# luotuoqingshan/SDPLRPlus.jl

Measured on NVIDIA B200. Metric: AL inner iterations per second, MaxCut on a synthetic 10M-vertex power-law graph (rank 10), higher is better.
Workload: dtype f64

## Files before the change

### sdplrplus.jl_b200/csrc/api.cu

```cuda
#include <math.h>
#include <stdlib.h>
#include <string.h>
#include <algorithm>
#include "common.cuh"

static const char *kNoHandle = "null handle";

#define REQUIRE_H(h) \
    if (!(h)) return SDPLRP_ERR_ARG
#define REQUIRE_PRE(h)                                                                   \
    if (!(h)->preprocessed) return fail(h, SDPLRP_ERR_STATE, "call sdplrp_preprocess first")
#define REQUIRE_RANK(h)                                                                  \
    if ((h)->r <= 0) return fail(h, SDPLRP_ERR_STATE, "call sdplrp_set_rank first")

int32_t fetch_scalars(sdplrp_handle *h, int first, int count) {
    CUDA_TRY(h, cudaMemcpyAsync(h->hscal + first, h->dscal + first, (size_t)count * sizeof(double), cudaMemcpyDeviceToHost, h->stream));
    CUDA_TRY(h, cudaStreamSynchronize(h->stream));
    return SDPLRP_OK;
}

cudaEvent_t prof_begin(sdplrp_handle *h) {
    cudaEvent_t e = nullptr;
    if (!h->ev_free.empty()) { e = h->ev_free.back(); h->ev_free.pop_back(); }
    else if (cudaEventCreate(&e) != cudaSuccess) return nullptr;
    cudaEventRecord(e, h->stream);
    return e;
}
void prof_end(sdplrp_handle *h, int sec, cudaEvent_t a) {
    cudaEvent_t e = nullptr;
    if (!h->ev_free.empty()) { e = h->ev_free.back(); h->ev_free.pop_back(); }
    else if (cudaEventCreate(&e) != cudaSuccess) { h->ev_free.push_back(a); return; }
    cudaEventRecord(e, h->stream);
    h->ev_pending.push_back({sec, a, e});
}
static void prof_collect(sdplrp_handle *h) {
    for (auto &p : h->ev_pending) {
        float ms = 0.f;
        if (cudaEventElapsedTime(&ms, p.a, p.b) == cudaSuccess) { h->sec_ms[p.sec] += ms; h->sec_cnt[p.sec] += 1; }
        h->ev_free.push_back(p.a); h->ev_free.push_back(p.b);
    }
    h->ev_pending.clear();
}

static double *mat_ptr(sdplrp_handle *h, int id) {
    switch (id) {
    case SDPLRP_MAT_R: return h->R;
    case SDPLRP_MAT_G: return h->G;
    case SDPLRP_MAT_D: return h->D;
    case SDPLRP_MAT_W0: return h->W0;
    case SDPLRP_MAT_W1: return h->W1;
    case SDPLRP_MAT_CR: return h->CR;
    case SDPLRP_MAT_CD: return h->CD;
    default: break;
    }
    if (id >= SDPLRP_MAT_S0 && id < SDPLRP_MAT_S0 + h->hist) return h->Sh[id - SDPLRP_MAT_S0];
    if (id >= SDPLRP_MAT_Y0 && id < SDPLRP_MAT_Y0 + h->hist) return h->Yh[id - SDPLRP_MAT_Y0];
    return nullptr;
}

static double *vec_ptr(sdplrp_handle *h, int id, i64 *len) {
    switch (id) {
    case SDPLRP_VEC_LAMBDA: *len = h->m; return h->lambda;
    case SDPLRP_VEC_LAMBDA_UB: *len = h->m; return h->lambda_ub;
    case SDPLRP_VEC_B: *len = h->m; return h->b;
    case SDPLRP_VEC_PVIO_RAW: *len = h->m + 1; return h->pvio_raw;
    case SDPLRP_VEC_Y: *len = h->m + 1; return h->y;
    case SDPLRP_VEC_PVIO_LB: *len = h->m; return h->pvio_lb;
    case SDPLRP_VEC_A_RD: *len = h->m + 1; return h->A_RD;
    case SDPLRP_VEC_A_DD: *len = h->m + 1; return h->A_DD;
    case SDPLRP_VEC_S_NZVAL: *len = h->nnzF; return h->S;
    default: return nullptr;
    }
}

__global__ void k_fill(i64 len, double v, double *__restrict__ x) {
    for (i64 i = blockIdx.x * (i64)blockDim.x + threadIdx.x; i < len; i += (i64)gridDim.x * blockDim.x) x[i] = v;
}
__global__ void k_bounds(i64 m, const unsigned char *__restrict__ ineq, const int *__restrict__ cperm, double *__restrict__ ub,
                         double *__restrict__ lb) {
    for (i64 g = blockIdx.x * (i64)blockDim.x + threadIdx.x; g < m; g += (i64)gridDim.x * blockDim.x) {
        const bool q = ineq && ineq[g];
        const i64 c = cperm ? cperm[g] : g;
        ub[c] = q ? 0.0 : INFINITY;
        lb[c] = q ? 0.0 : -INFINITY;
    }
}

extern "C" {

int32_t sdplrp_version(void) { return 100; }

const char *sdplrp_error_string(int32_t code) {
    switch (code) {
    case SDPLRP_OK: return "ok";
    case SDPLRP_ERR_CUDA: return "CUDA runtime error";
    case SDPLRP_ERR_ARG: return "bad argument";
    case SDPLRP_ERR_STATE: return "call order violated";
    case SDPLRP_ERR_ASYMMETRIC: return "constraint matrix not stored symmetric";
    case SDPLRP_ERR_NCCL: return "NCCL error";
    case SDPLRP_ERR_NO_DEVICE: return "no CUDA device (there is no CPU fallback)";
    case SDPLRP_ERR_LINESEARCH: return "line search slope is positive";
    default: return "unknown error";
    }
}

const char *sdplrp_last_error(sdplrp_handle *h) { return h ? h->err.c_str() : kNoHandle; }

int32_t sdplrp_create(int32_t device, int32_t rank, int32_t world, const void *nccl_id, sdplrp_handle **out) {
    if (!out) return SDPLRP_ERR_ARG;
    *out = nullptr;
    int ndev = 0;
    if (cudaGetDeviceCount(&ndev) != cudaSuccess || ndev <= 0) return SDPLRP_ERR_NO_DEVICE;
    if (device < 0 || device >= ndev || world < 1 || rank < 0 || rank >= world) return SDPLRP_ERR_ARG;
    if (cudaSetDevice(device) != cudaSuccess) return SDPLRP_ERR_CUDA;
    sdplrp_handle *h = new sdplrp_handle();
    h->device = device; h->rank = rank; h->world = world;
    if (const char *e = getenv("SDPLRP_RELABEL")) h->relabel_mode = atoi(e) < 0 ? -1 : (atoi(e) > 0 ? 1 : 0);
    if (const char *e = getenv("SDPLRP_HOT_ROWS")) h->hot_rows = atoll(e);
    if (const char *e = getenv("SDPLRP_LBFGS_KERNEL")) h->lbfgs_kernel = atoi(e);
    if (const char *e = getenv("SDPLRP_SPMM_UNROLL")) h->spmm_unroll = atoi(e);
    if (const char *e = getenv("SDPLRP_SPMM_G0")) h->spmm_g0 = atoi(e);
    if (const char *e = getenv("SDPLRP_LANCZOS_DIST")) h->lanczos_dist = atoi(e) > 0 ? 1 : 0;
    if (cudaStreamCreateWithFlags(&h->stream, cudaStreamNonBlocking) != cudaSuccess) { delete h; return SDPLRP_ERR_CUDA; }
    {
        const char *e = getenv("SDPLRP_CLASS_STREAMS");
        if (!e || atoi(e) != 0) {
            bool ok = cudaEventCreateWithFlags(&h->ev_fork, cudaEventDisableTiming) == cudaSuccess;
            for (int c = 0; c < 2 && ok; c++)
                ok = cudaStreamCreateWithFlags(&h->class_streams[c], cudaStreamNonBlocking) == cudaSuccess &&
                     cudaEventCreateWithFlags(&h->ev_join[c], cudaEventDisableTiming) == cudaSuccess;
            if (!ok) { cudaGetLastError(); h->class_streams[0] = nullptr; }
        }
    }
    if (const char *e = getenv("SDPLRP_L2_FETCH")) {
        if (cudaDeviceSetLimit(cudaLimitMaxL2FetchGranularity, (size_t)atoll(e)) != cudaSuccess) cudaGetLastError();
    }
    if (const char *e = getenv("SDPLRP_L2_PERSIST_MB")) {
        int maxp = 0;
        cudaDeviceGetAttribute(&maxp, cudaDevAttrMaxPersistingL2CacheSize, device);
        const size_t want = std::min<size_t>((size_t)maxp, (size_t)atoll(e) << 20);
        if (cudaDeviceSetLimit(cudaLimitPersistingL2CacheSize, want) == cudaSuccess) h->l2_persist_bytes = (i64)want;
        else cudaGetLastError();
    }
    bool ok = cudaMalloc((void **)&h->dscal, SC_COUNT * sizeof(double)) == cudaSuccess &&
              cudaMallocHost((void **)&h->hscal, SC_COUNT * sizeof(double)) == cudaSuccess &&
              cudaMalloc((void **)&h->partials, (size_t)kPartialsLen * sizeof(double)) == cudaSuccess &&
              cudaMalloc((void **)&h->ticket, 4 * sizeof(unsigned)) == cudaSuccess;
    if (ok) ok = cudaMemset(h->dscal, 0, SC_COUNT * sizeof(double)) == cudaSuccess && cudaMemset(h->ticket, 0, 4 * sizeof(unsigned)) == cudaSuccess;
    if (!ok) { sdplrp_destroy(h); return SDPLRP_ERR_CUDA; }
    memset(h->hscal, 0, SC_COUNT * sizeof(double));
    if (world > 1) {
        int32_t rc = comm_init(h, nccl_id);
        if (rc != SDPLRP_OK) { sdplrp_destroy(h); return rc; }
    }
    *out = h;
    return SDPLRP_OK;
}

static i64 mat_capacity(const sdplrp_handle *h, int r) {
    const i64 rows = h->equal_blocks ? std::max<i64>(h->n, (i64)h->world * h->block_rows) : h->n;
    return rows * (i64)r;
}

static void free_state(sdplrp_handle *h) {
    dev_free(&h->R); dev_free(&h->G); dev_free(&h->D); dev_free(&h->W0); dev_free(&h->W1);
    dev_free(&h->CR); dev_free(&h->CD);
    h->CR_valid = h->CD_valid = false;
    for (int j = 0; j < kMaxHist; j++) { dev_free(&h->Sh[j]); dev_free(&h->Yh[j]); }
    dev_free(&h->lb_small);
    h->gram_pairs_valid = h->gram_g_valid = false; h->gram_prestored = -1;
    dev_free(&h->lr_tmp); h->lr_tmp_len = 0;
    h->r = 0; h->hist = 0;
    h->state_cap = 0;
}

static void free_problem(sdplrp_handle *h) {
    pre_free(h);
    for (LowRank &L : h->lr) { dev_free(&L.dB); dev_free(&L.dD); }
    h->lr.clear();
    dev_free(&h->b); dev_free(&h->lambda); dev_free(&h->lambda_ub); dev_free(&h->pvio_lb);
    dev_free(&h->y); dev_free(&h->pvio_raw); dev_free(&h->pvio_raw_alt); dev_free(&h->A_RD); dev_free(&h->A_DD); dev_free(&h->A_out);
    dev_free(&h->lz_v); dev_free(&h->lz_w); dev_free(&h->lz_vp); dev_free(&h->lz_ab); dev_free(&h->lz_basis);
    h->lz_ab_len = 0; h->lz_basis_len = 0;
    dev_free(&h->stage); h->stage_len = 0;
}

int32_t sdplrp_destroy(sdplrp_handle *h) {
    if (!h) return SDPLRP_OK;
    cudaSetDevice(h->device);
    if (h->stream) cudaStreamSynchronize(h->stream);
    comm_destroy(h);
    prof_collect(h);
    for (cudaEvent_t e : h->ev_free) cudaEventDestroy(e);
    h->ev_free.clear();
    free_state(h);
    free_problem(h);
    dev_free(&h->dscal); dev_free(&h->partials); dev_free(&h->ticket);
    if (h->hscal) cudaFreeHost(h->hscal);
    for (int c = 0; c < 2; c++) {
        if (h->class_streams[c]) cudaStreamDestroy(h->class_streams[c]);
        if (h->ev_join[c]) cudaEventDestroy(h->ev_join[c]);
    }
    if (h->ev_fork) cudaEventDestroy(h->ev_fork);
    if (h->stream) cudaStreamDestroy(h->stream);
    delete h;
    return SDPLRP_OK;
}

int32_t sdplrp_synchronize(sdplrp_handle *h) {
    REQUIRE_H(h);
    CUDA_TRY(h, cudaStreamSynchronize(h->stream));
    return SDPLRP_OK;
}

void *sdplrp_stream(sdplrp_handle *h) { return h ? (void *)h->stream : nullptr; }

static int32_t preprocess_common(sdplrp_handle *h, int64_t n, int64_t m, int64_t nA, const int64_t *mat_off, const int64_t *I,
                                 const int64_t *J, const double *V, const int64_t *gids, bool triplets_on_device);

int32_t sdplrp_preprocess(sdplrp_handle *h, int64_t n, int64_t m, int64_t nA, const int64_t *mat_off, const int64_t *I,
                          const int64_t *J, const double *V, const int64_t *gids) {
    return preprocess_common(h, n, m, nA, mat_off, I, J, V, gids, false);
}

int32_t sdplrp_preprocess_device(sdplrp_handle *h, int64_t n, int64_t m, int64_t nA, const int64_t *mat_off, const int64_t *d_I,
                                 const int64_t *d_J, const double *d_V, const int64_t *gids) {
    REQUIRE_H(h);
    if (nA > 0 && mat_off && mat_off[nA] > 0) {
        if (!d_I || !d_J || !d_V) return fail(h, SDPLRP_ERR_ARG, "preprocess_device: null triplet arrays");
        cudaPointerAttributes at;
        const void *ptrs[3] = {d_I, d_J, d_V};
        for (const void *p : ptrs) {
            if (cudaPointerGetAttributes(&at, p) != cudaSuccess || at.type != cudaMemoryTypeDevice || at.device != h->device) {
                cudaGetLastError();
                return fail(h, SDPLRP_ERR_ARG, "preprocess_device: I, J, V must be device memory of the handle's GPU");
            }
        }
    }
    return preprocess_common(h, n, m, nA, mat_off, d_I, d_J, d_V, gids, true);
}

static int32_t preprocess_common(sdplrp_handle *h, int64_t n, int64_t m, int64_t nA, const int64_t *mat_off, const int64_t *I,
                                 const int64_t *J, const double *V, const int64_t *gids, bool triplets_on_device) {
    REQUIRE_H(h);
    CUDA_TRY(h, cudaSetDevice(h->device));
    free_state(h);
    free_problem(h);
    if (nA > 0 && (!mat_off || !gids)) return fail(h, SDPLRP_ERR_ARG, "preprocess: null arrays");
    int32_t rc = pre_build(h, n, m, nA, mat_off, I, J, V, gids, triplets_on_device);
    if (rc != SDPLRP_OK && rc != SDPLRP_ERR_ASYMMETRIC) return rc;
    SDP_CHECK(dev_alloc(h, &h->b, m)); SDP_CHECK(dev_alloc(h, &h->lambda, m)); SDP_CHECK(dev_alloc(h, &h->lambda_ub, m));
    SDP_CHECK(dev_alloc(h, &h->pvio_lb, m)); SDP_CHECK(dev_alloc(h, &h->y, m + 1)); SDP_CHECK(dev_alloc(h, &h->pvio_raw, m + 1)); SDP_CHECK(dev_alloc(h, &h->pvio_raw_alt, m + 1));
    SDP_CHECK(dev_alloc(h, &h->A_RD, m + 1)); SDP_CHECK(dev_alloc(h, &h->A_DD, m + 1)); SDP_CHECK(dev_alloc(h, &h->A_out, m + 1));
    cudaStream_t st = h->stream;
    CUDA_TRY(h, cudaMemsetAsync(h->b, 0, (size_t)std::max<i64>(m, 1) * 8, st));
    CUDA_TRY(h, cudaMemsetAsync(h->lambda, 0, (size_t)std::max<i64>(m, 1) * 8, st));
    CUDA_TRY(h, cudaMemsetAsync(h->y, 0, (size_t)(m + 1) * 8, st));
    CUDA_TRY(h, cudaMemsetAsync(h->pvio_raw, 0, (size_t)(m + 1) * 8, st));
    CUDA_TRY(h, cudaMemsetAsync(h->pvio_raw_alt, 0, (size_t)(m + 1) * 8, st));
    CUDA_TRY(h, cudaMemsetAsync(h->A_RD, 0, (size_t)(m + 1) * 8, st));
    CUDA_TRY(h, cudaMemsetAsync(h->A_DD, 0, (size_t)(m + 1) * 8, st));
    CUDA_TRY(h, cudaMemsetAsync(h->A_out, 0, (size_t)(m + 1) * 8, st));
    k_bounds<<<grid_for(m, 256, kRedBlocks), 256, 0, st>>>(m, nullptr, h->cperm, h->lambda_ub, h->pvio_lb);
    KLAUNCH(h);
    CUDA_TRY(h, cudaStreamSynchronize(st));
    h->y_obj = 0.0;
    SDP_CHECK(comm_partition(h));
    SDP_CHECK(halo_build(h));
    return rc;
}

int32_t sdplrp_halo_stats(sdplrp_handle *h, int64_t out[7]) {
    REQUIRE_H(h);
    REQUIRE_PRE(h);
    const HaloPlan &p = h->halo;
    out[0] = halo_active(h) ? 1 : 0; out[1] = p.nloc; out[2] = p.lnnz; out[3] = p.n_ghost[0]; out[4] = p.n_ghost[1];
    out[5] = p.n_send[0]; out[6] = p.n_send[1];
    return SDPLRP_OK;
}

int32_t sdplrp_pattern_sizes(sdplrp_handle *h, int64_t *nnzT, int64_t *nnzF, int64_t *Ec) {
    REQUIRE_H(h);
    REQUIRE_PRE(h);
    if (nnzT) *nnzT = h->nnzT;
    if (nnzF) *nnzF = h->nnzF;
    if (Ec) *Ec = h->Ec;
    return SDPLRP_OK;
}

int32_t sdplrp_pattern_export(sdplrp_handle *h, int64_t *triu_colptr, int64_t *triu_rowval, int64_t *matptr, int64_t *nzind,
                              double *nzval_one, double *nzval_two, int64_t *full_colptr, int64_t *full_rowval,
                              int64_t *mappedto_triu) {
    REQUIRE_H(h);
    REQUIRE_PRE(h);
    CUDA_TRY(h, cudaSetDevice(h->device));
    return pre_export(h, triu_colptr, triu_rowval, matptr, nzind, nzval_one, nzval_two, full_colptr, full_rowval, mappedto_triu);
}

int32_t sdplrp_add_symlowrank(sdplrp_handle *h, int64_t global_id, int64_t s, const double *B, const double *D) {
    REQUIRE_H(h);
    REQUIRE_PRE(h);
    if (global_id < 1 || global_id > h->m + 1 || s < 1 || !B || !D) return fail(h, SDPLRP_ERR_ARG, "add_symlowrank: bad argument");
    CUDA_TRY(h, cudaSetDevice(h->device));
    LowRank L;
    int gid_internal = (int)(global_id - 1);
    CUDA_TRY(h, cudaMemcpy(&gid_internal, h->cperm + (global_id - 1), sizeof(int), cudaMemcpyDeviceToHost));
    L.gid = gid_internal; L.s = s; L.dB = nullptr; L.dD = nullptr;
    SDP_CHECK(dev_alloc(h, &L.dB, h->n * s));
    SDP_CHECK(dev_alloc(h, &L.dD, s));
    h->lr.push_back(L);
    SDP_CHECK(perm_upload(h, L.dB, B, s, false));
    CUDA_TRY(h, cudaMemcpy(L.dD, D, (size_t)s * 8, cudaMemcpyHostToDevice));
    return SDPLRP_OK;
}

int32_t sdplrp_set_problem(sdplrp_handle *h, const double *b, const uint8_t *is_ineq) {
    REQUIRE_H(h);
    REQUIRE_PRE(h);
    CUDA_TRY(h, cudaSetDevice(h->device));
    const i64 m = h->m;
    if (m > 0 && !b) return fail(h, SDPLRP_ERR_ARG, "set_problem: null b");
    if (m > 0) SDP_CHECK(perm_cvec_upload(h, h->b, b, m));
    unsigned char *dq = nullptr;
    h->has_ineq = false;
    if (is_ineq) for (i64 i = 0; i < m; i++) h->has_ineq |= is_ineq[i] != 0;
    if (is_ineq && m > 0) {
        CUDA_TRY(h, cudaMalloc((void **)&dq, (size_t)m));
        CUDA_TRY(h, cudaMemcpy(dq, is_ineq, (size_t)m, cudaMemcpyHostToDevice));
    }
    k_bounds<<<grid_for(m, 256, kRedBlocks), 256, 0, h->stream>>>(m, dq, h->cperm, h->lambda_ub, h->pvio_lb);
    KLAUNCH(h);
    cudaError_t e = cudaStreamSynchronize(h->stream);
    if (dq) cudaFree(dq);
    CUDA_TRY(h, e);
    return SDPLRP_OK;
}

int32_t sdplrp_set_rank(sdplrp_handle *h, int32_t r, int32_t numlbfgsvecs) {
    REQUIRE_H(h);
    REQUIRE_PRE(h);
    if (r < 1 || numlbfgsvecs < 0 || numlbfgsvecs > kMaxHist) return fail(h, SDPLRP_ERR_ARG, "set_rank: bad rank / history length");
    CUDA_TRY(h, cudaSetDevice(h->device));
    const i64 N = mat_capacity(h, r);
    const bool reuse = h->R && h->G && h->D && h->lb_small && h->r == r && h->hist == numlbfgsvecs && h->state_cap == N &&
                       ((h->obj_mat >= 0) == (h->CR != nullptr)) && ((h->obj_mat >= 0) == (h->CD != nullptr));
    if (reuse) {
        h->CR_valid = h->CD_valid = false;
        if (h->W0) CUDA_TRY(h, cudaMemsetAsync(h->W0, 0, (size_t)N * 8, h->stream));
        if (h->W1) CUDA_TRY(h, cudaMemsetAsync(h->W1, 0, (size_t)N * 8, h->stream));
    } else {
        free_state(h);
        SDP_CHECK(dev_alloc(h, &h->R, N)); SDP_CHECK(dev_alloc(h, &h->G, N)); SDP_CHECK(dev_alloc(h, &h->D, N));
        if (h->obj_mat >= 0) { SDP_CHECK(dev_alloc(h, &h->CR, N)); SDP_CHECK(dev_alloc(h, &h->CD, N)); }
        for (int j = 0; j < numlbfgsvecs; j++) { SDP_CHECK(dev_alloc(h, &h->Sh[j], N)); SDP_CHECK(dev_alloc(h, &h->Yh[j], N)); }
        SDP_CHECK(dev_alloc(h, &h->lb_small, kLbSmallLen));
        h->state_cap = N;
    }
    h->r = r; h->hist = numlbfgsvecs; h->latest = numlbfgsvecs;
    CUDA_TRY(h, cudaMemsetAsync(h->R, 0, (size_t)N * 8, h->stream));
    CUDA_TRY(h, cudaMemsetAsync(h->G, 0, (size_t)N * 8, h->stream));
    CUDA_TRY(h, cudaMemsetAsync(h->D, 0, (size_t)N * 8, h->stream));
    SDP_CHECK(lb_clear(h));
    CUDA_TRY(h, cudaStreamSynchronize(h->stream));
    return SDPLRP_OK;
}

int32_t sdplrp_set_option(sdplrp_handle *h, const char *key, double value) {
    REQUIRE_H(h);
    if (!key) return fail(h, SDPLRP_ERR_ARG, "set_option: null key");
    const std::string k(key);
    if (k == "relabel") { h->relabel_mode = value < 0 ? -1 : (value > 0 ? 1 : 0); return SDPLRP_OK; }
    if (k == "hot_rows") { h->hot_rows = (i64)value; return SDPLRP_OK; }
    if (k == "spmm_phases") { h->spmm_phases = value < 0 ? 0 : (int)value; return SDPLRP_OK; }
    if (k == "lanczos_dist") { h->lanczos_dist = value > 0 ? 1 : 0; return SDPLRP_OK; }
    if (k == "row_group_max") { h->row_group_max = std::max(1, std::min((int)value, kRowWarpMax)); return SDPLRP_OK; }
    if (k == "spmm_unroll") { h->spmm_unroll = (int)value; return SDPLRP_OK; }
    if (k == "spmm_g0") { h->spmm_g0 = (int)value; return SDPLRP_OK; }
    if (k == "rowc_kernel") { h->rowc_kernel = value > 0 ? 1 : 0; return SDPLRP_OK; }
    if (k == "tail_ctas") { h->tail_ctas = std::max(0, std::min((int)value, 8)); return SDPLRP_OK; }
    if (k == "halo") { h->halo_mode = value < 0.5 ? 0 : (value < 1.5 ? 1 : (value < 2.5 ? 2 : 3)); return SDPLRP_OK; }
    if (k == "gather_mode") { h->gather_mode = value < 0 ? 0 : (int)value; return SDPLRP_OK; }
    if (k == "gather_tile") { h->gather_tile = (int)value; return SDPLRP_OK; }
    if (k == "gather_stages") { h->gather_stages = (int)value; return SDPLRP_OK; }
    if (k == "gather_warps") { h->gather_warps = (int)value; return SDPLRP_OK; }
    if (k == "gather_hints") { h->gather_hints = value > 0 ? 1 : 0; return SDPLRP_OK; }
    if (k == "fused_tail") { h->fused_tail = value != 0; return SDPLRP_OK; }
    if (k == "lbfgs_kernel") { h->lbfgs_kernel = (int)value; h->gram_pairs_valid = h->gram_g_valid = false; return SDPLRP_OK; }
    return fail(h, SDPLRP_ERR_ARG, "set_option: unknown key " + k);
}

int32_t sdplrp_set_sigma(sdplrp_handle *h, double sigma) { REQUIRE_H(h); h->sigma = sigma; return SDPLRP_OK; }
int32_t sdplrp_get_sigma(sdplrp_handle *h, double *sigma) { REQUIRE_H(h); *sigma = h->sigma; return SDPLRP_OK; }
int32_t sdplrp_get_obj(sdplrp_handle *h, double *obj) {
    REQUIRE_H(h);
    SDP_CHECK(fetch_scalars(h, SC_OBJ, 1));
    *obj = h->hscal[SC_OBJ];
    return SDPLRP_OK;
}

static int32_t lazy_scratch(sdplrp_handle *h, int id) {
    const i64 N = mat_capacity(h, h->r);
    if (id == SDPLRP_MAT_W0 && !h->W0) { SDP_CHECK(dev_alloc(h, &h->W0, N)); CUDA_TRY(h, cudaMemset(h->W0, 0, (size_t)N * 8)); }
    if (id == SDPLRP_MAT_W1 && !h->W1) { SDP_CHECK(dev_alloc(h, &h->W1, N)); CUDA_TRY(h, cudaMemset(h->W1, 0, (size_t)N * 8)); }
    return SDPLRP_OK;
}

int32_t sdplrp_upload_mat(sdplrp_handle *h, int32_t id, const double *src) {
    REQUIRE_H(h);
    REQUIRE_RANK(h);
    CUDA_TRY(h, cudaSetDevice(h->device));
    SDP_CHECK(lazy_scratch(h, id));
    if (id == SDPLRP_MAT_CR || id == SDPLRP_MAT_CD) return fail(h, SDPLRP_ERR_ARG, "upload_mat: CR / CD are download-only");
    double *p = mat_ptr(h, id);
    if (!p || !src) return fail(h, SDPLRP_ERR_ARG, "upload_mat: bad id");
    SDP_CHECK(perm_upload(h, p, src, h->r, true));
    comm_mark_full(h, id);
    if (id == SDPLRP_MAT_R) h->CR_valid = false;
    if (id == SDPLRP_MAT_D) { h->CD_valid = false; h->ls_valid = false; }
    if (id == SDPLRP_MAT_R) h->ls_valid = false;
    if (id == SDPLRP_MAT_G) h->gram_g_valid = false;
    if (id >= SDPLRP_MAT_S0) { h->gram_pairs_valid = false; h->gram_prestored = -1; }
    return SDPLRP_OK;
}

int32_t sdplrp_upload_mat_slice(sdplrp_handle *h, int32_t id, const double *src) {
    REQUIRE_H(h);
    REQUIRE_RANK(h);
    if (h->world <= 1) return sdplrp_upload_mat(h, id, src);
    CUDA_TRY(h, cudaSetDevice(h->device));
    SDP_CHECK(lazy_scratch(h, id));
    if (id == SDPLRP_MAT_CR || id == SDPLRP_MAT_CD) return fail(h, SDPLRP_ERR_ARG, "upload_mat: CR / CD are download-only");
    double *p = mat_ptr(h, id);
    if (!p || !src) return fail(h, SDPLRP_ERR_ARG, "upload_mat_slice: bad id");
    SDP_CHECK(perm_upload_slice(h, p, src, h->r));
    comm_mark_full(h, id);
    if (id == SDPLRP_MAT_R) { h->CR_valid = false; h->ls_valid = false; }
    if (id == SDPLRP_MAT_D) { h->CD_valid = false; h->ls_valid = false; }
    if (id == SDPLRP_MAT_G) h->gram_g_valid = false;
    if (id >= SDPLRP_MAT_S0) { h->gram_pairs_valid = false; h->gram_prestored = -1; }
    return SDPLRP_OK;
}

int32_t sdplrp_download_mat_slice(sdplrp_handle *h, int32_t id, double *dst) {
    REQUIRE_H(h);
    REQUIRE_RANK(h);
    if (h->world <= 1) return sdplrp_download_mat(h, id, dst);
    CUDA_TRY(h, cudaSetDevice(h->device));
    SDP_CHECK(lazy_scratch(h, id));
    double *p = mat_ptr(h, id);
    if (!p || !dst) return fail(h, SDPLRP_ERR_ARG, "download_mat_slice: bad id");
    SDP_CHECK(comm_gather_rows(h, p, id));
    return perm_download_slice(h, p, dst, h->r);
}

int32_t sdplrp_download_mat(sdplrp_handle *h, int32_t id, double *dst) {
    REQUIRE_H(h);
    REQUIRE_RANK(h);
    CUDA_TRY(h, cudaSetDevice(h->device));
    SDP_CHECK(lazy_scratch(h, id));
    double *p = mat_ptr(h, id);
    if (!p || !dst) return fail(h, SDPLRP_ERR_ARG, "download_mat: bad id");
    SDP_CHECK(comm_gather_rows(h, p, id));
    return perm_download(h, p, dst, h->r, true);
}

int32_t sdplrp_upload_vec(sdplrp_handle *h, int32_t id, const double *src, int64_t len) {
    REQUIRE_H(h);
    REQUIRE_PRE(h);
    CUDA_TRY(h, cudaSetDevice(h->device));
    i64 want = 0;
    double *p = vec_ptr(h, id, &want);
    if (!p || !src || len != want) return fail(h, SDPLRP_ERR_ARG, "upload_vec: bad id or length");
    if (id == SDPLRP_VEC_S_NZVAL) {
        SDP_CHECK(perm_slots_upload(h, p, src, len));
    } else {
        SDP_CHECK(perm_cvec_upload(h, p, src, len));
    }
    if (id == SDPLRP_VEC_Y) { h->y_obj = src[h->m]; h->S_current = false; }
    if (id == SDPLRP_VEC_S_NZVAL) { h->S_static_valid = false; h->S_current = true; }
    return SDPLRP_OK;
}

int32_t sdplrp_download_vec(sdplrp_handle *h, int32_t id, double *dst, int64_t len) {
    REQUIRE_H(h);
    REQUIRE_PRE(h);
    CUDA_TRY(h, cudaSetDevice(h->device));
    if (id == SDPLRP_VEC_TRIUS_NZVAL) {
        if (len != h->nnzT || !dst) return fail(h, SDPLRP_ERR_ARG, "download_vec: bad length");
        double *tmp = nullptr;
        SDP_CHECK(dev_alloc(h, &tmp, h->nnzT));
        int32_t rc = grad_triuS(h, tmp);
        if (rc == SDPLRP_OK && len > 0) {
            cudaError_t e = cudaMemcpyAsync(dst, tmp, (size_t)len * 8, cudaMemcpyDeviceToHost, h->stream);
            if (e == cudaSuccess) e = cudaStreamSynchronize(h->stream);
            if (e != cudaSuccess) { h->err = cudaGetErrorString(e); rc = SDPLRP_ERR_CUDA; }
        }
        cudaFree(tmp);
        return rc;
    }
    i64 want = 0;
    double *p = vec_ptr(h, id, &want);
    if (!p || !dst || len != want) return fail(h, SDPLRP_ERR_ARG, "download_vec: bad id or length");
    if (id == SDPLRP_VEC_S_NZVAL) return perm_slots_download(h, p, dst, len);
    SDP_CHECK(comm_gather_cvec(h, p));
    return perm_cvec_download(h, p, dst, len);
}

static int32_t copy_out(sdplrp_handle *h, double *dev, double *host, i64 len) {
    if (!host) return SDPLRP_OK;
    SDP_CHECK(comm_gather_cvec(h, dev));
    return perm_cvec_download(h, dev, host, len);
}

int32_t sdplrp_A_uu(sdplrp_handle *h, int32_t U_id, double *out) {
    REQUIRE_H(h); REQUIRE_PRE(h); REQUIRE_RANK(h);
    CUDA_TRY(h, cudaSetDevice(h->device));
    SDP_CHECK(lazy_scratch(h, U_id));
    const double *U = mat_ptr(h, U_id);
    if (!U) return fail(h, SDPLRP_ERR_ARG, "A_uu: bad matrix id");
    SDP_CHECK(comm_require_full(h, U_id));
    SDP_CHECK(aop_uu(h, U, h->A_out));
    SDP_CHECK(comm_reduce_mvec(h, h->A_out, nullptr));
    return copy_out(h, h->A_out, out, h->m + 1);
}

int32_t sdplrp_A_uv(sdplrp_handle *h, int32_t U_id, int32_t V_id, double *out) {
    REQUIRE_H(h); REQUIRE_PRE(h); REQUIRE_RANK(h);
    CUDA_TRY(h, cudaSetDevice(h->device));
    SDP_CHECK(lazy_scratch(h, U_id)); SDP_CHECK(lazy_scratch(h, V_id));
    const double *U = mat_ptr(h, U_id), *V = mat_ptr(h, V_id);
    if (!U || !V) return fail(h, SDPLRP_ERR_ARG, "A_uv: bad matrix id");
    SDP_CHECK(comm_require_full(h, U_id)); SDP_CHECK(comm_require_full(h, V_id));
    SDP_CHECK(aop_uv(h, U, V, h->A_out));
    SDP_CHECK(comm_reduce_mvec(h, h->A_out, nullptr));
    return copy_out(h, h->A_out, out, h->m + 1);
}

int32_t sdplrp_At_preprocess(sdplrp_handle *h, const double *y) {
    REQUIRE_H(h); REQUIRE_PRE(h);
    CUDA_TRY(h, cudaSetDevice(h->device));
    if (y) {
        SDP_CHECK(perm_cvec_upload(h, h->y, y, h->m + 1));
        h->y_obj = y[h->m];
    }
    return grad_assemble_S(h);
}

int32_t sdplrp_At_left(sdplrp_handle *h, int32_t X_id, int32_t Y_id) {
    REQUIRE_H(h); REQUIRE_PRE(h); REQUIRE_RANK(h);
    CUDA_TRY(h, cudaSetDevice(h->device));
    SDP_CHECK(lazy_scratch(h, X_id)); SDP_CHECK(lazy_scratch(h, Y_id));
    const double *X = mat_ptr(h, X_id);
    double *Y = mat_ptr(h, Y_id);
    if (!X || !Y || X == Y) return fail(h, SDPLRP_ERR_ARG, "At_left: bad matrix ids");
    SDP_CHECK(comm_require_full(h, X_id));
    if (!h->S_current) SDP_CHECK(grad_assemble_S(h));
    SDP_CHECK(grad_spmm(h, X, Y, 1.0, false));
    comm_mark_partial(h, Y_id);
    return SDPLRP_OK;
}

int32_t sdplrp_At_right(sdplrp_handle *h, const double *x, double *y, int64_t ncols) {
    REQUIRE_H(h); REQUIRE_PRE(h);
    if (!x || !y || ncols < 1) return fail(h, SDPLRP_ERR_ARG, "At_right: bad argument");
    CUDA_TRY(h, cudaSetDevice(h->device));
    double *dx = nullptr, *dy = nullptr;
    const i64 len = h->n * ncols;
    SDP_CHECK(dev_alloc(h, &dx, len));
    int32_t rc = dev_alloc(h, &dy, len);
    if (rc == SDPLRP_OK && !h->S_current) rc = grad_assemble_S(h);
    if (rc == SDPLRP_OK) rc = perm_upload(h, dx, x, ncols, false);
    if (rc == SDPLRP_OK) rc = grad_spmv(h, dx, dy, ncols);
    if (rc == SDPLRP_OK) rc = perm_download(h, dy, y, ncols, false);
    cudaFree(dx);
    if (dy) cudaFree(dy);
    return rc;
}

static bool needs_remote_R_rows(const sdplrp_handle *h) {
    const i64 general = h->nA - h->n_sd - (h->obj_mat >= 0 ? 1 : 0);
    return general > 0 || h->n_dynF > 0;
}

static int32_t rebuild_CR(sdplrp_handle *h) {
    if (halo_active(h)) SDP_CHECK(halo_begin(h, h->R));
    else SDP_CHECK(comm_require_full(h, SDPLRP_MAT_R));
    SectionScope sc(h, SDPLRP_SEC_SPMM);
    SDP_CHECK(grad_obj_spmm(h, h->R, h->CR, nullptr, h->dscal + SC_SUMS));
    h->CR_valid = true;
    return SDPLRP_OK;
}

__global__ void k_store_sum3(const double *__restrict__ sums6, double *out) { *out = sums6[0] + sums6[2] + sums6[4]; }

static int32_t do_f(sdplrp_handle *h) {
    if (!halo_active(h)) SDP_CHECK(comm_require_full(h, SDPLRP_MAT_R));
    const bool split = h->obj_mat >= 0;
    {
        SectionScope sc(h, SDPLRP_SEC_A_UU);
        SDP_CHECK(aop_uu_skip(h, h->R, h->pvio_raw, split));
    }
    if (split) {
        SDP_CHECK(rebuild_CR(h));
        k_store_sum3<<<1, 1, 0, h->stream>>>(h->dscal + SC_SUMS, h->pvio_raw + h->m);
        KLAUNCH(h);
    }
    SDP_CHECK(comm_reduce_mvec(h, h->pvio_raw, nullptr));
    SectionScope sc(h, SDPLRP_SEC_F_FINISH);
    return vec_f_finish(h);
}

static int32_t do_g(sdplrp_handle *h) {
    if (h->obj_mat >= 0 && !h->CR_valid) SDP_CHECK(rebuild_CR(h));
    if (needs_remote_R_rows(h)) SDP_CHECK(comm_require_full(h, SDPLRP_MAT_R));
    {
        SectionScope sc(h, SDPLRP_SEC_S_ASSEMBLE);
        SDP_CHECK(grad_form_y(h));
    }
    {
        SectionScope sc(h, SDPLRP_SEC_GRAD);
        SDP_CHECK(grad_hot(h));
    }
    h->gram_g_valid = false;
    comm_mark_partial(h, SDPLRP_MAT_G);
    SectionScope sc(h, SDPLRP_SEC_NORMS);
    SDP_CHECK(comm_reduce_scalars(h, SC_GNORM2, 1));
    return vec_pnorm2(h);
}

int32_t sdplrp_f(sdplrp_handle *h, double *L, double *obj) {
    REQUIRE_H(h); REQUIRE_PRE(h); REQUIRE_RANK(h);
    CUDA_TRY(h, cudaSetDevice(h->device));
    SDP_CHECK(do_f(h));
    SDP_CHECK(fetch_scalars(h, SC_OBJ, 2));
    if (obj) *obj = h->hscal[SC_OBJ];
    if (L) *L = h->hscal[SC_LVAL];
    return SDPLRP_OK;
}

int32_t sdplrp_g(sdplrp_handle *h, double *gnorm2, double *pnorm2) {
    REQUIRE_H(h); REQUIRE_PRE(h); REQUIRE_RANK(h);
    CUDA_TRY(h, cudaSetDevice(h->device));
    SDP_CHECK(do_g(h));
    SDP_CHECK(fetch_scalars(h, SC_GNORM2, 2));
    if (gnorm2) *gnorm2 = h->hscal[SC_GNORM2];
    if (pnorm2) *pnorm2 = h->hscal[SC_PNORM2];
    return SDPLRP_OK;
}

int32_t sdplrp_fg(sdplrp_handle *h, double out[4]) {
    REQUIRE_H(h); REQUIRE_PRE(h); REQUIRE_RANK(h);
    CUDA_TRY(h, cudaSetDevice(h->device));
    SDP_CHECK(do_f(h));
    SDP_CHECK(do_g(h));
    SDP_CHECK(fetch_scalars(h, SC_GNORM2, 4));
    out[0] = h->hscal[SC_LVAL]; out[1] = h->hscal[SC_OBJ]; out[2] = h->hscal[SC_GNORM2]; out[3] = h->hscal[SC_PNORM2];
    return SDPLRP_OK;
}

int32_t api_lbfgs_dir_async(sdplrp_handle *h) {
    REQUIRE_H(h); REQUIRE_PRE(h); REQUIRE_RANK(h);
    CUDA_TRY(h, cudaSetDevice(h->device));
    {
        SectionScope sc(h, SDPLRP_SEC_LBFGS_DIR);
        SDP_CHECK(lb_dir(h));
    }
    h->CD_valid = false; h->ls_valid = false;
    comm_mark_partial(h, SDPLRP_MAT_D);
    return SDPLRP_OK;
}

int32_t sdplrp_lbfgs_dir(sdplrp_handle *h, double *descent) {
    SDP_CHECK(api_lbfgs_dir_async(h));
    SDP_CHECK(fetch_scalars(h, SC_DESCENT, 1));
    if (descent) *descent = h->hscal[SC_DESCENT];
    return SDPLRP_OK;
}

int32_t sdplrp_use_gradient_direction(sdplrp_handle *h) {
    REQUIRE_H(h); REQUIRE_PRE(h); REQUIRE_RANK(h);
    CUDA_TRY(h, cudaSetDevice(h->device));
    SDP_CHECK(lb_neg_copy(h));
    h->gram_g_valid = false;
    h->CD_valid = false; h->ls_valid = false;
    comm_mark_partial(h, SDPLRP_MAT_D);
    return SDPLRP_OK;
}

int32_t api_linesearch_coeffs_descent(sdplrp_handle *h, double bq[5], double *descent) {
    REQUIRE_H(h); REQUIRE_PRE(h); REQUIRE_RANK(h);
    CUDA_TRY(h, cudaSetDevice(h->device));
    const bool split = h->obj_mat >= 0;
    if (split && !h->CR_valid) SDP_CHECK(rebuild_CR(h));
    if (halo_active(h)) SDP_CHECK(halo_begin(h, h->D));
    else SDP_CHECK(comm_require_full(h, SDPLRP_MAT_D));
    if (needs_remote_R_rows(h)) SDP_CHECK(comm_require_full(h, SDPLRP_MAT_R));
    {
        SectionScope sc(h, SDPLRP_SEC_LS_PASS);
        SDP_CHECK(aop_linesearch(h, split));
    }
    if (split) {
        SectionScope sc(h, SDPLRP_SEC_SPMM);
        SDP_CHECK(grad_obj_spmm(h, h->D, h->CD, h->CR, h->dscal + SC_SUMS));
        SDP_CHECK(grad_obj_slots(h, h->dscal + SC_SUMS, h->A_RD + h->m, h->A_DD + h->m));
        h->CD_valid = true;
    }
    SDP_CHECK(comm_reduce_mvec(h, h->A_RD, h->A_DD));
    {
        SectionScope sc(h, SDPLRP_SEC_LS_COEFF);
        SDP_CHECK(vec_biquadratic(h));
    }
    h->ls_valid = true;
    static_assert(SC_DESCENT < SC_BQ, "one contiguous fetch covers descent and the coefficients");
    SDP_CHECK(fetch_scalars(h, SC_DESCENT, SC_BQ + 5 - SC_DESCENT));
    for (int k = 0; k < 5; k++) bq[k] = h->hscal[SC_BQ + k];
    if (descent) *descent = h->hscal[SC_DESCENT];
    return SDPLRP_OK;
}

int32_t sdplrp_linesearch_coeffs(sdplrp_handle *h, double bq[5]) { return api_linesearch_coeffs_descent(h, bq, nullptr); }


int32_t sdplrp_step(sdplrp_handle *h, double alpha, double *obj) {
    REQUIRE_H(h); REQUIRE_PRE(h); REQUIRE_RANK(h);
    CUDA_TRY(h, cudaSetDevice(h->device));
    {
        SectionScope sc(h, SDPLRP_SEC_STEP);
        SDP_CHECK(vec_commit(h, alpha));
        const bool recur = h->obj_mat >= 0 && h->CR_valid && h->CD_valid;
        if (recur && h->world == 1) {
            SDP_CHECK(lb_axpy2(h, alpha, h->D, h->R, h->CD, h->CR));
        } else {
            SDP_CHECK(comm_step_R(h, alpha));
            if (recur) SDP_CHECK(lb_axpy(h, alpha, h->CD, h->CR));
            else h->CR_valid = false;
        }
    }
    h->ls_valid = false;
    if (obj) {
        SDP_CHECK(fetch_scalars(h, SC_OBJ, 1));
        *obj = h->hscal[SC_OBJ];
    }
    return SDPLRP_OK;
}

int32_t sdplrp_step_g(sdplrp_handle *h, double alpha, double out[3]) {
    REQUIRE_H(h); REQUIRE_PRE(h); REQUIRE_RANK(h);
    if (!out) return fail(h, SDPLRP_ERR_ARG, "step_g: null output");
    CUDA_TRY(h, cudaSetDevice(h->device));
    const bool split = h->obj_mat >= 0;
    const bool fused = h->fused_tail && h->ls_valid && (!split || (h->CR_valid && h->CD_valid));
    if (fused) {
        SectionScope sc(h, SDPLRP_SEC_TAIL);
        SDP_CHECK(grad_step_fused(h, alpha));
        h->ls_valid = false; h->CD_valid = false;
        h->gram_g_valid = false;
    } else {
        SDP_CHECK(sdplrp_step(h, alpha, nullptr));
        SDP_CHECK(do_g(h));
    }
    SDP_CHECK(fetch_scalars(h, SC_GNORM2, 3));
    out[0] = h->hscal[SC_OBJ]; out[1] = h->hscal[SC_GNORM2]; out[2] = h->hscal[SC_PNORM2];
    return SDPLRP_OK;
}

int32_t sdplrp_lbfgs_update(sdplrp_handle *h, double alpha) {
    REQUIRE_H(h); REQUIRE_PRE(h); REQUIRE_RANK(h);
    CUDA_TRY(h, cudaSetDevice(h->device));
    SectionScope sc(h, SDPLRP_SEC_LBFGS_UPDATE);
    return lb_update(h, alpha);
}

int32_t sdplrp_lbfgs_clear(sdplrp_handle *h) {
    REQUIRE_H(h); REQUIRE_PRE(h); REQUIRE_RANK(h);
    CUDA_TRY(h, cudaSetDevice(h->device));
    return lb_clear(h);
}

int32_t sdplrp_dual_update(sdplrp_handle *h) {
    REQUIRE_H(h); REQUIRE_PRE(h);
    CUDA_TRY(h, cudaSetDevice(h->device));
    return vec_dual_update(h);
}

int32_t sdplrp_armijo_eval(sdplrp_handle *h, const double *alphas, int32_t k, double *L, double *slope) {
    REQUIRE_H(h); REQUIRE_PRE(h);
    if (k < 0 || (k > 0 && (!alphas || !L))) return fail(h, SDPLRP_ERR_ARG, "armijo_eval: bad argument");
    CUDA_TRY(h, cudaSetDevice(h->device));
    return vec_armijo(h, alphas, k, L, slope);
}

int32_t sdplrp_lanczos(sdplrp_handle *h, int64_t q, const double *v0, uint64_t seed, int32_t reorth, double *alpha, double *beta,
                       int64_t *iters) {
    REQUIRE_H(h); REQUIRE_PRE(h);
    if (q < 1 || !alpha || !beta || !iters) return fail(h, SDPLRP_ERR_ARG, "lanczos: bad argument");
    CUDA_TRY(h, cudaSetDevice(h->device));
    i64 it = 0;
    if (!h->S_current) SDP_CHECK(grad_assemble_S(h));
    {
        SectionScope sc(h, SDPLRP_SEC_LANCZOS);
        SDP_CHECK(lz_run(h, q, v0, seed, reorth, alpha, beta, &it));
    }
    *iters = it;
    return SDPLRP_OK;
}

int32_t sdplrp_tridiag_mineig(const double *d, const double *e, int64_t k, double *out) {
    if (!d || !out || k < 1 || (k > 1 && !e)) return SDPLRP_ERR_ARG;
    *out = tridiag_mineig_host(d, e, k);
    return SDPLRP_OK;
}

int32_t sdplrp_dual_obj(sdplrp_handle *h, double trace_bound, int64_t iter, const double *v0, uint64_t seed, double *dual_value,
                        double *mineig, int64_t *lanczos_steps) {
    REQUIRE_H(h); REQUIRE_PRE(h);
    CUDA_TRY(h, cudaSetDevice(h->device));
    SDP_CHECK(grad_form_y(h));
    SDP_CHECK(grad_assemble_S(h));
    const double it = (double)std::max<i64>(iter, 100);
    i64 q = (i64)(2.0 * ceil(sqrt(it) * log((double)h->n)));
    q = std::max<i64>(1, std::min<i64>(q, h->n - 1));
    std::vector<double> a((size_t)q), b((size_t)q);
    i64 steps = 0;
    {
        SectionScope sc(h, SDPLRP_SEC_LANCZOS);
        SDP_CHECK(lz_run(h, q, v0, seed, 0, a.data(), b.data(), &steps));
    }
    for (i64 i = 0; i < steps; i++) a[(size_t)i] += 1.0;
    const double lam = (steps == 1 ? a[0] : tridiag_mineig_host(a.data(), b.data(), steps)) - 1.0;
    double yb = 0.0;
    SDP_CHECK(vec_dual_dot(h, &yb));
    if (dual_value) *dual_value = yb + trace_bound * std::min(lam, 0.0);
    if (mineig) *mineig = lam;
    if (lanczos_steps) *lanczos_steps = steps;
    return SDPLRP_OK;
}

int32_t sdplrp_dense_symeig(const double *A, int64_t k, double *ev, double *Q) {
    if (!A || !ev || k < 1 || k > 4096) return SDPLRP_ERR_ARG;
    dense_symeig_host(A, k, ev, Q);
    return SDPLRP_OK;
}

int32_t sdplrp_S_eigval(sdplrp_handle *h, int64_t nevs, int64_t ncv, double tol, int64_t maxiter, const double *v0, uint64_t seed,
                        double *eigvals, double *bounds, int64_t *matvecs, int64_t *restarts) {
    REQUIRE_H(h); REQUIRE_PRE(h);
    if (!eigvals) return fail(h, SDPLRP_ERR_ARG, "S_eigval: eigvals is null");
    CUDA_TRY(h, cudaSetDevice(h->device));
    if (!h->S_current) SDP_CHECK(grad_assemble_S(h));
    i64 mv = 0, rs = 0;
    {
        SectionScope sc(h, SDPLRP_SEC_LANCZOS);
        SDP_CHECK(lz_eigs(h, nevs, ncv, tol, maxiter, v0, seed, eigvals, bounds, &mv, &rs));
    }
    if (matvecs) *matvecs = mv;
    if (restarts) *restarts = rs;
    return SDPLRP_OK;
}

int32_t sdplrp_dual_obj_highprecision(sdplrp_handle *h, double trace_bound, const double *v0, uint64_t seed, double *dual_value,
                                      double *mineig, int64_t *matvecs) {
    REQUIRE_H(h); REQUIRE_PRE(h);
    CUDA_TRY(h, cudaSetDevice(h->device));
    SDP_CHECK(grad_form_y(h));
    SDP_CHECK(grad_assemble_S(h));
    double lam = 0.0;
    i64 mv = 0;
    {
        SectionScope sc(h, SDPLRP_SEC_LANCZOS);
        SDP_CHECK(lz_eigs(h, 1, std::min<i64>(100, h->n), 1e-6, 1000000, v0, seed, &lam, nullptr, &mv, nullptr));
    }
    double yb = 0.0;
    SDP_CHECK(vec_dual_dot(h, &yb));
    if (dual_value) *dual_value = yb + trace_bound * std::min(lam, 0.0);
    if (mineig) *mineig = lam;
    if (matvecs) *matvecs = mv;
    return SDPLRP_OK;
}

int32_t sdplrp_dimacs_errors(sdplrp_handle *h, double normb, double normC, const double *v0, uint64_t seed, double errs[6]) {
    REQUIRE_H(h); REQUIRE_PRE(h); REQUIRE_RANK(h);
    if (!errs) return fail(h, SDPLRP_ERR_ARG, "dimacs_errors: errs is null");
    CUDA_TRY(h, cudaSetDevice(h->device));
    double raw2 = 0.0, lamb = 0.0, obj = 0.0;
    SDP_CHECK(vec_dimacs_sums(h, &raw2, &lamb));
    SDP_CHECK(fetch_scalars(h, SC_OBJ, 1));
    obj = h->hscal[SC_OBJ];
    SDP_CHECK(vec_copy2y_lambda(h));
    SDP_CHECK(grad_assemble_S(h));
    double lam = 0.0;
    {
        SectionScope sc(h, SDPLRP_SEC_LANCZOS);
        SDP_CHECK(lz_eigs(h, 1, std::min<i64>(100, h->n), 0.0, 1000000, v0, seed, &lam, nullptr, nullptr, nullptr));
    }
    SDP_CHECK(lazy_scratch(h, SDPLRP_MAT_W0));
    SDP_CHECK(comm_require_full(h, SDPLRP_MAT_R));
    SDP_CHECK(grad_spmm_sparse(h, h->R, h->W0, 1.0));
    comm_mark_partial(h, SDPLRP_MAT_W0);
    SDP_CHECK(lb_dot(h, h->R, h->W0, SC_LANCZOS + 9));
    SDP_CHECK(comm_reduce_scalars(h, SC_LANCZOS + 9, 1));
    SDP_CHECK(fetch_scalars(h, SC_LANCZOS + 9, 1));
    const double xz = h->hscal[SC_LANCZOS + 9];
    const double den = 1.0 + fabs(obj) + fabs(lamb);
    errs[0] = sqrt(raw2) / (1.0 + normb);
    errs[1] = 0.0;
    errs[2] = 0.0;
    errs[3] = std::max(0.0, -lam) / (1.0 + normC);
    errs[4] = (obj - lamb) / den;
    errs[5] = xz / den;
    return SDPLRP_OK;
}

int32_t sdplrp_set_profiling(sdplrp_handle *h, int32_t on) {
    REQUIRE_H(h);
    h->prof = on != 0;
    return SDPLRP_OK;
}

int32_t sdplrp_section_times(sdplrp_handle *h, double *ms, int64_t *counts) {
    REQUIRE_H(h);
    CUDA_TRY(h, cudaSetDevice(h->device));
    CUDA_TRY(h, cudaStreamSynchronize(h->stream));
    prof_collect(h);
    for (int k = 0; k < SDPLRP_SEC_COUNT; k++) {
        if (ms) ms[k] = h->sec_ms[k];
        if (counts) counts[k] = h->sec_cnt[k];
        h->sec_ms[k] = 0.0; h->sec_cnt[k] = 0;
    }
    return SDPLRP_OK;
}

int32_t sdplrp_launch_count(sdplrp_handle *h, int64_t *count) {
    REQUIRE_H(h);
    if (count) *count = h->launches;
    return SDPLRP_OK;
}

int32_t sdplrp_row_range(sdplrp_handle *h, int64_t *lo, int64_t *hi) {
    REQUIRE_H(h);
    if (lo) *lo = h->row_lo;
    if (hi) *hi = h->row_hi;
    return SDPLRP_OK;
}

}
```

### sdplrplus.jl_b200/csrc/common.cuh

```cuda
#pragma once
#include <cuda_runtime.h>
#include <stdint.h>
#include <string>
#include <vector>
#include "../../include/sdplrp_b200.h"

typedef long long i64;

constexpr int kNumSM = 148;
constexpr int kMaxHist = 32;
constexpr int kRedBlocks = 4 * kNumSM;
constexpr int kRedThreads = 256;
constexpr int kMaxRedK = 64;
constexpr int kLbSmallLen = 17 * 17 + 3 * 17 + 17 + 7;
constexpr long long kPartialsLen = (long long)kRedBlocks * kMaxRedK * 8;
constexpr int kLongMatThreshold = 64;
constexpr int kChunkEntries = 2048;
constexpr int kRowGroupMax = 64;
constexpr int kRowWarpMax = 512;

struct RowClasses {
    int *list[3] = {nullptr, nullptr, nullptr};
    long long cnt[3] = {0, 0, 0};
    int *storage = nullptr;
};

struct TileLayout {
    long long n_long = 0, n_chunks = 0;
    int *long_rows = nullptr;
    int *long_cptr = nullptr;
    int *chunk_start = nullptr, *chunk_end = nullptr, *chunk_row = nullptr;
};

struct GatherPlan {
    int4 *tiles = nullptr;
    long long ntiles = 0, n_long = 0, n_chunks = 0;
    int *long_rows = nullptr;
    int *long_cptr = nullptr;
    const int *ptr_key = nullptr;
    long long row_lo = 0, row_hi = 0;
    int T = 0;
};

struct HaloPlan {
    bool active = false;
    long long nloc = 0, lnnz = 0;
    long long n_ghost[2] = {0, 0};
    long long n_send[2] = {0, 0};
    int *lptr = nullptr, *lmid = nullptr, *lidx = nullptr;
    double *lval = nullptr;
    RowClasses cls;
    TileLayout longs;
    int *send_rows[2] = {nullptr, nullptr};
    std::vector<long long> send_off[2], recv_off[2];
    double *sendbuf = nullptr;
    double *xc = nullptr;
    long long sendbuf_len = 0, xc_len = 0;
};

struct LowRank {
    i64 gid;
    i64 s;
    double *dB;
    double *dD;
};

enum {
    SC_DOT = 0,
    SC_DESCENT = 1,
    SC_GNORM2 = 2,
    SC_PNORM2 = 3,
    SC_OBJ = 4,
    SC_LVAL = 5,
    SC_BQ = 8,
    SC_RHO = 32,
    SC_A = 64,
    SC_SUMS = 16,
    SC_LANCZOS = 96,
    SC_COUNT = 128
};

struct sdplrp_handle {
    int device = 0, rank = 0, world = 1;
    cudaStream_t stream = nullptr;
    std::string err;
    i64 launches = 0;
    void *nccl = nullptr;

    i64 n = 0, m = 0, nA = 0, nnzT = 0, nnzF = 0, Ec = 0;
    i64 row_lo = 0, row_hi = 0;
    std::vector<i64> row_starts;
    i64 c_lo = 0, c_hi = 0;
    std::vector<i64> c_starts;
    bool mat_full[8] = {true, true, true, true, true, true, true, true};
    bool preprocessed = false;
    bool has_ineq = false;

    int *triu_colptr = nullptr, *triu_rowval = nullptr;
    int *ref_full_ptr = nullptr, *ref_full_idx = nullptr;
    int *mapped = nullptr;
    bool relabeled = false;
    bool equal_blocks = false;
    i64 block_rows = 0;
    bool dealt = false;
    int relabel_mode = -1;
    int *perm = nullptr, *iperm = nullptr;
    int *i2r = nullptr, *r2i = nullptr;
    int *full_ptr = nullptr, *full_idx = nullptr;
    double *S = nullptr;
    double *stage = nullptr;
    i64 stage_len = 0;
    i64 l2_persist_bytes = 0;
    i64 hot_rows = -1;
    int row_group_max = kRowGroupMax;
    int spmm_unroll = 8;
    int tail_ctas = 0;
    int rowc_kernel = 1;
    int spmm_g0 = 1;
    int spmm_phases = 0;
    int lanczos_dist = 1;
    cudaStream_t class_streams[2] = {nullptr, nullptr};
    cudaEvent_t ev_fork = nullptr, ev_join[2] = {nullptr, nullptr};
    bool fork_open = false;
    int halo_mode = 3;
    HaloPlan halo;
    void *nccl_halo = nullptr;
    cudaStream_t comm_stream = nullptr;
    cudaEvent_t ev_pack = nullptr, ev_class[2] = {nullptr, nullptr};
    int gather_mode = 0;
    int gather_tile = 0, gather_stages = 0, gather_warps = 0;
    int gather_hints = 0;
    i64 gather_attr_smem[2][5] = {{0}};
    GatherPlan full_plan;
    int *row_mid = nullptr;
    i64 row_mid_cols = -1;
    int *matptr = nullptr;
    int *mat_gid = nullptr;
    int *ent_slot = nullptr;
    int *ent_row = nullptr, *ent_col = nullptr;
    double *ent_one = nullptr, *ent_two = nullptr;
    i64 n_long = 0, n_chunks = 0;
    int *long_mat = nullptr;
    int *long_chunk_ptr = nullptr;
    int *chunk_mat = nullptr;
    double *chunk_part = nullptr;
    int obj_mat = -1;
    double *triuS_static = nullptr;
    double S_static_scale = 0.0;
    bool S_static_valid = false;
    bool S_current = false;
    i64 n_dyn = 0;
    int *dyn_slot = nullptr;
    int *dyn_ptr = nullptr;
    int *dyn_gid = nullptr;
    double *dyn_val = nullptr;
    int *dyn_pos_a = nullptr, *dyn_pos_b = nullptr;
    double *Cfull = nullptr;
    double *dynS = nullptr;
    i64 n_dynF = 0;
    int *dynrow_ptr = nullptr;
    int *dynrow_col = nullptr;
    int *dynrow_src = nullptr;
    int *dyn_diag = nullptr;
    i64 n_sd = 0;
    int *rowc_ptr = nullptr;
    double *rowc_val = nullptr;
    int *cperm = nullptr;
    int *dyn_nsd_end = nullptr;
    i64 n_dyn_nsd = 0;
    unsigned char *sd_flag = nullptr;
    RowClasses full_cls, dyn_cls;
    TileLayout full_long, dyn_long;
    double *tile_scratch = nullptr;
    i64 tile_scratch_len = 0;
    double *CR = nullptr, *CD = nullptr;
    bool CR_valid = false, CD_valid = false;
    i64 state_cap = 0;
    bool ls_valid = false;
    bool fused_tail = true;

    std::vector<LowRank> lr;
    double *lr_tmp = nullptr;
    i64 lr_tmp_len = 0;

    double *b = nullptr, *lambda = nullptr, *lambda_ub = nullptr, *pvio_lb = nullptr;
    double *y = nullptr, *pvio_raw = nullptr, *A_RD = nullptr, *A_DD = nullptr, *A_out = nullptr;
    double *pvio_raw_alt = nullptr;
    double sigma = 2.0;
    double y_obj = 0.0;

    int r = 0, hist = 0, latest = 0;
    double *R = nullptr, *G = nullptr, *D = nullptr, *W0 = nullptr, *W1 = nullptr;
    double *Sh[kMaxHist] = {nullptr}, *Yh[kMaxHist] = {nullptr};
    int lbfgs_kernel = 1;
    double *lb_small = nullptr;
    bool gram_pairs_valid = false, gram_g_valid = false;
    int gram_prestored = -1;

    double *dscal = nullptr;
    double *hscal = nullptr;
    double *partials = nullptr;
    unsigned *ticket = nullptr;
    bool prof = false;
    std::vector<cudaEvent_t> ev_free;
    struct Pending { int sec; cudaEvent_t a, b; };
    std::vector<Pending> ev_pending;
    double sec_ms[SDPLRP_SEC_COUNT] = {0};
    i64 sec_cnt[SDPLRP_SEC_COUNT] = {0};
    double *lz_v = nullptr, *lz_w = nullptr, *lz_vp = nullptr, *lz_ab = nullptr;
    i64 lz_ab_len = 0;
    double *lz_basis = nullptr;
    i64 lz_basis_len = 0;
};

#define CUDA_TRY(h, call)                                                                      \
    do {                                                                                       \
        cudaError_t e__ = (call);                                                              \
        if (e__ != cudaSuccess) {                                                              \
            (h)->err = std::string(#call) + ": " + cudaGetErrorString(e__);                    \
            return SDPLRP_ERR_CUDA;                                                            \
        }                                                                                      \
    } while (0)

#define SDP_CHECK(expr)                        \
    do {                                       \
        int32_t rc__ = (expr);                 \
        if (rc__ != SDPLRP_OK) return rc__;    \
    } while (0)

#define KLAUNCH(h) ((h)->launches++)

static inline int32_t fail(sdplrp_handle *h, int32_t code, const std::string &msg) {
    h->err = msg;
    return code;
}

template <typename T>
static inline int32_t dev_alloc(sdplrp_handle *h, T **p, i64 count) {
    if (*p) { cudaFree(*p); *p = nullptr; }
    if (count <= 0) count = 1;
    CUDA_TRY(h, cudaMalloc((void **)p, (size_t)count * sizeof(T)));
    return SDPLRP_OK;
}
template <typename T>
static inline void dev_free(T **p) {
    if (*p) { cudaFree(*p); *p = nullptr; }
}

static inline int grid_for(i64 work_items, int per_block, int max_blocks = 1 << 30) {
    i64 g = (work_items + per_block - 1) / per_block;
    if (g < 1) g = 1;
    if (g > max_blocks) g = max_blocks;
    return (int)g;
}

__device__ __forceinline__ double warp_sum(double v) {
#pragma unroll
    for (int o = 16; o > 0; o >>= 1) v += __shfl_xor_sync(0xffffffffu, v, o);
    return v;
}

template <int K>
__device__ __forceinline__ void block_sum(double (&v)[K]) {
    __shared__ double sm[K][32];
    const int lane = threadIdx.x & 31, wid = threadIdx.x >> 5, nw = blockDim.x >> 5;
#pragma unroll
    for (int k = 0; k < K; k++) v[k] = warp_sum(v[k]);
    __syncthreads();
    if (lane == 0) {
#pragma unroll
        for (int k = 0; k < K; k++) sm[k][wid] = v[k];
    }
    __syncthreads();
    if (wid == 0) {
#pragma unroll
        for (int k = 0; k < K; k++) {
            double t = lane < nw ? sm[k][lane] : 0.0;
            v[k] = warp_sum(t);
        }
    }
}

template <int K, typename Fin>
__device__ __forceinline__ void grid_sum_finalize(double (&v)[K], double *partials, unsigned *ticket, Fin fin) {
    block_sum<K>(v);
    __shared__ bool is_last;
    if (threadIdx.x == 0) {
#pragma unroll
        for (int k = 0; k < K; k++) partials[(size_t)blockIdx.x * K + k] = v[k];
        __threadfence();
        unsigned t = atomicAdd(ticket, 1u);
        is_last = (t == gridDim.x - 1);
    }
    __syncthreads();
    if (is_last) {
        __threadfence();
        double s[K];
#pragma unroll
        for (int k = 0; k < K; k++) s[k] = 0.0;
        for (unsigned bI = threadIdx.x; bI < gridDim.x; bI += blockDim.x) {
#pragma unroll
            for (int k = 0; k < K; k++) s[k] += __ldcg(&partials[(size_t)bI * K + k]);
        }
        block_sum<K>(s);
        if (threadIdx.x == 0) {
            fin(s);
            *ticket = 0u;
        }
    }
}

__device__ __forceinline__ double2 ldg2(const double *p) { return __ldg(reinterpret_cast<const double2 *>(p)); }

int32_t pre_build(sdplrp_handle *h, i64 n, i64 m, i64 nA, const int64_t *mat_off, const int64_t *I,
                  const int64_t *J, const double *V, const int64_t *gids, bool triplets_on_device = false);
int32_t pre_export(sdplrp_handle *h, int64_t *triu_colptr, int64_t *triu_rowval, int64_t *matptr,
                   int64_t *nzind, double *one, double *two, int64_t *full_colptr, int64_t *full_rowval,
                   int64_t *mapped);
void pre_free(sdplrp_handle *h);

int32_t aop_uu(sdplrp_handle *h, const double *U, double *out_dev);
int32_t aop_uv(sdplrp_handle *h, const double *U, const double *V, double *out_dev);
int32_t aop_linesearch(sdplrp_handle *h, bool skip_objective);
int32_t aop_uu_skip(sdplrp_handle *h, const double *U, double *out_dev, bool skip_objective);

int32_t lr_project(sdplrp_handle *h, const LowRank &L, const double *X, double *dst);
int32_t lr_scratch(sdplrp_handle *h);

int32_t grad_form_y(sdplrp_handle *h);
int32_t grad_assemble_S(sdplrp_handle *h);
int32_t grad_spmm(sdplrp_handle *h, const double *X, double *Y, double scale, bool want_norm);
int32_t grad_spmm_sparse(sdplrp_handle *h, const double *X, double *Y, double scale);
int32_t grad_obj_spmm(sdplrp_handle *h, const double *X, double *Y, const double *Z, double *sums6);
int32_t grad_obj_slots(sdplrp_handle *h, const double *sums6, double *a_rd_m, double *a_dd_m);
int32_t grad_hot(sdplrp_handle *h);
int32_t grad_step_fused(sdplrp_handle *h, double alpha);
int32_t vec_tail_rest(sdplrp_handle *h, double alpha, const double *raw_in, double *raw_out, double *pn2_out);
int32_t grad_spmv(sdplrp_handle *h, const double *x, double *y, i64 ncols);
int32_t grad_triuS(sdplrp_handle *h, double *out_dev);

bool gather_supported(const sdplrp_handle *h);
int gather_tile_size(const sdplrp_handle *h);
void gather_plan_free(GatherPlan &p);
int32_t gather_plan_build(sdplrp_handle *h, GatherPlan &p, const int *ptr_dev, i64 row_lo, i64 row_hi, int T);
int32_t gather_spmm(sdplrp_handle *h, const GatherPlan &plan, const int *ptr, const int *idx, const double *val, const double *Xg,
                    const double *X, const double *Z, double *Y, int epi, double scale, double *sums4);

i64 tile_hot_rows(const sdplrp_handle *h);

int32_t vec_f_finish(sdplrp_handle *h);
int32_t vec_biquadratic(sdplrp_handle *h);
int32_t vec_commit(sdplrp_handle *h, double alpha);
int32_t vec_pnorm2(sdplrp_handle *h);
int32_t vec_dual_update(sdplrp_handle *h);
int32_t vec_armijo(sdplrp_handle *h, const double *alphas, int k, double *L, double *slope);
int32_t vec_dual_dot(sdplrp_handle *h, double *out);
int32_t vec_copy2y_lambda(sdplrp_handle *h);
int32_t vec_dimacs_sums(sdplrp_handle *h, double *raw_norm2, double *lambda_b);

int32_t lb_dir(sdplrp_handle *h);
int32_t lb_update(sdplrp_handle *h, double alpha);
int32_t lb_clear(sdplrp_handle *h);
int32_t lb_axpy(sdplrp_handle *h, double alpha, const double *x, double *y);
int32_t lb_axpy2(sdplrp_handle *h, double alpha, const double *x1, double *y1, const double *x2, double *y2);
int32_t lb_neg_copy(sdplrp_handle *h);
int32_t lb_norm2(sdplrp_handle *h, const double *x, int slot);
int32_t lb_dot(sdplrp_handle *h, const double *x, const double *y, int slot);

int32_t lz_run(sdplrp_handle *h, i64 q, const double *v0_host, uint64_t seed, int reorth, double *alpha,
               double *beta, i64 *iters);
double tridiag_mineig_host(const double *d, const double *e, i64 k);
void dense_symeig_host(const double *A, i64 m, double *ev, double *Q);
int32_t lz_eigs(sdplrp_handle *h, i64 nev, i64 ncv, double tol, i64 maxiter, const double *v0_host, uint64_t seed, double *eigs,
                double *bounds, i64 *matvecs, i64 *restarts);

int32_t comm_init(sdplrp_handle *h, const void *nccl_id);
void comm_destroy(sdplrp_handle *h);
int32_t comm_partition(sdplrp_handle *h);
void comm_mark_partial(sdplrp_handle *h, int mat_id);
void comm_mark_full(sdplrp_handle *h, int mat_id);
int32_t comm_require_full(sdplrp_handle *h, int mat_id);
int32_t comm_gather_rows(sdplrp_handle *h, double *p, int mat_id);
int32_t comm_reduce_mvec(sdplrp_handle *h, double *v1, double *v2);
int32_t comm_gather_rowvec(sdplrp_handle *h, double *v);
int32_t comm_gather_cvec(sdplrp_handle *h, double *v);
int32_t comm_reduce_scalars(sdplrp_handle *h, int slot, int count);
int32_t comm_check_same(sdplrp_handle *h, unsigned long long value, const char *what);
int32_t comm_reduce_ptr(sdplrp_handle *h, double *p, int count);
int32_t comm_step_R(sdplrp_handle *h, double alpha);
int32_t comm_allgather_bytes(sdplrp_handle *h, const void *send, void *recv, size_t bytes);
int32_t halo_build(sdplrp_handle *h);
void halo_free(sdplrp_handle *h);
bool halo_active(const sdplrp_handle *h);
int32_t halo_begin(sdplrp_handle *h, const double *X);
int32_t halo_wait(sdplrp_handle *h, int klass);

int32_t perm_stage(sdplrp_handle *h, i64 len);
int32_t perm_upload(sdplrp_handle *h, double *dst_dev, const double *src_host, i64 ncols, bool row_major);
int32_t perm_download(sdplrp_handle *h, const double *src_dev, double *dst_host, i64 ncols, bool row_major);
int32_t perm_upload_slice(sdplrp_handle *h, double *dst_dev, const double *src_host, i64 ncols);
int32_t perm_download_slice(sdplrp_handle *h, const double *src_dev, double *dst_host, i64 ncols);
int32_t comm_allgather_inplace(sdplrp_handle *h, double *buf, size_t cnt);
int32_t perm_device(sdplrp_handle *h, double *dst, const double *src, i64 ncols, bool row_major, bool to_internal);
int32_t perm_slots_upload(sdplrp_handle *h, double *dst_dev, const double *src_host, i64 len);
int32_t perm_slots_download(sdplrp_handle *h, const double *src_dev, double *dst_host, i64 len);
int32_t perm_cvec_upload(sdplrp_handle *h, double *dst_dev, const double *src_host, i64 len);
int32_t perm_cvec_download(sdplrp_handle *h, const double *src_dev, double *dst_host, i64 len);

cudaEvent_t prof_begin(sdplrp_handle *h);
void prof_end(sdplrp_handle *h, int sec, cudaEvent_t a);
struct SectionScope {
    sdplrp_handle *h; int sec; cudaEvent_t a;
    SectionScope(sdplrp_handle *h_, int sec_) : h(h_), sec(sec_), a(h_->prof ? prof_begin(h_) : nullptr) {}
    ~SectionScope() { if (a) prof_end(h, sec, a); }
};

int32_t fetch_scalars(sdplrp_handle *h, int first, int count);
```

### sdplrplus.jl_b200/csrc/driver.cu

```cuda
#include <math.h>
#include <stdio.h>
#include <algorithm>
#include <chrono>
#include <vector>
#include "common.cuh"

extern "C" {
int32_t api_lbfgs_dir_async(sdplrp_handle *h);
int32_t api_linesearch_coeffs_descent(sdplrp_handle *h, double bq[5], double *descent);
}

namespace {

constexpr double kEps = 2.220446049250313e-16;

double now_s() {
    return std::chrono::duration<double>(std::chrono::steady_clock::now().time_since_epoch()).count();
}

unsigned long long mix64(unsigned long long x) {
    x += 0x9E3779B97F4A7C15ull;
    x = (x ^ (x >> 30)) * 0xBF58476D1CE4E5B9ull;
    x = (x ^ (x >> 27)) * 0x94D049BB133111EBull;
    return x ^ (x >> 31);
}

double horner(const double *c, int deg, double x) {
    double v = c[deg];
    for (int k = deg - 1; k >= 0; k--) v = v * x + c[k];
    return v;
}

long double cubic_eval(const double *c, long double x) { return ((c[3] * x + c[2]) * x + c[1]) * x + c[0]; }

int cubic_roots_in(const double *c, double A, double *out) {
    double cuts[4];
    int nc = 0;
    cuts[nc++] = 0.0;
    const double qa = 3.0 * c[3], qb = 2.0 * c[2], qc = c[1];
    double cp[2];
    int ncp = 0;
    if (qa != 0.0) {
        const double disc = qb * qb - 4.0 * qa * qc;
        if (disc > 0.0) {
            const double t = -0.5 * (qb + (qb >= 0.0 ? 1.0 : -1.0) * sqrt(disc));
            cp[ncp++] = t / qa;
            if (t != 0.0) cp[ncp++] = qc / t;
        }
    } else if (qb != 0.0) {
        cp[ncp++] = -qc / qb;
    }
    if (ncp == 2 && cp[0] > cp[1]) std::swap(cp[0], cp[1]);
    for (int k = 0; k < ncp; k++)
        if (cp[k] > 0.0 && cp[k] < A && std::isfinite(cp[k])) cuts[nc++] = cp[k];
    cuts[nc++] = A;
    int nr = 0;
    for (int k = 0; k + 1 < nc; k++) {
        long double lo = cuts[k], hi = cuts[k + 1];
        long double flo = cubic_eval(c, lo), fhi = cubic_eval(c, hi);
        if (flo == 0.0L) { if (nr == 0 || out[nr - 1] != (double)lo) out[nr++] = (double)lo; continue; }
        if (fhi == 0.0L) { out[nr++] = (double)hi; continue; }
        if ((flo < 0.0L) == (fhi < 0.0L)) continue;
        for (int it = 0; it < 200; it++) {
            const long double mid = 0.5L * (lo + hi);
            if (mid <= lo || mid >= hi) break;
            const long double fm = cubic_eval(c, mid);
            if (fm == 0.0L) { lo = hi = mid; break; }
            if ((fm < 0.0L) == (flo < 0.0L)) { lo = mid; flo = fm; } else { hi = mid; }
        }
        out[nr++] = (double)(0.5L * (lo + hi));
    }
    return nr;
}

int32_t pick_alpha(const double bq[5], double alpha_max, double *alpha_star, double *f_star) {
    double cubic[4] = {bq[1], 2.0 * bq[2], 3.0 * bq[3], 4.0 * bq[4]};
    if (cubic[0] > kEps) return SDPLRP_ERR_LINESEARCH;
    if (fabs(cubic[3]) < kEps) cubic[3] = 0.0;
    double roots[5];
    int nr = cubic_roots_in(cubic, alpha_max, roots);
    roots[nr++] = alpha_max;
    double a_best = 0.0, f_best = bq[0];
    for (int i = 0; i < nr; i++) {
        const double x = roots[i];
        if (!(x >= 0.0) || x > alpha_max || !std::isfinite(x)) continue;
        const double fx = horner(bq, 4, x);
        if (fx < f_best) { f_best = fx; a_best = x; }
    }
    *alpha_star = a_best;
    *f_star = f_best;
    return SDPLRP_OK;
}

__global__ void k_fill_uniform(i64 n, int r, unsigned long long seed, const int *__restrict__ iperm, double *__restrict__ X) {
    const i64 total = n * r;
    for (i64 e = blockIdx.x * (i64)blockDim.x + threadIdx.x; e < total; e += (i64)gridDim.x * blockDim.x) {
        const i64 i = e / r, c = e - i * r;
        const unsigned long long v = (unsigned long long)(iperm ? iperm[i] : i);
        unsigned long long x = seed ^ (v * (unsigned long long)r + (unsigned long long)c) * 0xD6E8FEB86659FD93ull;
        x += 0x9E3779B97F4A7C15ull;
        x = (x ^ (x >> 30)) * 0xBF58476D1CE4E5B9ull;
        x = (x ^ (x >> 27)) * 0x94D049BB133111EBull;
        x ^= x >> 31;
        X[e] = 2.0 * ((double)(x >> 11) * (1.0 / 9007199254740992.0)) - 1.0;
    }
}

struct Driver {
    sdplrp_handle *h;
    const sdplrp_config &cfg;
    unsigned long long seed_ctr = 0;
    unsigned long long next_seed() { return mix64((unsigned long long)cfg.seed + 0x632BE59BD9B4E019ull * (++seed_ctr)); }
};

int32_t agree(sdplrp_handle *h, bool mine, bool *all) {
    if (h->world <= 1) { *all = mine; return SDPLRP_OK; }
    h->hscal[SC_LANCZOS + 11] = mine ? 1.0 : 0.0;
    CUDA_TRY(h, cudaMemcpyAsync(h->dscal + SC_LANCZOS + 11, h->hscal + SC_LANCZOS + 11, sizeof(double), cudaMemcpyHostToDevice, h->stream));
    SDP_CHECK(comm_reduce_scalars(h, SC_LANCZOS + 11, 1));
    SDP_CHECK(fetch_scalars(h, SC_LANCZOS + 11, 1));
    *all = h->hscal[SC_LANCZOS + 11] != 0.0;
    return SDPLRP_OK;
}

void print_row(const sdplrp_config &cfg, i64 T, i64 localiter, i64 it, double L, double obj, double sigma, double gtol, double ptol,
               double gn, double pn, double gap, double dual) {
    printf("T=%lld iter_T=%lld tot=%lld L=%.6e pobj=%.6e sigma=%g eta=%.2e omega=%.2e |grad|=%.3e |pinf|=%.3e gap=%.3e dobj=%.6e\n",
           (long long)T, (long long)localiter, (long long)it, L, obj, sigma, ptol, gtol, gn, pn, gap, dual);
    fflush(stdout);
}

int32_t inner_iteration(sdplrp_handle *h, bool use_armijo, double alpha_max, double *L_val, double *alpha_out, double sg[3]) {
    double descent = 0.0, alpha = 0.0, bq[5];
    SDP_CHECK(api_lbfgs_dir_async(h));
    SDP_CHECK(api_linesearch_coeffs_descent(h, bq, &descent));
    if (std::isnan(descent) || descent >= 0.0) {
        SDP_CHECK(sdplrp_use_gradient_direction(h));
        SDP_CHECK(sdplrp_linesearch_coeffs(h, bq));
    }
    if (!use_armijo) {
        if (pick_alpha(bq, alpha_max, &alpha, L_val) != SDPLRP_OK)
            return fail(h, SDPLRP_ERR_LINESEARCH, "Error: cubic[1] = " + std::to_string(bq[1]) + " should be less than 0.");
    } else {
        double L0 = 0.0, slope = 0.0, zero = 0.0;
        SDP_CHECK(sdplrp_armijo_eval(h, &zero, 1, &L0, &slope));
        double alphas[51], Ls[51];
        for (int k = 0; k < 51; k++) alphas[k] = alpha_max / pow(2.0, (double)k);
        int pick = 50;
        bool found = false;
        for (int s = 0; s < 51 && !found; s += 15) {
            const int cnt = std::min(15, 51 - s);
            SDP_CHECK(sdplrp_armijo_eval(h, alphas + s, cnt, Ls + s, nullptr));
            for (int k = s; k < s + cnt; k++)
                if (Ls[k] <= L0 + 1e-4 * alphas[k] * slope) { pick = k; found = true; break; }
        }
        alpha = alphas[pick]; *L_val = Ls[pick];
    }
    SDP_CHECK(sdplrp_step_g(h, alpha, sg));
    *alpha_out = alpha;
    return SDPLRP_OK;
}

}

extern "C" {

int32_t sdplrp_config_default(sdplrp_config *c) {
    if (!c) return SDPLRP_ERR_ARG;
    c->ptol = 1e-2; c->gtol = 0.0; c->objtol = 1e-2; c->sigma_0 = 2.0; c->sigmafac = 2.0; c->maxtime = 3600.0;
    c->printfreq = 60.0; c->fprec = 1e8; c->prior_trace_bound = 1e18; c->alpha_max = 1.0;
    c->maxmajoriter = 100000; c->maxiter = 10000000; c->numlbfgsvecs = 4; c->rankupd_tol = 4; c->printlevel = 1;
    c->gtol_relative = 1; c->ptol_relative = 1; c->objtol_relative = 1; c->eval_DIMACS_errs = 0; c->eigval_highprecision = 0;
    c->seed = 0;
    return SDPLRP_OK;
}

int32_t sdplrp_pick_alpha(const double biquadratic[5], double alpha_max, double *alpha, double *value) {
    if (!biquadratic || !alpha || !value) return SDPLRP_ERR_ARG;
    return pick_alpha(biquadratic, alpha_max, alpha, value);
}

int32_t sdplrp_fill_uniform(sdplrp_handle *h, int32_t mat_id, uint64_t seed) {
    if (!h) return SDPLRP_ERR_ARG;
    if (!h->preprocessed || h->r <= 0) return fail(h, SDPLRP_ERR_STATE, "fill_uniform: call sdplrp_set_rank first");
    double *X = mat_id == SDPLRP_MAT_R ? h->R : mat_id == SDPLRP_MAT_G ? h->G : mat_id == SDPLRP_MAT_D ? h->D : nullptr;
    if (!X) return fail(h, SDPLRP_ERR_ARG, "fill_uniform: R, G or D only");
    CUDA_TRY(h, cudaSetDevice(h->device));
    k_fill_uniform<<<grid_for(h->n * h->r, 256, 8 * kNumSM), 256, 0, h->stream>>>(h->n, h->r, seed, h->relabeled ? h->iperm : nullptr, X);
    KLAUNCH(h);
    CUDA_TRY(h, cudaGetLastError());
    comm_mark_full(h, mat_id);
    if (mat_id == SDPLRP_MAT_R) { h->CR_valid = false; h->ls_valid = false; }
    if (mat_id == SDPLRP_MAT_D) { h->CD_valid = false; h->ls_valid = false; }
    if (mat_id == SDPLRP_MAT_G) h->gram_g_valid = false;
    return SDPLRP_OK;
}

int32_t sdplrp_iterate(sdplrp_handle *h, int64_t k, double alpha_max, int32_t use_armijo, int32_t update_history, double out[5]) {
    if (!h) return SDPLRP_ERR_ARG;
    if (!h->preprocessed || h->r <= 0) return fail(h, SDPLRP_ERR_STATE, "iterate: no problem / rank set");
    if (k < 0 || !out) return fail(h, SDPLRP_ERR_ARG, "iterate: bad argument");
    double L_val = 0.0, alpha = 0.0, sg[3] = {0.0, 0.0, 0.0};
    for (int64_t i = 0; i < k; i++) {
        SDP_CHECK(inner_iteration(h, use_armijo != 0, alpha_max, &L_val, &alpha, sg));
        if (update_history && h->hist > 0) SDP_CHECK(sdplrp_lbfgs_update(h, alpha));
    }
    out[0] = L_val; out[1] = sg[0]; out[2] = sg[1]; out[3] = sg[2]; out[4] = alpha;
    return SDPLRP_OK;
}

int32_t sdplrp_solve(sdplrp_handle *h, const sdplrp_config *cfgp, int64_t r0, const double *Rt0, const double *lambda0, double normb,
                     double normC, sdplrp_result *res, double *best_lambda) {
    if (!h) return SDPLRP_ERR_ARG;
    if (!h->preprocessed) return fail(h, SDPLRP_ERR_STATE, "solve: sdplrp_preprocess / sdplrp_set_problem first");
    if (!cfgp || !res || r0 < 1) return fail(h, SDPLRP_ERR_ARG, "solve: bad argument");
    const sdplrp_config &cfg = *cfgp;
    Driver drv{h, cfg};
    const i64 n = h->n, m = h->m;
    const double t_start = now_s();
    double lastprint = t_start, dual_time = 0.0;
    const int hist = (int)cfg.numlbfgsvecs;

    auto init_point = [&](i64 r, const double *R_in, const double *lam_in) -> int32_t {
        SDP_CHECK(sdplrp_set_rank(h, (int32_t)r, hist));
        if (R_in) SDP_CHECK(sdplrp_upload_mat(h, SDPLRP_MAT_R, R_in));
        else SDP_CHECK(sdplrp_fill_uniform(h, SDPLRP_MAT_R, drv.next_seed()));
        std::vector<double> lam((size_t)std::max<i64>(m, 1), 0.0);
        if (lam_in) for (i64 i = 0; i < m; i++) lam[(size_t)i] = lam_in[i];
        if (h->has_ineq) {
            std::vector<double> ub((size_t)std::max<i64>(m, 1));
            SDP_CHECK(sdplrp_download_vec(h, SDPLRP_VEC_LAMBDA_UB, ub.data(), m));
            for (i64 i = 0; i < m; i++) lam[(size_t)i] = std::min(lam[(size_t)i], ub[(size_t)i]);
        }
        SDP_CHECK(sdplrp_upload_vec(h, SDPLRP_VEC_LAMBDA, lam.data(), m));
        return sdplrp_set_sigma(h, cfg.sigma_0);
    };
    i64 r = r0;
    SDP_CHECK(init_point(r, Rt0, lambda0));

    const double gscale = cfg.gtol_relative ? normC : 1.0, pscale = cfg.ptol_relative ? normb : 1.0;
    double sigma = h->sigma;
    double cur_gtol = std::max(1.0 / sigma, cfg.gtol), cur_ptol = std::max(1.0 / pow(sigma, 0.1), cfg.ptol);
    double fg[4];
    SDP_CHECK(sdplrp_fg(h, fg));
    double L_val = fg[0], obj = fg[1], grad_norm = sqrt(fg[2]) / gscale, pvio_norm = sqrt(fg[3]) / pscale;

    i64 it = 0, majoriter = 0, lanczos_steps = 0;
    const bool use_armijo = h->has_ineq;
    i64 rankupd_cnt = cfg.rankupd_tol;
    double duality_gap = 1e20, min_gap = 1e20, max_dual = -1e20;
    if (best_lambda) {
        SDP_CHECK(sdplrp_download_vec(h, SDPLRP_VEC_LAMBDA, best_lambda, m));
        best_lambda[m] = 0.0;
    }
    std::vector<double> ybuf;
    bool stop = false, out_of_budget = false;

    for (i64 major = 0; major < cfg.maxmajoriter; major++) {
        majoriter++;
        i64 localiter = 0;
        while (grad_norm > cur_gtol) {
            localiter++; it++;
            const double lastval = L_val;
            double alpha = 0.0, sg[3];
            SDP_CHECK(inner_iteration(h, use_armijo, cfg.alpha_max, &L_val, &alpha, sg));
            obj = sg[0]; grad_norm = sqrt(sg[1]) / gscale; pvio_norm = sqrt(sg[2]) / pscale;
            const double rel_delta = (lastval - L_val) / std::max(1.0, std::max(fabs(L_val), fabs(lastval)));
            if (rel_delta < cfg.fprec * kEps) break;
            if (hist > 0) SDP_CHECK(sdplrp_lbfgs_update(h, alpha));
            if (it > cfg.maxiter) { out_of_budget = true; break; }
            if ((it & 15) == 0 || h->world <= 1) {
                const double now = now_s();
                if (now - lastprint >= cfg.printfreq) {
                    lastprint = now;
                    if (cfg.printlevel > 0 && h->rank == 0)
                        print_row(cfg, majoriter, localiter, it, L_val, obj, h->sigma, cur_gtol, cur_ptol, grad_norm, pvio_norm, min_gap, max_dual);
                }
                bool over = false;
                SDP_CHECK(agree(h, now - t_start > cfg.maxtime, &over));
                if (over) { out_of_budget = true; break; }
            }
        }
        if (cfg.printlevel > 0 && h->rank == 0)
            print_row(cfg, majoriter, localiter, it, L_val, obj, h->sigma, cur_gtol, cur_ptol, grad_norm, pvio_norm, min_gap, max_dual);
        lastprint = now_s();
        {
            bool over = false;
            SDP_CHECK(agree(h, out_of_budget || lastprint - t_start > cfg.maxtime || it > cfg.maxiter, &over));
            if (over) break;
        }

        bool rank_double = false;
        sigma = h->sigma;
        if (pvio_norm <= cur_ptol) {
            const double t0 = now_s();
            double dual_value = 0.0, mineig = 0.0;
            int64_t steps = 0;
            if (cfg.eigval_highprecision) SDP_CHECK(sdplrp_dual_obj_highprecision(h, cfg.prior_trace_bound, nullptr, drv.next_seed(), &dual_value, &mineig, &steps));
            else SDP_CHECK(sdplrp_dual_obj(h, cfg.prior_trace_bound, it, nullptr, drv.next_seed(), &dual_value, &mineig, &steps));
            lanczos_steps += steps;
            if (dual_value > max_dual) {
                if (best_lambda) {
                    SDP_CHECK(sdplrp_download_vec(h, SDPLRP_VEC_Y, best_lambda, m + 1));
                    for (i64 i = 0; i <= m; i++) best_lambda[i] = -best_lambda[i];
                }
                max_dual = dual_value;
            }
            duality_gap = cfg.objtol_relative ? (obj - max_dual) / std::min(fabs(obj), fabs(max_dual)) : obj - max_dual;
            dual_time += now_s() - t0;
            if (pvio_norm <= cfg.ptol) {
                if (std::isinf(cfg.objtol) && cfg.objtol > 0) stop = true;
                else if (duality_gap <= cfg.objtol) { min_gap = std::min(min_gap, duality_gap); stop = true; }
                else {
                    if (min_gap - duality_gap < cfg.objtol) rankupd_cnt--;
                    else rankupd_cnt = cfg.rankupd_tol;
                    min_gap = std::min(min_gap, duality_gap);
                    if (rankupd_cnt == 0) rank_double = true;
                }
            }
            if (stop) break;
            SDP_CHECK(sdplrp_dual_update(h));
            cur_ptol = cur_ptol / pow(sigma, 0.9);
            cur_gtol = cur_gtol / sigma;
        } else {
            sigma *= cfg.sigmafac;
            SDP_CHECK(sdplrp_set_sigma(h, sigma));
            cur_ptol = 1.0 / pow(sigma, 0.1);
            cur_gtol = 1.0 / sigma;
        }

        if (rank_double) {
            const i64 bp = std::min<i64>(n, (i64)floor(sqrt(2.0 * (double)m) + 1.0));
            r = std::min<i64>(bp, 2 * r);
            SDP_CHECK(init_point(r, nullptr, nullptr));
            sigma = cfg.sigma_0;
            cur_ptol = 1.0 / pow(sigma, 0.1);
            cur_gtol = 1.0 / sigma;
            min_gap = 1e20; max_dual = -1e20; rankupd_cnt = cfg.rankupd_tol;
        } else {
            SDP_CHECK(sdplrp_lbfgs_clear(h));
        }
        cur_ptol = std::max(cur_ptol, cfg.ptol);
        cur_gtol = std::max(cur_gtol, cfg.gtol);
        SDP_CHECK(sdplrp_fg(h, fg));
        L_val = fg[0]; obj = fg[1]; grad_norm = sqrt(fg[2]) / gscale; pvio_norm = sqrt(fg[3]) / pscale;
    }

    SDP_CHECK(sdplrp_fg(h, fg));
    L_val = fg[0]; obj = fg[1]; grad_norm = sqrt(fg[2]) / gscale; pvio_norm = sqrt(fg[3]) / pscale;
    const double t_end = now_s();
    res->sigma = h->sigma; res->grad_norm = grad_norm; res->primal_vio = pvio_norm; res->obj = obj; res->L = L_val;
    res->max_dual_value = max_dual; res->min_duality_gap = min_gap;
    res->totaltime = t_end - t_start; res->dual_time = dual_time; res->primaltime = res->totaltime - dual_time;
    res->iter = it; res->majoriter = majoriter; res->lanczos_steps = lanczos_steps; res->r = r;
    res->status = stop ? 0 : 1;
    for (int k = 0; k < 6; k++) res->DIMACS_errs[k] = 0.0;
    res->DIMACS_time = 0.0;
    if (cfg.eval_DIMACS_errs) {
        const double t0 = now_s();
        SDP_CHECK(sdplrp_dimacs_errors(h, normb, normC, nullptr, drv.next_seed(), res->DIMACS_errs));
        res->DIMACS_time = now_s() - t0;
    }
    return SDPLRP_OK;
}

}
```

### sdplrplus.jl_b200/csrc/gradient.cu

```cuda
#include <algorithm>
#include "common.cuh"

namespace {

constexpr int TPB = 256;

__device__ __forceinline__ unsigned long long pol_evict_last() {
    unsigned long long p;
    asm volatile("createpolicy.fractional.L2::evict_last.b64 %0, 1.0;" : "=l"(p));
    return p;
}
__device__ __forceinline__ unsigned long long pol_evict_first() {
    unsigned long long p;
    asm volatile("createpolicy.fractional.L2::evict_first.b64 %0, 1.0;" : "=l"(p));
    return p;
}
__device__ __forceinline__ int ldg_i32_hint(const int *p, unsigned long long pol) {
    int v;
    asm volatile("ld.global.nc.L2::cache_hint.b32 %0, [%1], %2;" : "=r"(v) : "l"(p), "l"(pol));
    return v;
}
__device__ __forceinline__ double ldg_f64_hint(const double *p, unsigned long long pol) {
    double v;
    asm volatile("ld.global.nc.L2::cache_hint.f64 %0, [%1], %2;" : "=d"(v) : "l"(p), "l"(pol));
    return v;
}
__device__ __forceinline__ double2 ldg_f64x2_hint(const double *p, unsigned long long pol) {
    double2 v;
    asm volatile("ld.global.nc.L2::cache_hint.v2.f64 {%0, %1}, [%2], %3;" : "=d"(v.x), "=d"(v.y) : "l"(p), "l"(pol));
    return v;
}

__global__ void k_form_y(i64 m, double sigma, const double *__restrict__ lambda, const double *__restrict__ ub,
                         const double *__restrict__ raw, double *__restrict__ y) {
    for (i64 i = blockIdx.x * (i64)blockDim.x + threadIdx.x; i <= m; i += (i64)gridDim.x * blockDim.x) {
        if (i == m) { y[i] = 1.0; continue; }
        y[i] = -fmin(ub[i], lambda[i] - sigma * raw[i]);
    }
}

__global__ void k_S_static(i64 nnzF, double yobj, const double *__restrict__ cfull, double *__restrict__ S) {
    for (i64 k = blockIdx.x * (i64)blockDim.x + threadIdx.x; k < nnzF; k += (i64)gridDim.x * blockDim.x) S[k] = yobj * cfull[k];
}

template <int MODE>
__global__ void k_S_dynamic(i64 nd, double yobj, const int *__restrict__ dyn_slot, const int *__restrict__ dyn_ptr,
                            const int *__restrict__ dyn_nsd_end, const int *__restrict__ dyn_gid, const double *__restrict__ dyn_val,
                            const int *__restrict__ pos_a, const int *__restrict__ pos_b, const double *__restrict__ st,
                            const double *__restrict__ y, double *__restrict__ out) {
    for (i64 d = blockIdx.x * (i64)blockDim.x + threadIdx.x; d < nd; d += (i64)gridDim.x * blockDim.x) {
        double s = 0.0;
        const int jend = (MODE == 2) ? dyn_nsd_end[d] : dyn_ptr[d + 1];
        for (int j = dyn_ptr[d]; j < jend; j++) s += dyn_val[j] * y[dyn_gid[j]];
        if (MODE == 2) { out[d] = s; continue; }
        const int t = dyn_slot[d];
        s += yobj * st[t];
        if (MODE == 1) {
            out[t] = s;
        } else {
            out[pos_a[d]] = s;
            const int pb = pos_b[d];
            if (pb >= 0) out[pb] = s;
        }
    }
}

__global__ void k_scale_copy(i64 len, double a, const double *__restrict__ x, double *__restrict__ y) {
    for (i64 k = blockIdx.x * (i64)blockDim.x + threadIdx.x; k < len; k += (i64)gridDim.x * blockDim.x) y[k] = a * x[k];
}

template <int VEC>
struct Acc;
template <>
struct Acc<1> {
    double v;
    __device__ __forceinline__ void zero() { v = 0.0; }
    __device__ __forceinline__ void fma(double s, const double *p) { v += s * __ldg(p); }
    __device__ __forceinline__ void fma_hint(double s, const double *p, unsigned long long pol) { v += s * ldg_f64_hint(p, pol); }
    __device__ __forceinline__ void shfl_add(int o) { v += __shfl_xor_sync(0xffffffffu, v, o); }
    __device__ __forceinline__ void add_from_lane(const Acc &o, int src) { v += __shfl_sync(0xffffffffu, o.v, src & 31); }
    __device__ __forceinline__ void scale_add(double sc, double a, const double *p) { v = sc * (v + a * __ldg(p)); }
    __device__ __forceinline__ void accumulate_onto(double sc, const double *p) { v = p[0] + sc * v; }
    __device__ __forceinline__ void fma_reg(double s, const Acc &o) { v += s * o.v; }
    __device__ __forceinline__ void add_mem(const double *p) { v += p[0]; }
    __device__ __forceinline__ void scale(double sc) { v *= sc; }
    __device__ __forceinline__ double dot_ld(const double *p) const { return v * __ldg(p); }
    __device__ __forceinline__ double norm2() const { return v * v; }
    __device__ __forceinline__ void store(double *p) const { *p = v; }
    __device__ __forceinline__ void ld(const double *p) { v = __ldg(p); }
    __device__ __forceinline__ void ld_hint(const double *p, unsigned long long pol) { v = ldg_f64_hint(p, pol); }
    __device__ __forceinline__ double dot_reg(const Acc &o) const { return v * o.v; }
    __device__ __forceinline__ void add_reg_first(const Acc &o) { v = o.v + 1.0 * v; }
};
template <>
struct Acc<2> {
    double2 v;
    __device__ __forceinline__ void zero() { v.x = v.y = 0.0; }
    __device__ __forceinline__ void fma(double s, const double *p) {
        const double2 x = ldg2(p);
        v.x += s * x.x; v.y += s * x.y;
    }
    __device__ __forceinline__ void fma_hint(double s, const double *p, unsigned long long pol) {
        const double2 x = ldg_f64x2_hint(p, pol);
        v.x += s * x.x; v.y += s * x.y;
    }
    __device__ __forceinline__ void shfl_add(int o) {
        v.x += __shfl_xor_sync(0xffffffffu, v.x, o);
        v.y += __shfl_xor_sync(0xffffffffu, v.y, o);
    }
    __device__ __forceinline__ void add_from_lane(const Acc &o, int src) {
        v.x += __shfl_sync(0xffffffffu, o.v.x, src & 31);
        v.y += __shfl_sync(0xffffffffu, o.v.y, src & 31);
    }
    __device__ __forceinline__ void scale_add(double sc, double a, const double *p) {
        const double2 x = ldg2(p);
        v.x = sc * (v.x + a * x.x); v.y = sc * (v.y + a * x.y);
    }
    __device__ __forceinline__ void scale(double sc) { v.x *= sc; v.y *= sc; }
    __device__ __forceinline__ void accumulate_onto(double sc, const double *p) {
        const double2 x = *reinterpret_cast<const double2 *>(p);
        v.x = x.x + sc * v.x; v.y = x.y + sc * v.y;
    }
    __device__ __forceinline__ void fma_reg(double s, const Acc &o) { v.x += s * o.v.x; v.y += s * o.v.y; }
    __device__ __forceinline__ void add_mem(const double *p) {
        const double2 x = *reinterpret_cast<const double2 *>(p);
        v.x += x.x; v.y += x.y;
    }
    __device__ __forceinline__ double dot_ld(const double *p) const {
        const double2 x = ldg2(p);
        return v.x * x.x + v.y * x.y;
    }
    __device__ __forceinline__ double norm2() const { return v.x * v.x + v.y * v.y; }
    __device__ __forceinline__ void store(double *p) const { *reinterpret_cast<double2 *>(p) = v; }
    __device__ __forceinline__ void ld(const double *p) { v = ldg2(p); }
    __device__ __forceinline__ void ld_hint(const double *p, unsigned long long pol) { v = ldg_f64x2_hint(p, pol); }
    __device__ __forceinline__ double dot_reg(const Acc &o) const { return v.x * o.v.x + v.y * o.v.y; }
    __device__ __forceinline__ void add_reg_first(const Acc &o) { v.x = o.v.x + 1.0 * v.x; v.y = o.v.y + 1.0 * v.y; }
};

struct RowArgs {
    const int *rows;
    i64 n_rows;
    const int *ptr, *idx;
    const int *beg_arr, *end_arr;
    const double *val;
    const int *src;
    const double *X;
    double *Y;
    int r, G;
    int Gw;
    int G0;
    int hot_rows;
    double scale, yobj;
    const double *ADD, *Z;
    double *partials;
    unsigned *ticket;
    double *out;
    i64 own_lo, own_hi;
    const int *chunk_start, *chunk_end, *chunk_row;
    const int *long_rows, *long_cptr;
    double *scratch;
};

template <int VEC, int MAXU, int EPI>
__device__ __forceinline__ void row_epilogue(const RowArgs &a, i64 i, Acc<VEC> (&acc)[MAXU], int lg, int nv, double &s0, double &s1,
                                             int G) {
#pragma unroll
    for (int u = 0; u < MAXU; u++) {
        const int c = lg + u * G;
        if (c < nv) {
            const size_t off = (size_t)i * a.r + c * VEC;
            if (EPI == 0) {
                acc[u].scale(a.scale);
            } else if (EPI == 3) {
                acc[u].accumulate_onto(a.scale, a.Y + off);
            } else if (EPI == 4) {
                acc[u].accumulate_onto(1.0, a.Y + off);
                s0 += acc[u].dot_ld(a.X + off);
                if (a.Z) {
                    Acc<VEC> t;
                    t.zero(); t.fma(1.0, a.X + off);
                    s1 += t.dot_ld(a.Z + off);
                }
            } else if (EPI == 1) {
                if (a.ADD) acc[u].scale_add(a.scale, a.yobj, a.ADD + off); else acc[u].scale(a.scale);
                s0 += acc[u].norm2();
            } else {
                s0 += acc[u].dot_ld(a.X + off);
                if (a.Z) {
                    Acc<VEC> t;
                    t.zero(); t.fma(1.0, a.X + off);
                    s1 += t.dot_ld(a.Z + off);
                }
            }
            acc[u].store(a.Y + off);
        }
    }
}

template <int EPI>
__device__ __forceinline__ void finish_sums(const RowArgs &a, double s0, double s1) {
    if (EPI == 0 || EPI == 3) return;
    double v[2] = {s0, s1};
    double *out = a.out;
    grid_sum_finalize<2>(v, a.partials, a.ticket, [&](double (&s)[2]) { out[0] = s[0]; out[1] = s[1]; });
}

#define VAL_AT(k) (IND ? __ldg(a.val + __ldg(a.src + (k))) : __ldg(a.val + (k)))

#ifndef SDPLRP_LB_GROUP
#define SDPLRP_LB_GROUP 0
#endif
#ifndef SDPLRP_LB_WARP
#define SDPLRP_LB_WARP 0
#endif
#if SDPLRP_LB_GROUP > 0
#define LB_GROUP __launch_bounds__(TPB, SDPLRP_LB_GROUP)
#else
#define LB_GROUP __launch_bounds__(TPB)
#endif
#if SDPLRP_LB_WARP > 0
#define LB_WARP __launch_bounds__(TPB, SDPLRP_LB_WARP)
#else
#define LB_WARP __launch_bounds__(TPB)
#endif

template <int VEC, int MAXU, bool IND, int EPI, int NB>
__global__ void LB_GROUP k_rows_group(RowArgs a) {
    const int nv = a.r / VEC;
    const int G = a.G0;
    const int gpb = TPB / G;
    const int gib = threadIdx.x / G;
    const int lg = threadIdx.x - gib * G;
    const bool lane_ok = gib < gpb;
    const i64 group = (i64)blockIdx.x * gpb + gib;
    const i64 n_groups = (i64)gridDim.x * gpb;
    const unsigned long long p_hot = pol_evict_last(), p_str = pol_evict_first();
    double s0 = 0.0, s1 = 0.0;
    if (lane_ok)
    for (i64 q = group; q < a.n_rows; q += n_groups) {
        const i64 i = a.rows ? a.rows[q] : q;
        if (i < a.own_lo || i >= a.own_hi) continue;
        const int beg = a.beg_arr ? a.beg_arr[i] : a.ptr[i], end = a.end_arr ? a.end_arr[i] : a.ptr[i + 1];
        Acc<VEC> acc[MAXU];
#pragma unroll
        for (int u = 0; u < MAXU; u++) acc[u].zero();
        for (int k0 = beg; k0 < end; k0 += NB) {
            int cc[NB];
            double vv[NB];
#pragma unroll
            for (int j = 0; j < NB; j++) {
                const bool ok = k0 + j < end;
                cc[j] = ok ? ldg_i32_hint(a.idx + k0 + j, p_str) : 0;
                vv[j] = ok ? (IND ? __ldg(a.val + ldg_i32_hint(a.src + k0 + j, p_str)) : ldg_f64_hint(a.val + k0 + j, p_str)) : 0.0;
            }
#pragma unroll
            for (int u = 0; u < MAXU; u++) {
                const int c = lg + u * G;
                if (c < nv) {
#pragma unroll
                    for (int j = 0; j < NB; j++)
                        if (k0 + j < end) acc[u].fma_hint(vv[j], a.X + (size_t)cc[j] * a.r + c * VEC, cc[j] < a.hot_rows ? p_hot : p_str);
                }
            }
        }
        row_epilogue<VEC, MAXU, EPI>(a, i, acc, lg, nv, s0, s1, G);
    }
    finish_sums<EPI>(a, s0, s1);
}

template <int VEC, int MAXU, bool IND, int EPI, bool CHUNK>
__global__ void LB_WARP k_rows_warp(RowArgs a) {
    const int nv = a.r / VEC;
    const int lane = threadIdx.x & 31;
    const int Gw = a.Gw, ng = 32 / Gw;
    const int grp = lane / Gw, lg = lane - grp * Gw;
    const bool lane_ok = grp < ng;
    const i64 warp = (i64)blockIdx.x * (TPB / 32) + (threadIdx.x >> 5);
    const i64 n_warps = (i64)gridDim.x * (TPB / 32);
    const unsigned long long p_hot = pol_evict_last(), p_str = pol_evict_first();
    double s0 = 0.0, s1 = 0.0;
    for (i64 q = warp; q < a.n_rows; q += n_warps) {
        const i64 i = CHUNK ? a.chunk_row[q] : (a.rows ? a.rows[q] : q);
        if (i < a.own_lo || i >= a.own_hi) continue;
        const int beg = CHUNK ? a.chunk_start[q] : (a.beg_arr ? a.beg_arr[i] : a.ptr[i]);
        const int end = CHUNK ? a.chunk_end[q] : (a.end_arr ? a.end_arr[i] : a.ptr[i + 1]);
        Acc<VEC> acc[MAXU];
#pragma unroll
        for (int u = 0; u < MAXU; u++) acc[u].zero();
        for (int k0 = beg + grp * 4; lane_ok && k0 < end; k0 += ng * 4) {
            int cc[4];
            double vv[4];
#pragma unroll
            for (int j = 0; j < 4; j++) {
                const bool ok = k0 + j < end;
                cc[j] = ok ? ldg_i32_hint(a.idx + k0 + j, p_str) : 0;
                vv[j] = ok ? (IND ? __ldg(a.val + ldg_i32_hint(a.src + k0 + j, p_str)) : ldg_f64_hint(a.val + k0 + j, p_str)) : 0.0;
            }
#pragma unroll
            for (int u = 0; u < MAXU; u++) {
                const int c = lg + u * Gw;
                if (c < nv) {
#pragma unroll
                    for (int j = 0; j < 4; j++)
                        if (k0 + j < end) acc[u].fma_hint(vv[j], a.X + (size_t)cc[j] * a.r + c * VEC, cc[j] < a.hot_rows ? p_hot : p_str);
                }
            }
        }
        if ((Gw & (Gw - 1)) == 0) {
#pragma unroll
            for (int u = 0; u < MAXU; u++)
                for (int o = Gw; o < 32; o <<= 1) acc[u].shfl_add(o);
        } else {
#pragma unroll
            for (int u = 0; u < MAXU; u++) {
                const Acc<VEC> own = acc[u];
                for (int o = 1; o < ng; o++) acc[u].add_from_lane(own, (((lane_ok ? grp : 0) + o) % ng) * Gw + lg);
            }
        }
        if (grp == 0) {
            if (CHUNK) {
#pragma unroll
                for (int u = 0; u < MAXU; u++) {
                    const int c = lg + u * Gw;
                    if (c < nv) acc[u].store(a.scratch + (size_t)q * a.r + c * VEC);
                }
            } else {
                row_epilogue<VEC, MAXU, EPI>(a, i, acc, lg, nv, s0, s1, Gw);
            }
        }
    }
    if (!CHUNK) finish_sums<EPI>(a, s0, s1);
}

template <int VEC, int MAXU, int EPI>
__global__ void __launch_bounds__(TPB) k_rows_combine(RowArgs a) {
    const int nv = a.r / VEC;
    const int lg = threadIdx.x & (a.G - 1);
    const i64 group = ((i64)blockIdx.x * TPB + threadIdx.x) / a.G;
    const i64 n_groups = (i64)gridDim.x * TPB / a.G;
    double s0 = 0.0, s1 = 0.0;
    for (i64 q = group; q < a.n_rows; q += n_groups) {
        const i64 i = a.long_rows[q];
        if (i < a.own_lo || i >= a.own_hi) continue;
        Acc<VEC> acc[MAXU];
#pragma unroll
        for (int u = 0; u < MAXU; u++) acc[u].zero();
        for (int c = a.long_cptr[q]; c < a.long_cptr[q + 1]; c++) {
#pragma unroll
            for (int u = 0; u < MAXU; u++) {
                const int p = lg + u * a.G;
                if (p < nv) acc[u].add_mem(a.scratch + (size_t)c * a.r + p * VEC);
            }
        }
        row_epilogue<VEC, MAXU, EPI>(a, i, acc, lg, nv, s0, s1, a.G);
    }
    finish_sums<EPI>(a, s0, s1);
}

__global__ void k_lr_apply(i64 lo, i64 hi, int r, int s, i64 n, const double *__restrict__ XB, const double *__restrict__ Dg,
                           const double *__restrict__ B, const double *__restrict__ y, int gid, double scale,
                           double *__restrict__ Y) {
    const double coeff = scale * y[gid];
    for (i64 e = lo * r + blockIdx.x * (i64)blockDim.x + threadIdx.x; e < hi * r; e += (i64)gridDim.x * blockDim.x) {
        const i64 j = e / r;
        const int i = (int)(e - j * r);
        double t = 0.0;
        for (int k = 0; k < s; k++) t += XB[k * r + i] * Dg[k] * __ldg(&B[j + k * n]);
        Y[e] += coeff * t;
    }
}

constexpr int SPMV_L = 8;
__global__ void __launch_bounds__(TPB) k_spmv(i64 n, const int *__restrict__ ptr, const int *__restrict__ idx,
                                              const double *__restrict__ S, const double *__restrict__ x,
                                              double *__restrict__ y) {
    const int lg = threadIdx.x & (SPMV_L - 1);
    const i64 warp_global = (i64)blockIdx.x * (TPB / 32) + (threadIdx.x >> 5);
    const i64 n_warps = (i64)gridDim.x * (TPB / 32);
    const int g_in_warp = (threadIdx.x & 31) / SPMV_L;
    constexpr int gpw = 32 / SPMV_L;
    for (i64 base = warp_global * gpw; base < n; base += n_warps * gpw) {
        const i64 i = base + g_in_warp;
        double t = 0.0;
        if (i < n)
            for (int k = ptr[i] + lg; k < ptr[i + 1]; k += SPMV_L) t += __ldg(S + k) * __ldg(x + __ldg(idx + k));
#pragma unroll
        for (int o = SPMV_L >> 1; o > 0; o >>= 1) t += __shfl_xor_sync(0xffffffffu, t, o);
        if (i < n && lg == 0) y[i] = t;
    }
}

__global__ void __launch_bounds__(TPB) k_lr_dot(i64 n, const double *__restrict__ B, const double *__restrict__ x,
                                                double *__restrict__ partials, unsigned *__restrict__ ticket,
                                                double *__restrict__ out) {
    double acc[1] = {0.0};
    for (i64 j = blockIdx.x * (i64)blockDim.x + threadIdx.x; j < n; j += (i64)gridDim.x * blockDim.x) acc[0] += B[j] * x[j];
    grid_sum_finalize<1>(acc, partials, ticket, [&](double (&sv)[1]) { out[0] = sv[0]; });
}
__global__ void k_lr_axpy_vec(i64 n, const double *__restrict__ B, const double *__restrict__ dot, const double *__restrict__ Dg,
                              int k, const double *__restrict__ yv, int gid, double *__restrict__ out) {
    const double t = dot[0] * Dg[k] * yv[gid];
    for (i64 j = blockIdx.x * (i64)blockDim.x + threadIdx.x; j < n; j += (i64)gridDim.x * blockDim.x) out[j] += B[j] * t;
}

__global__ void k_obj_slots(int ncls, const double *__restrict__ sums , double *a_rd_m, double *a_dd_m) {
    double s0 = 0.0, s1 = 0.0;
    for (int c = 0; c < ncls; c++) { s0 += sums[2 * c]; s1 += sums[2 * c + 1]; }
    if (a_dd_m) *a_dd_m = s0;
    if (a_rd_m) *a_rd_m = 2.0 * s1;
}
__global__ void k_sum_slots(int ncls, const double *__restrict__ sums, int stride, double *out) {
    double s = 0.0;
    for (int c = 0; c < ncls; c++) s += sums[stride * c];
    *out = s;
}

template <int VEC>
__global__ void __launch_bounds__(TPB) k_grad_diag(i64 lo, i64 hi, int r, double yobj, const double *__restrict__ CR,
                                                   const double *__restrict__ R, const int *__restrict__ rowc_ptr,
                                                   const double *__restrict__ rowc_val, const double *__restrict__ y,
                                                   const int *__restrict__ dyn_diag,
                                                   const double *__restrict__ dynS, double *__restrict__ G, double *partials,
                                                   unsigned *ticket, double *out) {
    const int nv = r / VEC;
    const i64 total = (hi - lo) * nv;
    double acc[1] = {0.0};
    for (i64 e = blockIdx.x * (i64)blockDim.x + threadIdx.x; e < total; e += (i64)gridDim.x * blockDim.x) {
        const i64 i = lo + e / nv;
        const int c = (int)(e - (i - lo) * nv);
        double d = 0.0;
        for (int p = rowc_ptr[i]; p < rowc_ptr[i + 1]; p++) d += rowc_val[p] * y[p];
        if (dynS) {
            const int dd = dyn_diag[i];
            if (dd >= 0) d += dynS[dd];
        }
        const size_t off = (size_t)i * r + c * VEC;
        Acc<VEC> g;
        g.zero();
        g.fma(d, R + off);
        if (CR) g.scale_add(2.0, yobj, CR + off); else g.scale(2.0);
        acc[0] += g.norm2();
        g.store(G + off);
    }
    grid_sum_finalize<1>(acc, partials, ticket, [&](double (&s)[1]) { out[0] = s[0]; });
}

#ifndef SDPLRP_LB_TAIL
#define SDPLRP_LB_TAIL 0
#endif
#if SDPLRP_LB_TAIL > 0
#define LB_TAIL __launch_bounds__(TPB, SDPLRP_LB_TAIL)
#else
#define LB_TAIL __launch_bounds__(TPB)
#endif
template <int VEC>
__global__ void LB_TAIL k_step_grad(i64 lo, i64 hi, int r, double a, double sigma, double yobj,
                                                   const double *__restrict__ D, double *__restrict__ R,
                                                   const double *__restrict__ CD, double *__restrict__ CR,
                                                   const int *__restrict__ rowc_ptr, const double *__restrict__ rowc_val,
                                                   const double *__restrict__ lambda, const double *__restrict__ ub,
                                                   const double *__restrict__ lb, const double *__restrict__ raw_in,
                                                   double *__restrict__ raw_out, const double *__restrict__ q1v,
                                                   const double *__restrict__ q2v, double *__restrict__ y,
                                                   const int *__restrict__ dyn_diag, const double *__restrict__ dynS,
                                                   double *__restrict__ G, const double *__restrict__ pn2_rest,
                                                   double *partials, unsigned *ticket, double *gn2_out, double *pn2_out) {
    const int nv = r / VEC;
    const i64 total = (hi - lo) * nv;
    double acc[2] = {0.0, 0.0};
    for (i64 e = blockIdx.x * (i64)blockDim.x + threadIdx.x; e < total; e += (i64)gridDim.x * blockDim.x) {
        const i64 i = lo + e / nv;
        const int c = (int)(e - (i - lo) * nv);
        const size_t off = (size_t)i * r + c * VEC;
        Acc<VEC> rr, cr;
        rr.zero(); cr.zero();
        rr.fma(1.0, R + off); rr.fma(a, D + off);
        if (CR) { cr.fma(1.0, CR + off); cr.fma(a, CD + off); }
        double d = 0.0;
        for (int p = rowc_ptr[i]; p < rowc_ptr[i + 1]; p++) {
            const double v = raw_in[p] + a * (a * q2v[p] + q1v[p]);
            const double yp = -fmin(ub[p], lambda[p] - sigma * v);
            d += rowc_val[p] * yp;
            if (c == 0) {
                raw_out[p] = v;
                y[p] = yp;
                const double w = fmax(v, lb[p]);
                acc[1] += w * w;
            }
        }
        if (dynS) {
            const int dd = dyn_diag[i];
            if (dd >= 0) d += dynS[dd];
        }
        rr.store(R + off);
        if (CR) cr.store(CR + off);
        Acc<VEC> g;
        g.zero();
        g.fma_reg(d, rr);
        if (CR) g.fma_reg(yobj, cr);
        g.scale(2.0);
        acc[0] += g.norm2();
        g.store(G + off);
    }
    grid_sum_finalize<2>(acc, partials, ticket, [&](double (&s)[2]) { gn2_out[0] = s[0]; pn2_out[0] = s[1] + pn2_rest[0]; });
}

}

i64 tile_hot_rows(const sdplrp_handle *h) {
    if (h->hot_rows >= 0) return std::min<i64>(h->hot_rows, h->n);
    if (!h->relabeled) return 0;
    if (h->dealt) return h->n;
    return std::min<i64>(h->n, (i64)(48.0 * 1024 * 1024) / (8 * (i64)std::max(1, h->r)));
}

namespace {

int pick_group(int nv) {
    int G = 1;
    while (G < nv && G < 32) G <<= 1;
    return G;
}

struct Csr {
    const int *ptr, *idx;
    const double *val;
    const int *src;
    const RowClasses *cls;
};

static int32_t classes_fork(sdplrp_handle *h) {
    if (!h->class_streams[0]) return SDPLRP_OK;
    CUDA_TRY(h, cudaEventRecord(h->ev_fork, h->stream));
    for (int c = 0; c < 2; c++) CUDA_TRY(h, cudaStreamWaitEvent(h->class_streams[c], h->ev_fork, 0));
    h->fork_open = true;
    return SDPLRP_OK;
}
static int32_t classes_join(sdplrp_handle *h) {
    if (!h->class_streams[0]) return SDPLRP_OK;
    for (int c = 0; c < 2; c++) {
        CUDA_TRY(h, cudaEventRecord(h->ev_join[c], h->class_streams[c]));
        CUDA_TRY(h, cudaStreamWaitEvent(h->stream, h->ev_join[c], 0));
    }
    h->fork_open = false;
    return SDPLRP_OK;
}

template <int VEC, int MAXU, bool IND, int EPI>
int32_t launch_classes(sdplrp_handle *h, RowArgs a, const RowClasses &cls, const TileLayout &longs, double *sums ,
                       bool long_empty = false, int class_mask = 7) {
    const int gpb = TPB / a.G;
    const int gpb0 = TPB / a.G0;
    const int spmm_cap = 16 * kNumSM;
    const bool fork = h->class_streams[0] != nullptr;
    const bool own_fork = fork && !h->fork_open;
    if (own_fork) SDP_CHECK(classes_fork(h));
    for (int c = 0; c < 3; c++) {
        if (!(class_mask & (1 << c))) continue;
        cudaStream_t st = (fork && c > 0) ? h->class_streams[c - 1] : h->stream;
        if (sums) a.out = sums + 2 * c;
        a.partials = h->partials + (size_t)c * 16384;
        a.ticket = h->ticket + c;
        a.rows = cls.list[c];
        a.n_rows = cls.cnt[c];
        if (a.n_rows <= 0) {
            if (sums) CUDA_TRY(h, cudaMemsetAsync(sums + 2 * c, 0, 2 * sizeof(double), st));
            continue;
        }
        if (c == 0) {
            if (h->spmm_unroll >= 8) k_rows_group<VEC, MAXU, IND, EPI, 8><<<grid_for(a.n_rows, gpb0, spmm_cap), TPB, 0, st>>>(a);
            else k_rows_group<VEC, MAXU, IND, EPI, 4><<<grid_for(a.n_rows, gpb0, spmm_cap), TPB, 0, st>>>(a);
        } else if (c == 1) {
            k_rows_warp<VEC, MAXU, IND, EPI, false><<<grid_for(a.n_rows, TPB / 32, spmm_cap), TPB, 0, st>>>(a);
        } else if (long_empty) {
            RowArgs b = a;
            b.beg_arr = a.ptr + 1; b.end_arr = a.ptr + 1;
            k_rows_warp<VEC, MAXU, IND, EPI, false><<<grid_for(b.n_rows, TPB / 32, spmm_cap), TPB, 0, st>>>(b);
        } else {
            const i64 need = longs.n_chunks * (i64)a.r;
            if (h->tile_scratch_len < need) {
                if (fork) CUDA_TRY(h, cudaDeviceSynchronize());
                SDP_CHECK(dev_alloc(h, &h->tile_scratch, need));
                h->tile_scratch_len = need;
            }
            RowArgs b = a;
            b.chunk_start = longs.chunk_start; b.chunk_end = longs.chunk_end; b.chunk_row = longs.chunk_row;
            b.long_rows = longs.long_rows; b.long_cptr = longs.long_cptr; b.scratch = h->tile_scratch;
            b.n_rows = longs.n_chunks;
            k_rows_warp<VEC, MAXU, IND, EPI, true><<<grid_for(b.n_rows, TPB / 32, spmm_cap), TPB, 0, st>>>(b);
            KLAUNCH(h);
            b.n_rows = longs.n_long;
            k_rows_combine<VEC, MAXU, EPI><<<grid_for(b.n_rows, gpb, 4 * kNumSM), TPB, 0, st>>>(b);
        }
        KLAUNCH(h);
    }
    if (own_fork) SDP_CHECK(classes_join(h));
    CUDA_TRY(h, cudaGetLastError());
    return SDPLRP_OK;
}

template <bool IND, int EPI>
int32_t launch_csr(sdplrp_handle *h, RowArgs a, const RowClasses &cls, const TileLayout &longs, double *sums, bool long_empty = false,
                   i64 hot_override = -1, int class_mask = 7) {
    const int r = h->r;
    const bool vec2 = (r % 2 == 0);
    const int nv = vec2 ? r / 2 : r;
    a.r = r;
    a.G = pick_group(nv);
    if (a.own_hi <= 0) {
        a.own_lo = h->row_lo;
        a.own_hi = h->row_hi;
    }
    a.G0 = (nv <= 32 && h->spmm_g0) ? nv : a.G;
    a.hot_rows = (int)(hot_override >= 0 ? hot_override : tile_hot_rows(h));
    const int units = (nv + a.G - 1) / a.G;
    a.Gw = (h->spmm_g0 && nv <= 16 && units == 1) ? nv : a.G;
    if (units > 4) return fail(h, SDPLRP_ERR_ARG, "rank too large for the sparse kernels (r <= 256 even / 128 odd)");
    if (vec2) {
        if (units == 1) return launch_classes<2, 1, IND, EPI>(h, a, cls, longs, sums, long_empty, class_mask);
        return launch_classes<2, 4, IND, EPI>(h, a, cls, longs, sums, long_empty, class_mask);
    }
    if (units == 1) return launch_classes<1, 1, IND, EPI>(h, a, cls, longs, sums, long_empty, class_mask);
    return launch_classes<1, 4, IND, EPI>(h, a, cls, longs, sums, long_empty, class_mask);
}

__global__ void k_row_split(i64 n, const int *__restrict__ ptr, const int *__restrict__ idx, int hub_cols, int *__restrict__ mid) {
    for (i64 i = blockIdx.x * (i64)blockDim.x + threadIdx.x; i < n; i += (i64)gridDim.x * blockDim.x) {
        int lo = ptr[i], hi = ptr[i + 1];
        while (lo < hi) {
            const int m = lo + ((hi - lo) >> 1);
            if (idx[m] < hub_cols) lo = m + 1; else hi = m;
        }
        mid[i] = lo;
    }
}

static i64 phase_hub_cols(const sdplrp_handle *h) {
    if (h->spmm_phases <= 0 || !h->relabeled || h->dealt || h->world > 1 || h->nnzF <= 0) return 0;
    const i64 want = h->spmm_phases == 1 ? (i64)(64.0 * 1024 * 1024) / (8 * (i64)std::max(1, h->r)) : (i64)h->spmm_phases;
    return std::min<i64>(want, h->n);
}
static int32_t ensure_row_mid(sdplrp_handle *h, i64 hub_cols) {
    if (h->row_mid && h->row_mid_cols == hub_cols) return SDPLRP_OK;
    SDP_CHECK(dev_alloc(h, &h->row_mid, h->n));
    k_row_split<<<grid_for(h->n, TPB, 8 * kNumSM), TPB, 0, h->stream>>>(h->n, h->full_ptr, h->full_idx, (int)hub_cols, h->row_mid);
    KLAUNCH(h);
    CUDA_TRY(h, cudaGetLastError());
    h->row_mid_cols = hub_cols;
    return SDPLRP_OK;
}

int32_t add_lowrank(sdplrp_handle *h, const double *X, double *Y, double scale) {
    if (h->lr.empty()) return SDPLRP_OK;
    const int r = h->r;
    SDP_CHECK(lr_scratch(h));
    for (const LowRank &L : h->lr) {
        SDP_CHECK(lr_project(h, L, X, h->lr_tmp));
        k_lr_apply<<<grid_for((h->row_hi - h->row_lo) * r, TPB, kRedBlocks), TPB, 0, h->stream>>>(
            h->row_lo, h->row_hi, r, (int)L.s, h->n, h->lr_tmp, L.dD, L.dB, h->y, (int)L.gid, scale, Y);
        KLAUNCH(h);
    }
    CUDA_TRY(h, cudaGetLastError());
    return SDPLRP_OK;
}

}

int32_t grad_form_y(sdplrp_handle *h) {
    k_form_y<<<grid_for(h->m + 1, TPB, kRedBlocks), TPB, 0, h->stream>>>(h->m, h->sigma, h->lambda, h->lambda_ub, h->pvio_raw, h->y);
    KLAUNCH(h);
    h->y_obj = 1.0;
    h->S_current = false;
    CUDA_TRY(h, cudaGetLastError());
    return SDPLRP_OK;
}

int32_t grad_assemble_S(sdplrp_handle *h) {
    h->S_current = true;
    SDP_CHECK(comm_gather_cvec(h, h->y));
    if (h->nA <= 0) return SDPLRP_OK;
    cudaStream_t st = h->stream;
    const double yobj = (h->obj_mat >= 0) ? h->y_obj : 0.0;
    if (!h->S_static_valid || h->S_static_scale != yobj) {
        if (h->nnzF > 0) {
            k_S_static<<<grid_for(h->nnzF, TPB, 8 * kNumSM), TPB, 0, st>>>(h->nnzF, yobj, h->Cfull, h->S);
            KLAUNCH(h);
        }
        h->S_static_valid = true;
        h->S_static_scale = yobj;
    }
    if (h->n_dyn > 0) {
        k_S_dynamic<0><<<grid_for(h->n_dyn, TPB, 8 * kNumSM), TPB, 0, st>>>(h->n_dyn, yobj, h->dyn_slot, h->dyn_ptr, h->dyn_nsd_end, h->dyn_gid, h->dyn_val,
                                                                           h->dyn_pos_a, h->dyn_pos_b, h->triuS_static, h->y, h->S);
        KLAUNCH(h);
    }
    CUDA_TRY(h, cudaGetLastError());
    return SDPLRP_OK;
}

int32_t grad_triuS(sdplrp_handle *h, double *out) {
    if (h->nnzT <= 0) return SDPLRP_OK;
    cudaStream_t st = h->stream;
    const double yobj = (h->obj_mat >= 0) ? h->y_obj : 0.0;
    k_scale_copy<<<grid_for(h->nnzT, TPB, 8 * kNumSM), TPB, 0, st>>>(h->nnzT, yobj, h->triuS_static, out);
    KLAUNCH(h);
    if (h->n_dyn > 0) {
        k_S_dynamic<1><<<grid_for(h->n_dyn, TPB, 8 * kNumSM), TPB, 0, st>>>(h->n_dyn, yobj, h->dyn_slot, h->dyn_ptr, h->dyn_nsd_end, h->dyn_gid, h->dyn_val,
                                                                           h->dyn_pos_a, h->dyn_pos_b, h->triuS_static, h->y, out);
        KLAUNCH(h);
    }
    CUDA_TRY(h, cudaGetLastError());
    return SDPLRP_OK;
}

int32_t grad_spmm(sdplrp_handle *h, const double *X, double *Y, double scale, bool ) {
    SDP_CHECK(grad_spmm_sparse(h, X, Y, scale));
    return add_lowrank(h, X, Y, scale);
}

int32_t grad_spmm_sparse(sdplrp_handle *h, const double *X, double *Y, double scale) {
    const int r = h->r;
    if (h->nA > 0 && gather_supported(h) && h->nnzF > 0) {
        SDP_CHECK(gather_plan_build(h, h->full_plan, h->full_ptr, h->row_lo, h->row_hi, gather_tile_size(h)));
        SDP_CHECK(gather_spmm(h, h->full_plan, h->full_ptr, h->full_idx, h->S, X, nullptr, nullptr, Y, 0, scale, nullptr));
    } else if (h->nA > 0) {
        RowArgs a = {};
        a.ptr = h->full_ptr; a.idx = h->full_idx; a.val = h->S; a.src = nullptr;
        a.X = X; a.Y = Y; a.scale = scale;
        SDP_CHECK((launch_csr<false, 0>(h, a, h->full_cls, h->full_long, nullptr)));
    } else {
        CUDA_TRY(h, cudaMemsetAsync(Y + h->row_lo * r, 0, (size_t)(h->row_hi - h->row_lo) * r * sizeof(double), h->stream));
    }
    return SDPLRP_OK;
}

static int32_t grad_obj_spmm_halo(sdplrp_handle *h, const double *X, double *Y, const double *Z, double *sums6) {
    const HaloPlan &p = h->halo;
    const size_t off = (size_t)h->row_lo * h->r;
    RowArgs a = {};
    a.ptr = p.lptr; a.idx = p.lidx; a.val = p.lval; a.src = nullptr;
    (void)X;
    a.X = p.xc; a.Y = Y + off; a.Z = Z ? Z + off : nullptr; a.scale = 1.0;
    a.own_lo = 0; a.own_hi = p.nloc;
    CUDA_TRY(h, cudaMemsetAsync(sums6, 0, 6 * sizeof(double), h->stream));
    bool single_sweep = h->halo_mode == 2;
    if (h->halo_mode == 3) {
        const double exch = (double)(p.n_ghost[0] + p.n_ghost[1]) * h->r * 8.0 / 450e9 * 1e3;
        const double sweep = (double)p.lnnz / 39e9 * 1e3;
        const double ls = 0.1 + 2.0 * (double)p.nloc * h->r * 8.0 / 3e12 * 1e3;
        const double hidden = std::min(std::max(0.0, exch - ls - 0.1), 0.58 * 1.27 * sweep);
        const double extra = 0.33 * sweep + 0.1;
        single_sweep = hidden < extra + 0.15;
    }
    if (single_sweep) {
        SDP_CHECK(halo_wait(h, 0));
        SDP_CHECK(halo_wait(h, 1));
        return launch_csr<false, 2>(h, a, p.cls, p.longs, sums6);
    }
    SDP_CHECK(halo_wait(h, 0));
    RowArgs a1 = a;
    a1.end_arr = p.lmid;
    SDP_CHECK((launch_csr<false, 0>(h, a1, p.cls, p.longs, nullptr, false, -1, 3)));
    SDP_CHECK(halo_wait(h, 1));
    RowArgs a2 = a;
    a2.beg_arr = p.lmid;
    SDP_CHECK(classes_fork(h));
    int32_t rc = launch_csr<false, 4>(h, a2, p.cls, p.longs, sums6, false, -1, 3);
    if (rc == SDPLRP_OK) rc = launch_csr<false, 2>(h, a, p.cls, p.longs, sums6, false, -1, 4);
    const int32_t rj = classes_join(h);
    return rc != SDPLRP_OK ? rc : rj;
}

int32_t grad_obj_spmm(sdplrp_handle *h, const double *X, double *Y, const double *Z, double *sums6) {
    if (halo_active(h)) return grad_obj_spmm_halo(h, X, Y, Z, sums6);
    if (gather_supported(h) && h->nnzF > 0) {
        SDP_CHECK(gather_plan_build(h, h->full_plan, h->full_ptr, h->row_lo, h->row_hi, gather_tile_size(h)));
        CUDA_TRY(h, cudaMemsetAsync(sums6 + 4, 0, 2 * sizeof(double), h->stream));
        return gather_spmm(h, h->full_plan, h->full_ptr, h->full_idx, h->Cfull, X, X, Z, Y, 2, 1.0, sums6);
    }
    RowArgs a = {};
    a.ptr = h->full_ptr; a.idx = h->full_idx; a.val = h->Cfull; a.src = nullptr;
    a.X = X; a.Y = Y; a.Z = Z; a.scale = 1.0;
    const i64 hub_cols = phase_hub_cols(h);
    if (hub_cols > 0 && hub_cols < h->n) {
        SDP_CHECK(ensure_row_mid(h, hub_cols));
        a.end_arr = h->row_mid;
        SDP_CHECK((launch_csr<false, 0>(h, a, h->full_cls, h->full_long, nullptr, false, hub_cols)));
        a.beg_arr = h->row_mid; a.end_arr = nullptr;
        return launch_csr<false, 4>(h, a, h->full_cls, h->full_long, sums6, true, hub_cols);
    }
    return launch_csr<false, 2>(h, a, h->full_cls, h->full_long, sums6);
}

int32_t grad_hot(sdplrp_handle *h) {
    cudaStream_t st = h->stream;
    const int r = h->r;
    const bool need_dynS = h->n_dyn > 0 && h->n_dyn_nsd > 0;
    if (need_dynS) {
        k_S_dynamic<2><<<grid_for(h->n_dyn, TPB, 8 * kNumSM), TPB, 0, st>>>(h->n_dyn, 0.0, h->dyn_slot, h->dyn_ptr, h->dyn_nsd_end, h->dyn_gid, h->dyn_val,
                                                                           h->dyn_pos_a, h->dyn_pos_b, h->triuS_static, h->y, h->dynS);
        KLAUNCH(h);
    }
    const bool vec2 = (r % 2 == 0);
    const int nv = vec2 ? r / 2 : r;
    const i64 total = (h->row_hi - h->row_lo) * nv;
    const double *CR = (h->obj_mat >= 0) ? h->CR : nullptr;
    const int grid = grid_for(total, TPB * 2, kRedBlocks);
    if (vec2) k_grad_diag<2><<<grid, TPB, 0, st>>>(h->row_lo, h->row_hi, r, h->y_obj, CR, h->R, h->rowc_ptr, h->rowc_val, h->y, h->dyn_diag, need_dynS ? h->dynS : nullptr, h->G, h->partials, h->ticket, h->dscal + SC_GNORM2);
    else k_grad_diag<1><<<grid, TPB, 0, st>>>(h->row_lo, h->row_hi, r, h->y_obj, CR, h->R, h->rowc_ptr, h->rowc_val, h->y, h->dyn_diag, need_dynS ? h->dynS : nullptr, h->G, h->partials, h->ticket, h->dscal + SC_GNORM2);
    KLAUNCH(h);
    bool renorm = false;
    if (h->n_dynF > 0) {
        RowArgs a = {};
        a.ptr = h->dynrow_ptr; a.idx = h->dynrow_col; a.val = h->dynS; a.src = h->dynrow_src;
        a.X = h->R; a.Y = h->G; a.scale = 2.0;
        SDP_CHECK((launch_csr<true, 3>(h, a, h->dyn_cls, h->dyn_long, nullptr)));
        renorm = true;
    }
    if (!h->lr.empty()) {
        SDP_CHECK(add_lowrank(h, h->R, h->G, 2.0));
        renorm = true;
    }
    if (renorm) SDP_CHECK(lb_norm2(h, h->G, SC_GNORM2));
    CUDA_TRY(h, cudaGetLastError());
    return SDPLRP_OK;
}

int32_t grad_step_fused(sdplrp_handle *h, double alpha) {
    cudaStream_t st = h->stream;
    const int r = h->r;
    const bool split = h->obj_mat >= 0;
    double *raw_in = h->pvio_raw, *raw_out = h->pvio_raw_alt;
    double *pn2_rest = h->dscal + SC_SUMS + 2;
    SDP_CHECK(vec_tail_rest(h, alpha, raw_in, raw_out, pn2_rest));
    h->y_obj = 1.0;
    h->S_current = false;
    const bool need_dynS = h->n_dyn > 0 && h->n_dyn_nsd > 0;
    if (need_dynS) {
        k_S_dynamic<2><<<grid_for(h->n_dyn, TPB, 8 * kNumSM), TPB, 0, st>>>(h->n_dyn, 0.0, h->dyn_slot, h->dyn_ptr, h->dyn_nsd_end, h->dyn_gid, h->dyn_val,
                                                                           h->dyn_pos_a, h->dyn_pos_b, h->triuS_static, h->y, h->dynS);
        KLAUNCH(h);
    }
    const bool vec2 = (r % 2 == 0);
    const int nv = vec2 ? r / 2 : r;
    const i64 total = (h->row_hi - h->row_lo) * nv;
    const int ctas = h->tail_ctas > 0 ? h->tail_ctas : (h->world == 1 ? 6 : 4);
    const int grid = grid_for(total, TPB * 2, ctas * kNumSM);
    const double *CD = split ? h->CD : nullptr;
    double *CR = split ? h->CR : nullptr;
#define SG_ARGS h->row_lo, h->row_hi, r, alpha, h->sigma, h->y_obj, h->D, h->R, CD, CR, h->rowc_ptr, h->rowc_val, h->lambda, h->lambda_ub, \
                h->pvio_lb, raw_in, raw_out, h->A_RD, h->A_DD, h->y, h->dyn_diag, need_dynS ? h->dynS : nullptr, h->G, pn2_rest, h->partials, \
                h->ticket, h->dscal + SC_GNORM2, h->dscal + SC_PNORM2
    if (vec2) k_step_grad<2><<<grid, TPB, 0, st>>>(SG_ARGS);
    else k_step_grad<1><<<grid, TPB, 0, st>>>(SG_ARGS);
#undef SG_ARGS
    KLAUNCH(h);
    std::swap(h->pvio_raw, h->pvio_raw_alt);
    comm_mark_partial(h, SDPLRP_MAT_R);
    comm_mark_partial(h, SDPLRP_MAT_G);
    if (h->n_dynF > 0) SDP_CHECK(comm_require_full(h, SDPLRP_MAT_R));
    bool renorm = false;
    if (h->n_dynF > 0) {
        RowArgs a = {};
        a.ptr = h->dynrow_ptr; a.idx = h->dynrow_col; a.val = h->dynS; a.src = h->dynrow_src;
        a.X = h->R; a.Y = h->G; a.scale = 2.0;
        SDP_CHECK((launch_csr<true, 3>(h, a, h->dyn_cls, h->dyn_long, nullptr)));
        renorm = true;
    }
    if (!h->lr.empty()) {
        SDP_CHECK(add_lowrank(h, h->R, h->G, 2.0));
        renorm = true;
    }
    if (renorm) SDP_CHECK(lb_norm2(h, h->G, SC_GNORM2));
    SDP_CHECK(comm_reduce_scalars(h, SC_GNORM2, 2));
    CUDA_TRY(h, cudaGetLastError());
    return SDPLRP_OK;
}

int32_t grad_obj_slots(sdplrp_handle *h, const double *sums6, double *a_rd_m, double *a_dd_m) {
    k_obj_slots<<<1, 1, 0, h->stream>>>(3, sums6, a_rd_m, a_dd_m);
    KLAUNCH(h);
    CUDA_TRY(h, cudaGetLastError());
    return SDPLRP_OK;
}

int32_t grad_spmv(sdplrp_handle *h, const double *x, double *y, i64 ncols) {
    cudaStream_t st = h->stream;
    const i64 n = h->n;
    for (i64 q = 0; q < ncols; q++) {
        const double *xq = x + q * n;
        double *yq = y + q * n;
        if (h->nA > 0) {
            k_spmv<<<grid_for(n, TPB / SPMV_L, 16 * kNumSM), TPB, 0, st>>>(n, h->full_ptr, h->full_idx, h->S, xq, yq);
            KLAUNCH(h);
        } else {
            CUDA_TRY(h, cudaMemsetAsync(yq, 0, (size_t)n * sizeof(double), st));
        }
        for (const LowRank &L : h->lr) {
            for (i64 k = 0; k < L.s; k++) {
                k_lr_dot<<<kRedBlocks, TPB, 0, st>>>(n, L.dB + k * n, xq, h->partials, h->ticket, h->dscal + SC_LANCZOS + 8);
                KLAUNCH(h);
                k_lr_axpy_vec<<<grid_for(n, TPB, kRedBlocks), TPB, 0, st>>>(n, L.dB + k * n, h->dscal + SC_LANCZOS + 8, L.dD, (int)k, h->y, (int)L.gid, yq);
                KLAUNCH(h);
            }
        }
    }
    CUDA_TRY(h, cudaGetLastError());
    return SDPLRP_OK;
}
```

### sdplrplus.jl_b200/csrc/lbfgs.cu

```cuda
#include <algorithm>
#include "common.cuh"

namespace {

constexpr int TPB = kRedThreads;

template <int VEC>
struct V;
template <>
struct V<1> {
    typedef double T;
    static __device__ __forceinline__ T ld(const double *p, i64 i) { return p[i]; }
    static __device__ __forceinline__ void st(double *p, i64 i, T v) { p[i] = v; }
    static __device__ __forceinline__ T axpy(double a, T x, T y) { return y + a * x; }
    static __device__ __forceinline__ T neg(T x) { return -x; }
    static __device__ __forceinline__ T scale(double a, T x) { return a * x; }
    static __device__ __forceinline__ double dot(T a, T b) { return a * b; }
};
template <>
struct V<2> {
    typedef double2 T;
    static __device__ __forceinline__ T ld(const double *p, i64 i) { return reinterpret_cast<const double2 *>(p)[i]; }
    static __device__ __forceinline__ void st(double *p, i64 i, T v) { reinterpret_cast<double2 *>(p)[i] = v; }
    static __device__ __forceinline__ T axpy(double a, T x, T y) { return make_double2(y.x + a * x.x, y.y + a * x.y); }
    static __device__ __forceinline__ T neg(T x) { return make_double2(-x.x, -x.y); }
    static __device__ __forceinline__ T scale(double a, T x) { return make_double2(a * x.x, a * x.y); }
    static __device__ __forceinline__ double dot(T a, T b) { return a.x * b.x + a.y * b.y; }
};

#define GRID_STRIDE(i, nu) for (i64 i = blockIdx.x * (i64)blockDim.x + threadIdx.x; i < (nu); i += (i64)gridDim.x * blockDim.x)

template <int VEC>
__global__ void __launch_bounds__(TPB) k_dot(i64 nu, const double *__restrict__ x, const double *__restrict__ y, double *partials,
                                             unsigned *ticket, double *out) {
    double acc[1] = {0.0};
    GRID_STRIDE(i, nu) acc[0] += V<VEC>::dot(V<VEC>::ld(x, i), V<VEC>::ld(y, i));
    grid_sum_finalize<1>(acc, partials, ticket, [&](double (&s)[1]) { out[0] = s[0]; });
}

template <int VEC, int PHASE>
__global__ void __launch_bounds__(TPB) k_two_loop(i64 nu, const double *in, const double *__restrict__ w,
                                                  const double *z, double *out, const double *__restrict__ rho_j,
                                                  double *a_j, const double *__restrict__ dot_in, double *dot_out,
                                                  const double *grad, double *ypre, double *partials, unsigned *ticket) {
    double coef;
    if (PHASE == 1) {
        const double a = rho_j[0] * dot_in[0];
        coef = -a;
        if (blockIdx.x == 0 && threadIdx.x == 0) a_j[0] = a;
    } else {
        coef = a_j[0] - rho_j[0] * dot_in[0];
    }
    double acc[1] = {0.0};
    GRID_STRIDE(i, nu) {
        typename V<VEC>::T d = V<VEC>::axpy(coef, V<VEC>::ld(w, i), V<VEC>::ld(in, i));
        if (PHASE == 3) {
            d = V<VEC>::neg(d);
            typename V<VEC>::T g = V<VEC>::ld(grad, i);
            V<VEC>::st(ypre, i, V<VEC>::neg(g));
            acc[0] += V<VEC>::dot(d, g);
        } else {
            acc[0] += V<VEC>::dot(V<VEC>::ld(z, i), d);
        }
        V<VEC>::st(out, i, d);
    }
    grid_sum_finalize<1>(acc, partials, ticket, [&](double (&s)[1]) { dot_out[0] = s[0]; });
}

template <int VEC>
__global__ void __launch_bounds__(TPB) k_copy_dir(i64 nu, const double *__restrict__ grad, double *__restrict__ dir,
                                                 double *partials, unsigned *ticket, double *dot_out) {
    double acc[1] = {0.0};
    GRID_STRIDE(i, nu) {
        typename V<VEC>::T g = V<VEC>::ld(grad, i);
        V<VEC>::st(dir, i, g);
        acc[0] += V<VEC>::dot(g, g);
    }
    grid_sum_finalize<1>(acc, partials, ticket, [&](double (&s)[1]) { dot_out[0] = s[0]; });
}

template <int VEC>
__global__ void __launch_bounds__(TPB) k_update(i64 nu, double alpha, const double *__restrict__ dir,
                                                const double *__restrict__ grad, double *__restrict__ sj,
                                                double *__restrict__ yj, double *partials, unsigned *ticket, double *rho_j) {
    double acc[1] = {0.0};
    GRID_STRIDE(i, nu) {
        typename V<VEC>::T s = V<VEC>::scale(alpha, V<VEC>::ld(dir, i));
        typename V<VEC>::T y = V<VEC>::axpy(1.0, V<VEC>::ld(grad, i), V<VEC>::ld(yj, i));
        V<VEC>::st(sj, i, s);
        V<VEC>::st(yj, i, y);
        acc[0] += V<VEC>::dot(y, s);
    }
    grid_sum_finalize<1>(acc, partials, ticket, [&](double (&s)[1]) { rho_j[0] = s[0]; });
}
__global__ void k_invert(double *x) { x[0] = 1.0 / x[0]; }

template <int VEC>
__global__ void __launch_bounds__(TPB) k_axpy(i64 nu, double a, const double *__restrict__ x, double *__restrict__ y) {
    GRID_STRIDE(i, nu) V<VEC>::st(y, i, V<VEC>::axpy(a, V<VEC>::ld(x, i), V<VEC>::ld(y, i)));
}

template <int VEC>
__global__ void __launch_bounds__(TPB) k_axpy2(i64 nu, double a, const double *__restrict__ x1, double *__restrict__ y1,
                                               const double *__restrict__ x2, double *__restrict__ y2) {
    GRID_STRIDE(i, nu) {
        V<VEC>::st(y1, i, V<VEC>::axpy(a, V<VEC>::ld(x1, i), V<VEC>::ld(y1, i)));
        V<VEC>::st(y2, i, V<VEC>::axpy(a, V<VEC>::ld(x2, i), V<VEC>::ld(y2, i)));
    }
}

template <int VEC>
__global__ void __launch_bounds__(TPB) k_neg_copy(i64 nu, double *__restrict__ g, double *__restrict__ d) {
    GRID_STRIDE(i, nu) {
        typename V<VEC>::T v = V<VEC>::neg(V<VEC>::ld(g, i));
        V<VEC>::st(g, i, v);
        V<VEC>::st(d, i, v);
    }
}

template <int VEC>
__global__ void __launch_bounds__(TPB) k_norm2(i64 nu, const double *__restrict__ x, double *partials, unsigned *ticket, double *out) {
    double acc[1] = {0.0};
    GRID_STRIDE(i, nu) {
        typename V<VEC>::T v = V<VEC>::ld(x, i);
        acc[0] += V<VEC>::dot(v, v);
    }
    grid_sum_finalize<1>(acc, partials, ticket, [&](double (&s)[1]) { out[0] = s[0]; });
}

template <int VEC>
__global__ void __launch_bounds__(TPB) k_dot2(i64 nu, const double *__restrict__ x, const double *__restrict__ y, double *partials,
                                              unsigned *ticket, double *out) {
    double acc[1] = {0.0};
    GRID_STRIDE(i, nu) acc[0] += V<VEC>::dot(V<VEC>::ld(x, i), V<VEC>::ld(y, i));
    grid_sum_finalize<1>(acc, partials, ticket, [&](double (&s)[1]) { out[0] = s[0]; });
}

constexpr int kGramMaxHist = 8;
constexpr int kGramNB = 2 * kGramMaxHist + 1;
struct LbPtrs {
    const double *S[kGramMaxHist];
    const double *Y[kGramMaxHist];
};

template <int VEC, int M, bool UPDATE>
__global__ void __launch_bounds__(TPB) k_gram_pass(i64 nu, double alpha, LbPtrs P, const double *__restrict__ G,
                                                   const double *__restrict__ D, double *Sj_out, double *Yj_out,
                                                   int p0, int p1, int p2, double *partials, unsigned *ticket, double *out) {
    constexpr int NB = 2 * M + 1;
    double acc[3 * NB];
#pragma unroll
    for (int k = 0; k < 3 * NB; k++) acc[k] = 0.0;
    GRID_STRIDE(i, nu) {
        typename V<VEC>::T b[NB];
#pragma unroll
        for (int k = 0; k < M; k++) {
            b[k] = (UPDATE && k == M - 1) ? V<VEC>::ld(D, i) : V<VEC>::ld(P.S[k], i);
            b[M + k] = V<VEC>::ld(P.Y[k], i);
        }
        b[2 * M] = V<VEC>::ld(G, i);
        typename V<VEC>::T pv[3];
        if (UPDATE) {
            b[M - 1] = V<VEC>::scale(alpha, b[M - 1]);
            b[2 * M - 1] = V<VEC>::axpy(1.0, b[2 * M], b[2 * M - 1]);
            V<VEC>::st(Sj_out, i, b[M - 1]);
            V<VEC>::st(Yj_out, i, b[2 * M - 1]);
            pv[0] = b[M - 1]; pv[1] = b[2 * M - 1]; pv[2] = b[2 * M];
        } else {
            const int probe[3] = {p0, p1, p2};
#pragma unroll
            for (int p = 0; p < 3; p++) {
                pv[p] = b[0];
#pragma unroll
                for (int k = 1; k < NB; k++)
                    if (k == probe[p]) pv[p] = b[k];
            }
        }
#pragma unroll
        for (int p = 0; p < 3; p++) {
#pragma unroll
            for (int k = 0; k < NB; k++) acc[p * NB + k] += V<VEC>::dot(pv[p], b[k]);
        }
    }
    grid_sum_finalize<3 * NB>(acc, partials, ticket, [&](double (&sv)[3 * NB]) {
#pragma unroll
        for (int k = 0; k < 3 * NB; k++) out[k] = sv[k];
    });
}

__global__ void k_gram_commit(int M, int rot, int p0, int p1, int p2, const double *__restrict__ tmp, double *__restrict__ gram,
                              int upd_j, double *__restrict__ rho) {
    const int NB = 2 * M + 1;
    const int probe[3] = {p0, p1, p2};
    auto true_index = [&](int b) { return b < M ? (rot + b) % M : (b < 2 * M ? M + (rot + b - M) % M : 2 * M); };
    for (int p = 0; p < 3; p++) {
        if (probe[p] < 0) continue;
        const int tp = true_index(probe[p]);
        for (int k = threadIdx.x; k < NB; k += blockDim.x) {
            const double v = tmp[p * NB + k];
            const int tk = true_index(k);
            gram[tp * NB + tk] = v;
            gram[tk * NB + tp] = v;
        }
    }
    __syncthreads();
    if (threadIdx.x == 0 && upd_j >= 0) rho[upd_j] = 1.0 / gram[(M + upd_j) * NB + upd_j];
}

__global__ void k_gram_coef(int M, int latest, const double *__restrict__ gram, const double *__restrict__ rho,
                            double *__restrict__ coef) {
    if (threadIdx.x != 0) return;
    const int NB = 2 * M + 1;
    double c[kGramNB], a[kGramMaxHist];
    for (int k = 0; k < NB; k++) c[k] = 0.0;
    c[2 * M] = 1.0;
    int order[kGramMaxHist];
    {
        int j = latest;
        for (int q = 0; q < M; q++) { order[q] = j - 1; j -= 1; if (j == 0) j = M; }
    }
    for (int q = 0; q < M; q++) {
        const int j = order[q];
        double sd = 0.0;
        for (int k = 0; k < NB; k++) sd += c[k] * gram[j * NB + k];
        a[j] = rho[j] * sd;
        c[M + j] -= a[j];
    }
    for (int q = M - 1; q >= 0; q--) {
        const int j = order[q];
        double yd = 0.0;
        for (int k = 0; k < NB; k++) yd += c[k] * gram[(M + j) * NB + k];
        c[j] += a[j] - rho[j] * yd;
    }
    for (int k = 0; k < NB; k++) coef[k] = c[k];
}

template <int VEC, int M>
__global__ void __launch_bounds__(TPB) k_gram_form(i64 nu, LbPtrs P, const double *__restrict__ G, const double *__restrict__ coef,
                                                   double *dir, double *ypre, int jpre,
                                                   double *partials, unsigned *ticket, double *dot_out) {
    constexpr int NB = 2 * M + 1;
    double c[NB];
#pragma unroll
    for (int k = 0; k < NB; k++) c[k] = coef[k];
    double acc[1] = {0.0};
    GRID_STRIDE(i, nu) {
        const typename V<VEC>::T g = V<VEC>::ld(G, i);
        typename V<VEC>::T d = V<VEC>::scale(c[2 * M], g);
#pragma unroll
        for (int k = 0; k < M; k++) {
            d = V<VEC>::axpy(c[k], V<VEC>::ld(P.S[k], i), d);
            d = V<VEC>::axpy(c[M + k], V<VEC>::ld(P.Y[k], i), d);
        }
        d = V<VEC>::neg(d);
        V<VEC>::st(dir, i, d);
        V<VEC>::st(ypre, i, V<VEC>::neg(g));
        acc[0] += V<VEC>::dot(d, g);
    }
    grid_sum_finalize<1>(acc, partials, ticket, [&](double (&sv)[1]) { dot_out[0] = sv[0]; });
}

struct Slice {
    i64 off, len, nu;
    int vec;
    int grid;
};
Slice owned(const sdplrp_handle *h) {
    Slice s;
    s.off = h->row_lo * h->r;
    s.len = (h->row_hi - h->row_lo) * h->r;
    s.vec = (s.off % 2 == 0 && s.len % 2 == 0) ? 2 : 1;
    s.nu = s.len / s.vec;
    s.grid = grid_for(s.nu, TPB * 4, kRedBlocks);
    return s;
}

#define DISPATCH_VEC(sl, KERNEL, ...)                                              \
    do {                                                                           \
        if ((sl).vec == 2) KERNEL<2><<<(sl).grid, TPB, 0, h->stream>>>(__VA_ARGS__); \
        else KERNEL<1><<<(sl).grid, TPB, 0, h->stream>>>(__VA_ARGS__);             \
        KLAUNCH(h);                                                                \
    } while (0)

template <int PHASE>
void launch_two_loop(sdplrp_handle *h, const Slice &sl, const double *in, const double *w, const double *z, double *out,
                     const double *rho_j, double *a_j, const double *dot_in, double *dot_out, const double *grad, double *ypre) {
    if (sl.vec == 2)
        k_two_loop<2, PHASE><<<sl.grid, TPB, 0, h->stream>>>(sl.nu, in, w, z, out, rho_j, a_j, dot_in, dot_out, grad, ypre, h->partials, h->ticket);
    else
        k_two_loop<1, PHASE><<<sl.grid, TPB, 0, h->stream>>>(sl.nu, in, w, z, out, rho_j, a_j, dot_in, dot_out, grad, ypre, h->partials, h->ticket);
    KLAUNCH(h);
}


bool gram_enabled(const sdplrp_handle *h) { return h->lbfgs_kernel == 1 && h->hist >= 1 && h->hist <= kGramMaxHist; }

LbPtrs gram_ptrs(const sdplrp_handle *h, i64 off, int rot = 0) {
    LbPtrs P = {};
    for (int q = 0; q < h->hist; q++) {
        const int k = (rot + q) % h->hist;
        P.S[q] = h->Sh[k] + off; P.Y[q] = h->Yh[k] + off;
    }
    return P;
}

template <int M>
int32_t gram_pass_m(sdplrp_handle *h, const Slice &sl, bool update, double alpha, int j, int p0, int p1, int p2) {
    const int rot = update ? (j + 1) % M : 0;
    if (update) { p0 = M - 1; p1 = 2 * M - 1; p2 = 2 * M; }
    const LbPtrs P = gram_ptrs(h, sl.off, rot);
    const double *G = h->G + sl.off, *D = h->D + sl.off;
    double *Sj = update ? h->Sh[j] + sl.off : nullptr, *Yj = update ? h->Yh[j] + sl.off : nullptr;
    double *tmp = h->lb_small + kGramNB * kGramNB;
#define GP_LAUNCH(VECN, UPD) k_gram_pass<VECN, M, UPD><<<sl.grid, TPB, 0, h->stream>>>(sl.nu, alpha, P, G, D, Sj, Yj, p0, p1, p2, h->partials, h->ticket, tmp)
    if (sl.vec == 2) { if (update) GP_LAUNCH(2, true); else GP_LAUNCH(2, false); }
    else { if (update) GP_LAUNCH(1, true); else GP_LAUNCH(1, false); }
#undef GP_LAUNCH
    KLAUNCH(h);
    CUDA_TRY(h, cudaGetLastError());
    SDP_CHECK(comm_reduce_ptr(h, tmp, 3 * (2 * M + 1)));
    k_gram_commit<<<1, 32, 0, h->stream>>>(M, rot, p0, p1, p2, tmp, h->lb_small, update ? j : -1, h->dscal + SC_RHO);
    KLAUNCH(h);
    return SDPLRP_OK;
}
int32_t gram_pass(sdplrp_handle *h, const Slice &sl, bool update, double alpha, int j, int p0, int p1, int p2) {
    switch (h->hist) {
    case 1: return gram_pass_m<1>(h, sl, update, alpha, j, p0, p1, p2);
    case 2: return gram_pass_m<2>(h, sl, update, alpha, j, p0, p1, p2);
    case 3: return gram_pass_m<3>(h, sl, update, alpha, j, p0, p1, p2);
    case 4: return gram_pass_m<4>(h, sl, update, alpha, j, p0, p1, p2);
    case 5: return gram_pass_m<5>(h, sl, update, alpha, j, p0, p1, p2);
    case 6: return gram_pass_m<6>(h, sl, update, alpha, j, p0, p1, p2);
    case 7: return gram_pass_m<7>(h, sl, update, alpha, j, p0, p1, p2);
    default: return gram_pass_m<8>(h, sl, update, alpha, j, p0, p1, p2);
    }
}

template <int M>
int32_t gram_form_m(sdplrp_handle *h, const Slice &sl, int jpre) {
    const LbPtrs P = gram_ptrs(h, sl.off);
    const double *coef = h->lb_small + kGramNB * kGramNB + 3 * kGramNB;
    if (sl.vec == 2)
        k_gram_form<2, M><<<sl.grid, TPB, 0, h->stream>>>(sl.nu, P, h->G + sl.off, coef, h->D + sl.off, h->Yh[jpre] + sl.off, jpre,
                                                          h->partials, h->ticket, h->dscal + SC_DESCENT);
    else
        k_gram_form<1, M><<<sl.grid, TPB, 0, h->stream>>>(sl.nu, P, h->G + sl.off, coef, h->D + sl.off, h->Yh[jpre] + sl.off, jpre,
                                                          h->partials, h->ticket, h->dscal + SC_DESCENT);
    KLAUNCH(h);
    CUDA_TRY(h, cudaGetLastError());
    return SDPLRP_OK;
}
int32_t gram_form(sdplrp_handle *h, const Slice &sl, int jpre) {
    switch (h->hist) {
    case 1: return gram_form_m<1>(h, sl, jpre);
    case 2: return gram_form_m<2>(h, sl, jpre);
    case 3: return gram_form_m<3>(h, sl, jpre);
    case 4: return gram_form_m<4>(h, sl, jpre);
    case 5: return gram_form_m<5>(h, sl, jpre);
    case 6: return gram_form_m<6>(h, sl, jpre);
    case 7: return gram_form_m<7>(h, sl, jpre);
    default: return gram_form_m<8>(h, sl, jpre);
    }
}

int32_t gram_refresh(sdplrp_handle *h, const Slice &sl) {
    const int M = h->hist, NB = 2 * M + 1;
    if (!h->gram_pairs_valid) {
        for (int p = 0; p < NB - 1; p += 3)
            SDP_CHECK(gram_pass(h, sl, false, 0.0, -1, p, p + 1 < NB - 1 ? p + 1 : -1, p + 2 < NB - 1 ? p + 2 : -1));
        h->gram_pairs_valid = true;
    }
    if (!h->gram_g_valid) {
        SDP_CHECK(gram_pass(h, sl, false, 0.0, -1, 2 * M, -1, -1));
        h->gram_g_valid = true;
    }
    return SDPLRP_OK;
}

int32_t lb_dir_gram(sdplrp_handle *h) {
    const Slice sl = owned(h);
    const int M = h->hist;
    SDP_CHECK(gram_refresh(h, sl));
    double *coef = h->lb_small + kGramNB * kGramNB + 3 * kGramNB;
    k_gram_coef<<<1, 32, 0, h->stream>>>(M, h->latest, h->lb_small, h->dscal + SC_RHO, coef);
    KLAUNCH(h);
    const int jpre = h->latest % M;
    SDP_CHECK(gram_form(h, sl, jpre));
    SDP_CHECK(comm_reduce_ptr(h, h->dscal + SC_DESCENT, 1));
    h->gram_pairs_valid = false;
    h->gram_prestored = jpre;
    return SDPLRP_OK;
}

int32_t lb_update_gram(sdplrp_handle *h, double alpha) {
    const Slice sl = owned(h);
    const int M = h->hist;
    const int j = h->latest % M;
    if (!h->gram_pairs_valid && h->gram_prestored != j) {
        for (int p = 0; p < 2 * M; p++) {
            if (p == j || p == M + j) continue;
            SDP_CHECK(gram_pass(h, sl, false, 0.0, -1, p, -1, -1));
        }
    }
    SDP_CHECK(gram_pass(h, sl, true, alpha, j, j, M + j, 2 * M));
    h->gram_pairs_valid = true; h->gram_g_valid = true; h->gram_prestored = -1;
    h->latest = j + 1;
    return SDPLRP_OK;
}

}

int32_t lb_dir(sdplrp_handle *h) {
    const Slice sl = owned(h);
    const int m = h->hist;
    const double *grad = h->G + sl.off;
    double *dir = h->D + sl.off;
    double *descent = h->dscal + SC_DESCENT;
    if (m == 0) {
        DISPATCH_VEC(sl, k_copy_dir, sl.nu, grad, dir, h->partials, h->ticket, descent);
        CUDA_TRY(h, cudaGetLastError());
        return comm_reduce_ptr(h, descent, 1);
    }
    if (gram_enabled(h)) return lb_dir_gram(h);
    int order[kMaxHist];
    {
        int j = h->latest;
        for (int q = 0; q < m; q++) { order[q] = j - 1; j -= 1; if (j == 0) j = m; }
    }
    double *dotA = h->dscal + SC_DOT, *dotB = h->dscal + SC_DOT + 6;
    DISPATCH_VEC(sl, k_dot, sl.nu, h->Sh[order[0]] + sl.off, grad, h->partials, h->ticket, dotA);
    SDP_CHECK(comm_reduce_ptr(h, dotA, 1));
    double *din = dotA, *dout = dotB;
    for (int q = 0; q < m; q++) {
        const int j = order[q];
        const double *in = (q == 0) ? grad : dir;
        const double *w = h->Yh[j] + sl.off;
        const double *z = (q + 1 < m) ? h->Sh[order[q + 1]] + sl.off : h->Yh[order[m - 1]] + sl.off;
        launch_two_loop<1>(h, sl, in, w, z, dir, h->dscal + SC_RHO + j, h->dscal + SC_A + j, din, dout, nullptr, nullptr);
        SDP_CHECK(comm_reduce_ptr(h, dout, 1));
        std::swap(din, dout);
    }
    const int jpre = h->latest % m;
    for (int q = m - 1; q >= 0; q--) {
        const int j = order[q];
        const double *w = h->Sh[j] + sl.off;
        if (q > 0) {
            const double *z = h->Yh[order[q - 1]] + sl.off;
            launch_two_loop<2>(h, sl, dir, w, z, dir, h->dscal + SC_RHO + j, h->dscal + SC_A + j, din, dout, nullptr, nullptr);
            SDP_CHECK(comm_reduce_ptr(h, dout, 1));
            std::swap(din, dout);
        } else {
            launch_two_loop<3>(h, sl, dir, w, nullptr, dir, h->dscal + SC_RHO + j, h->dscal + SC_A + j, din, descent, grad,
                               h->Yh[jpre] + sl.off);
            SDP_CHECK(comm_reduce_ptr(h, descent, 1));
        }
    }
    CUDA_TRY(h, cudaGetLastError());
    return SDPLRP_OK;
}

int32_t lb_update(sdplrp_handle *h, double alpha) {
    const int m = h->hist;
    if (m == 0) return SDPLRP_OK;
    if (gram_enabled(h)) return lb_update_gram(h, alpha);
    const Slice sl = owned(h);
    const int j = h->latest % m;
    DISPATCH_VEC(sl, k_update, sl.nu, alpha, h->D + sl.off, h->G + sl.off, h->Sh[j] + sl.off, h->Yh[j] + sl.off, h->partials,
                 h->ticket, h->dscal + SC_RHO + j);
    SDP_CHECK(comm_reduce_ptr(h, h->dscal + SC_RHO + j, 1));
    k_invert<<<1, 1, 0, h->stream>>>(h->dscal + SC_RHO + j);
    KLAUNCH(h);
    h->latest = j + 1;
    CUDA_TRY(h, cudaGetLastError());
    return SDPLRP_OK;
}

int32_t lb_clear(sdplrp_handle *h) {
    const size_t bytes = (size_t)h->n * h->r * sizeof(double);
    for (int j = 0; j < h->hist; j++) {
        CUDA_TRY(h, cudaMemsetAsync(h->Sh[j], 0, bytes, h->stream));
        CUDA_TRY(h, cudaMemsetAsync(h->Yh[j], 0, bytes, h->stream));
    }
    CUDA_TRY(h, cudaMemsetAsync(h->dscal + SC_RHO, 0, kMaxHist * sizeof(double), h->stream));
    CUDA_TRY(h, cudaMemsetAsync(h->dscal + SC_A, 0, kMaxHist * sizeof(double), h->stream));
    if (h->lb_small) CUDA_TRY(h, cudaMemsetAsync(h->lb_small, 0, (size_t)kLbSmallLen * sizeof(double), h->stream));
    h->gram_pairs_valid = true;
    h->gram_g_valid = true;
    h->gram_prestored = -1;
    return SDPLRP_OK;
}

int32_t lb_axpy(sdplrp_handle *h, double alpha, const double *x, double *y) {
    const Slice sl = owned(h);
    DISPATCH_VEC(sl, k_axpy, sl.nu, alpha, x + sl.off, y + sl.off);
    CUDA_TRY(h, cudaGetLastError());
    return SDPLRP_OK;
}

int32_t lb_axpy2(sdplrp_handle *h, double alpha, const double *x1, double *y1, const double *x2, double *y2) {
    const Slice sl = owned(h);
    DISPATCH_VEC(sl, k_axpy2, sl.nu, alpha, x1 + sl.off, y1 + sl.off, x2 + sl.off, y2 + sl.off);
    CUDA_TRY(h, cudaGetLastError());
    return SDPLRP_OK;
}

int32_t lb_neg_copy(sdplrp_handle *h) {
    const Slice sl = owned(h);
    DISPATCH_VEC(sl, k_neg_copy, sl.nu, h->G + sl.off, h->D + sl.off);
    CUDA_TRY(h, cudaGetLastError());
    return SDPLRP_OK;
}

int32_t lb_dot(sdplrp_handle *h, const double *x, const double *y, int slot) {
    const Slice sl = owned(h);
    DISPATCH_VEC(sl, k_dot2, sl.nu, x + sl.off, y + sl.off, h->partials, h->ticket, h->dscal + slot);
    CUDA_TRY(h, cudaGetLastError());
    return SDPLRP_OK;
}

int32_t lb_norm2(sdplrp_handle *h, const double *x, int slot) {
    const Slice sl = owned(h);
    DISPATCH_VEC(sl, k_norm2, sl.nu, x + sl.off, h->partials, h->ticket, h->dscal + slot);
    CUDA_TRY(h, cudaGetLastError());
    return SDPLRP_OK;
}
```

Before: 121.9.

## Store L-BFGS history implicitly via pointer rotation and lazy step scaling

Makes the direction buffer D alias the next history slot S_j, and keeps the previous gradient G_k in its own buffer by ping-ponging G between two allocations. The update pass therefore no longer writes S_j or reads D, and the alpha scale is applied on the fly through per-slot scale factors. Y_j is formed from G minus G_k. This cuts full n*r vector reads and writes from the gram update and form kernels, removing the ypre store. In exchange it adds extra memcpy and scale launches on some transitions, plus more complex aliasing state handled in the API upload, download and operand paths.

```diff
diff --git a/sdplrplus.jl_b200/csrc/api.cu b/sdplrplus.jl_b200/csrc/api.cu
--- a/sdplrplus.jl_b200/csrc/api.cu
+++ b/sdplrplus.jl_b200/csrc/api.cu
@@ -56,6 +56,22 @@
     if (id >= SDPLRP_MAT_S0 && id < SDPLRP_MAT_S0 + h->hist) return h->Sh[id - SDPLRP_MAT_S0];
     if (id >= SDPLRP_MAT_Y0 && id < SDPLRP_MAT_Y0 + h->hist) return h->Yh[id - SDPLRP_MAT_Y0];
     return nullptr;
+}
+
+static double *write_ptr(sdplrp_handle *h, int id) {
+    if (id == SDPLRP_MAT_G) return lb_g_target(h);
+    if (id == SDPLRP_MAT_D) return lb_d_target(h);
+    return mat_ptr(h, id);
+}
+
+static double *operand_ptr(sdplrp_handle *h, int id) {
+    if (lb_slot_scale(h, id) != 1.0) return nullptr;
+    return mat_ptr(h, id);
+}
+
+static void scale_host(double *x, i64 len, double a) {
+    if (a == 1.0) return;
+    for (i64 i = 0; i < len; i++) x[i] = a * x[i];
 }
 
 static double *vec_ptr(sdplrp_handle *h, int id, i64 *len) {
@@ -163,7 +179,8 @@
 }
 
 static void free_state(sdplrp_handle *h) {
-    dev_free(&h->R); dev_free(&h->G); dev_free(&h->D); dev_free(&h->W0); dev_free(&h->W1);
+    dev_free(&h->R); dev_free(&h->G_mem); dev_free(&h->D_mem); dev_free(&h->W0); dev_free(&h->W1);
+    h->G = h->D = nullptr; h->G_k = nullptr;
     dev_free(&h->CR); dev_free(&h->CD);
     h->CR_valid = h->CD_valid = false;
     for (int j = 0; j < kMaxHist; j++) { dev_free(&h->Sh[j]); dev_free(&h->Yh[j]); }
@@ -342,7 +359,7 @@
     if (r < 1 || numlbfgsvecs < 0 || numlbfgsvecs > kMaxHist) return fail(h, SDPLRP_ERR_ARG, "set_rank: bad rank / history length");
     CUDA_TRY(h, cudaSetDevice(h->device));
     const i64 N = mat_capacity(h, r);
-    const bool reuse = h->R && h->G && h->D && h->lb_small && h->r == r && h->hist == numlbfgsvecs && h->state_cap == N &&
+    const bool reuse = h->R && h->G_mem && h->D_mem && h->lb_small && h->r == r && h->hist == numlbfgsvecs && h->state_cap == N &&
                        ((h->obj_mat >= 0) == (h->CR != nullptr)) && ((h->obj_mat >= 0) == (h->CD != nullptr));
     if (reuse) {
         h->CR_valid = h->CD_valid = false;
@@ -350,13 +367,14 @@
         if (h->W1) CUDA_TRY(h, cudaMemsetAsync(h->W1, 0, (size_t)N * 8, h->stream));
     } else {
         free_state(h);
-        SDP_CHECK(dev_alloc(h, &h->R, N)); SDP_CHECK(dev_alloc(h, &h->G, N)); SDP_CHECK(dev_alloc(h, &h->D, N));
+        SDP_CHECK(dev_alloc(h, &h->R, N)); SDP_CHECK(dev_alloc(h, &h->G_mem, N)); SDP_CHECK(dev_alloc(h, &h->D_mem, N));
         if (h->obj_mat >= 0) { SDP_CHECK(dev_alloc(h, &h->CR, N)); SDP_CHECK(dev_alloc(h, &h->CD, N)); }
         for (int j = 0; j < numlbfgsvecs; j++) { SDP_CHECK(dev_alloc(h, &h->Sh[j], N)); SDP_CHECK(dev_alloc(h, &h->Yh[j], N)); }
         SDP_CHECK(dev_alloc(h, &h->lb_small, kLbSmallLen));
         h->state_cap = N;
     }
     h->r = r; h->hist = numlbfgsvecs; h->latest = numlbfgsvecs;
+    SDP_CHECK(lb_layout_reset(h, false));
     CUDA_TRY(h, cudaMemsetAsync(h->R, 0, (size_t)N * 8, h->stream));
     CUDA_TRY(h, cudaMemsetAsync(h->G, 0, (size_t)N * 8, h->stream));
     CUDA_TRY(h, cudaMemsetAsync(h->D, 0, (size_t)N * 8, h->stream));
@@ -385,7 +403,11 @@
     if (k == "gather_warps") { h->gather_warps = (int)value; return SDPLRP_OK; }
     if (k == "gather_hints") { h->gather_hints = value > 0 ? 1 : 0; return SDPLRP_OK; }
     if (k == "fused_tail") { h->fused_tail = value != 0; return SDPLRP_OK; }
-    if (k == "lbfgs_kernel") { h->lbfgs_kernel = (int)value; h->gram_pairs_valid = h->gram_g_valid = false; return SDPLRP_OK; }
+    if (k == "lbfgs_kernel") {
+        h->lbfgs_kernel = (int)value;
+        if (h->lb_small) CUDA_TRY(h, cudaSetDevice(h->device));
+        return lb_layout_reset(h, true);
+    }
     return fail(h, SDPLRP_ERR_ARG, "set_option: unknown key " + k);
 }
 
@@ -411,8 +433,9 @@
     CUDA_TRY(h, cudaSetDevice(h->device));
     SDP_CHECK(lazy_scratch(h, id));
     if (id == SDPLRP_MAT_CR || id == SDPLRP_MAT_CD) return fail(h, SDPLRP_ERR_ARG, "upload_mat: CR / CD are download-only");
-    double *p = mat_ptr(h, id);
+    double *p = write_ptr(h, id);
     if (!p || !src) return fail(h, SDPLRP_ERR_ARG, "upload_mat: bad id");
+    SDP_CHECK(lb_slot_written(h, id));
     SDP_CHECK(perm_upload(h, p, src, h->r, true));
     comm_mark_full(h, id);
     if (id == SDPLRP_MAT_R) h->CR_valid = false;
@@ -430,8 +453,9 @@
     CUDA_TRY(h, cudaSetDevice(h->device));
     SDP_CHECK(lazy_scratch(h, id));
     if (id == SDPLRP_MAT_CR || id == SDPLRP_MAT_CD) return fail(h, SDPLRP_ERR_ARG, "upload_mat: CR / CD are download-only");
-    double *p = mat_ptr(h, id);
+    double *p = write_ptr(h, id);
     if (!p || !src) return fail(h, SDPLRP_ERR_ARG, "upload_mat_slice: bad id");
+    SDP_CHECK(lb_slot_written(h, id));
     SDP_CHECK(perm_upload_slice(h, p, src, h->r));
     comm_mark_full(h, id);
     if (id == SDPLRP_MAT_R) { h->CR_valid = false; h->ls_valid = false; }
@@ -450,7 +474,10 @@
     double *p = mat_ptr(h, id);
     if (!p || !dst) return fail(h, SDPLRP_ERR_ARG, "download_mat_slice: bad id");
     SDP_CHECK(comm_gather_rows(h, p, id));
-    return perm_download_slice(h, p, dst, h->r);
+    SDP_CHECK(perm_download_slice(h, p, dst, h->r));
+    const i64 S = (h->n + h->world - 1) / h->world, lo = std::min<i64>(h->n, (i64)h->rank * S), hi = std::min<i64>(h->n, lo + S);
+    scale_host(dst + lo * h->r, (hi - lo) * h->r, lb_slot_scale(h, id));
+    return SDPLRP_OK;
 }
 
 int32_t sdplrp_download_mat(sdplrp_handle *h, int32_t id, double *dst) {
@@ -461,7 +488,9 @@
     double *p = mat_ptr(h, id);
     if (!p || !dst) return fail(h, SDPLRP_ERR_ARG, "download_mat: bad id");
     SDP_CHECK(comm_gather_rows(h, p, id));
-    return perm_download(h, p, dst, h->r, true);
+    SDP_CHECK(perm_download(h, p, dst, h->r, true));
+    scale_host(dst, h->n * h->r, lb_slot_scale(h, id));
+    return SDPLRP_OK;
 }
 
 int32_t sdplrp_upload_vec(sdplrp_handle *h, int32_t id, const double *src, int64_t len) {
@@ -516,7 +545,7 @@
     REQUIRE_H(h); REQUIRE_PRE(h); REQUIRE_RANK(h);
     CUDA_TRY(h, cudaSetDevice(h->device));
     SDP_CHECK(lazy_scratch(h, U_id));
-    const double *U = mat_ptr(h, U_id);
+    const double *U = operand_ptr(h, U_id);
     if (!U) return fail(h, SDPLRP_ERR_ARG, "A_uu: bad matrix id");
     SDP_CHECK(comm_require_full(h, U_id));
     SDP_CHECK(aop_uu(h, U, h->A_out));
@@ -528,7 +557,7 @@
     REQUIRE_H(h); REQUIRE_PRE(h); REQUIRE_RANK(h);
     CUDA_TRY(h, cudaSetDevice(h->device));
     SDP_CHECK(lazy_scratch(h, U_id)); SDP_CHECK(lazy_scratch(h, V_id));
-    const double *U = mat_ptr(h, U_id), *V = mat_ptr(h, V_id);
+    const double *U = operand_ptr(h, U_id), *V = operand_ptr(h, V_id);
     if (!U || !V) return fail(h, SDPLRP_ERR_ARG, "A_uv: bad matrix id");
     SDP_CHECK(comm_require_full(h, U_id)); SDP_CHECK(comm_require_full(h, V_id));
     SDP_CHECK(aop_uv(h, U, V, h->A_out));
@@ -550,9 +579,11 @@
     REQUIRE_H(h); REQUIRE_PRE(h); REQUIRE_RANK(h);
     CUDA_TRY(h, cudaSetDevice(h->device));
     SDP_CHECK(lazy_scratch(h, X_id)); SDP_CHECK(lazy_scratch(h, Y_id));
+    if (X_id == Y_id || !operand_ptr(h, X_id) || !operand_ptr(h, Y_id)) return fail(h, SDPLRP_ERR_ARG, "At_left: bad matrix ids");
+    SDP_CHECK(lb_slot_written(h, Y_id));
+    double *Y = write_ptr(h, Y_id);
     const double *X = mat_ptr(h, X_id);
-    double *Y = mat_ptr(h, Y_id);
-    if (!X || !Y || X == Y) return fail(h, SDPLRP_ERR_ARG, "At_left: bad matrix ids");
+    if (X == Y) return fail(h, SDPLRP_ERR_ARG, "At_left: bad matrix ids");
     SDP_CHECK(comm_require_full(h, X_id));
     if (!h->S_current) SDP_CHECK(grad_assemble_S(h));
     SDP_CHECK(grad_spmm(h, X, Y, 1.0, false));
@@ -612,6 +643,7 @@
 
 static int32_t do_g(sdplrp_handle *h) {
     if (h->obj_mat >= 0 && !h->CR_valid) SDP_CHECK(rebuild_CR(h));
+    lb_g_target(h);
     if (needs_remote_R_rows(h)) SDP_CHECK(comm_require_full(h, SDPLRP_MAT_R));
     {
         SectionScope sc(h, SDPLRP_SEC_S_ASSEMBLE);
@@ -684,6 +716,7 @@
     h->gram_g_valid = false;
     h->CD_valid = false; h->ls_valid = false;
     comm_mark_partial(h, SDPLRP_MAT_D);
+    comm_mark_partial(h, SDPLRP_MAT_G);
     return SDPLRP_OK;
 }
 
diff --git a/sdplrplus.jl_b200/csrc/common.cuh b/sdplrplus.jl_b200/csrc/common.cuh
--- a/sdplrplus.jl_b200/csrc/common.cuh
+++ b/sdplrplus.jl_b200/csrc/common.cuh
@@ -196,6 +196,10 @@
     double *lb_small = nullptr;
     bool gram_pairs_valid = false, gram_g_valid = false;
     int gram_prestored = -1;
+    double *G_mem = nullptr, *D_mem = nullptr;
+    bool lb_implicit = false;
+    double lb_alpha[kMaxHist] = {0.0};
+    double *G_k = nullptr;
 
     double *dscal = nullptr;
     double *hscal = nullptr;
@@ -364,6 +368,11 @@
 int32_t lb_axpy(sdplrp_handle *h, double alpha, const double *x, double *y);
 int32_t lb_axpy2(sdplrp_handle *h, double alpha, const double *x1, double *y1, const double *x2, double *y2);
 int32_t lb_neg_copy(sdplrp_handle *h);
+double *lb_g_target(sdplrp_handle *h);
+double *lb_d_target(sdplrp_handle *h);
+int32_t lb_layout_reset(sdplrp_handle *h, bool keep);
+int32_t lb_slot_written(sdplrp_handle *h, int id);
+double lb_slot_scale(const sdplrp_handle *h, int id);
 int32_t lb_norm2(sdplrp_handle *h, const double *x, int slot);
 int32_t lb_dot(sdplrp_handle *h, const double *x, const double *y, int slot);
 
diff --git a/sdplrplus.jl_b200/csrc/driver.cu b/sdplrplus.jl_b200/csrc/driver.cu
--- a/sdplrplus.jl_b200/csrc/driver.cu
+++ b/sdplrplus.jl_b200/csrc/driver.cu
@@ -183,7 +183,7 @@
 int32_t sdplrp_fill_uniform(sdplrp_handle *h, int32_t mat_id, uint64_t seed) {
     if (!h) return SDPLRP_ERR_ARG;
     if (!h->preprocessed || h->r <= 0) return fail(h, SDPLRP_ERR_STATE, "fill_uniform: call sdplrp_set_rank first");
-    double *X = mat_id == SDPLRP_MAT_R ? h->R : mat_id == SDPLRP_MAT_G ? h->G : mat_id == SDPLRP_MAT_D ? h->D : nullptr;
+    double *X = mat_id == SDPLRP_MAT_R ? h->R : mat_id == SDPLRP_MAT_G ? lb_g_target(h) : mat_id == SDPLRP_MAT_D ? lb_d_target(h) : nullptr;
     if (!X) return fail(h, SDPLRP_ERR_ARG, "fill_uniform: R, G or D only");
     CUDA_TRY(h, cudaSetDevice(h->device));
     k_fill_uniform<<<grid_for(h->n * h->r, 256, 8 * kNumSM), 256, 0, h->stream>>>(h->n, h->r, seed, h->relabeled ? h->iperm : nullptr, X);
diff --git a/sdplrplus.jl_b200/csrc/gradient.cu b/sdplrplus.jl_b200/csrc/gradient.cu
--- a/sdplrplus.jl_b200/csrc/gradient.cu
+++ b/sdplrplus.jl_b200/csrc/gradient.cu
@@ -831,6 +831,7 @@
     cudaStream_t st = h->stream;
     const int r = h->r;
     const bool split = h->obj_mat >= 0;
+    lb_g_target(h);
     double *raw_in = h->pvio_raw, *raw_out = h->pvio_raw_alt;
     double *pn2_rest = h->dscal + SC_SUMS + 2;
     SDP_CHECK(vec_tail_rest(h, alpha, raw_in, raw_out, pn2_rest));
diff --git a/sdplrplus.jl_b200/csrc/lbfgs.cu b/sdplrplus.jl_b200/csrc/lbfgs.cu
--- a/sdplrplus.jl_b200/csrc/lbfgs.cu
+++ b/sdplrplus.jl_b200/csrc/lbfgs.cu
@@ -110,11 +110,25 @@
 }
 
 template <int VEC>
-__global__ void __launch_bounds__(TPB) k_neg_copy(i64 nu, double *__restrict__ g, double *__restrict__ d) {
-    GRID_STRIDE(i, nu) {
-        typename V<VEC>::T v = V<VEC>::neg(V<VEC>::ld(g, i));
-        V<VEC>::st(g, i, v);
+__global__ void __launch_bounds__(TPB) k_neg_copy(i64 nu, const double *gin, double *gout, double *__restrict__ d) {
+    GRID_STRIDE(i, nu) {
+        typename V<VEC>::T v = V<VEC>::neg(V<VEC>::ld(gin, i));
+        V<VEC>::st(gout, i, v);
         V<VEC>::st(d, i, v);
+    }
+}
+
+template <int VEC>
+__global__ void __launch_bounds__(TPB) k_scale_inplace(i64 nu, double a, double *__restrict__ x) {
+    GRID_STRIDE(i, nu) V<VEC>::st(x, i, V<VEC>::scale(a, V<VEC>::ld(x, i)));
+}
+
+template <int VEC>
+__global__ void __launch_bounds__(TPB) k_swap(i64 nu, double *__restrict__ x, double *__restrict__ y) {
+    GRID_STRIDE(i, nu) {
+        const typename V<VEC>::T a = V<VEC>::ld(x, i), b = V<VEC>::ld(y, i);
+        V<VEC>::st(x, i, b);
+        V<VEC>::st(y, i, a);
     }
 }
 
@@ -141,11 +155,15 @@
 struct LbPtrs {
     const double *S[kGramMaxHist];
     const double *Y[kGramMaxHist];
+    double a[kGramMaxHist];
 };
+
+template <int VEC>
+__device__ __forceinline__ typename V<VEC>::T ld_s(const LbPtrs &P, int q, i64 i) { return V<VEC>::scale(P.a[q], V<VEC>::ld(P.S[q], i)); }
 
 template <int VEC, int M, bool UPDATE>
 __global__ void __launch_bounds__(TPB) k_gram_pass(i64 nu, double alpha, LbPtrs P, const double *__restrict__ G,
-                                                   const double *__restrict__ D, double *Sj_out, double *Yj_out,
+                                                   const double *Gk, double *Yj_out,
                                                    int p0, int p1, int p2, double *partials, unsigned *ticket, double *out) {
     constexpr int NB = 2 * M + 1;
     double acc[3 * NB];
@@ -155,15 +173,13 @@
         typename V<VEC>::T b[NB];
 #pragma unroll
         for (int k = 0; k < M; k++) {
-            b[k] = (UPDATE && k == M - 1) ? V<VEC>::ld(D, i) : V<VEC>::ld(P.S[k], i);
-            b[M + k] = V<VEC>::ld(P.Y[k], i);
+            b[k] = (UPDATE && k == M - 1) ? V<VEC>::scale(alpha, V<VEC>::ld(P.S[k], i)) : ld_s<VEC>(P, k, i);
+            b[M + k] = (UPDATE && k == M - 1) ? V<VEC>::ld(Gk, i) : V<VEC>::ld(P.Y[k], i);
         }
         b[2 * M] = V<VEC>::ld(G, i);
         typename V<VEC>::T pv[3];
         if (UPDATE) {
-            b[M - 1] = V<VEC>::scale(alpha, b[M - 1]);
-            b[2 * M - 1] = V<VEC>::axpy(1.0, b[2 * M], b[2 * M - 1]);
-            V<VEC>::st(Sj_out, i, b[M - 1]);
+            b[2 * M - 1] = V<VEC>::axpy(-1.0, b[2 * M - 1], b[2 * M]);
             V<VEC>::st(Yj_out, i, b[2 * M - 1]);
             pv[0] = b[M - 1]; pv[1] = b[2 * M - 1]; pv[2] = b[2 * M];
         } else {
@@ -237,8 +253,7 @@
 
 template <int VEC, int M>
 __global__ void __launch_bounds__(TPB) k_gram_form(i64 nu, LbPtrs P, const double *__restrict__ G, const double *__restrict__ coef,
-                                                   double *dir, double *ypre, int jpre,
-                                                   double *partials, unsigned *ticket, double *dot_out) {
+                                                   double *dir, double *partials, unsigned *ticket, double *dot_out) {
     constexpr int NB = 2 * M + 1;
     double c[NB];
 #pragma unroll
@@ -249,12 +264,11 @@
         typename V<VEC>::T d = V<VEC>::scale(c[2 * M], g);
 #pragma unroll
         for (int k = 0; k < M; k++) {
-            d = V<VEC>::axpy(c[k], V<VEC>::ld(P.S[k], i), d);
+            d = V<VEC>::axpy(c[k], ld_s<VEC>(P, k, i), d);
             d = V<VEC>::axpy(c[M + k], V<VEC>::ld(P.Y[k], i), d);
         }
         d = V<VEC>::neg(d);
         V<VEC>::st(dir, i, d);
-        V<VEC>::st(ypre, i, V<VEC>::neg(g));
         acc[0] += V<VEC>::dot(d, g);
     }
     grid_sum_finalize<1>(acc, partials, ticket, [&](double (&sv)[1]) { dot_out[0] = sv[0]; });
@@ -299,7 +313,7 @@
     LbPtrs P = {};
     for (int q = 0; q < h->hist; q++) {
         const int k = (rot + q) % h->hist;
-        P.S[q] = h->Sh[k] + off; P.Y[q] = h->Yh[k] + off;
+        P.S[q] = h->Sh[k] + off; P.Y[q] = h->Yh[k] + off; P.a[q] = h->lb_alpha[k];
     }
     return P;
 }
@@ -309,10 +323,11 @@
     const int rot = update ? (j + 1) % M : 0;
     if (update) { p0 = M - 1; p1 = 2 * M - 1; p2 = 2 * M; }
     const LbPtrs P = gram_ptrs(h, sl.off, rot);
-    const double *G = h->G + sl.off, *D = h->D + sl.off;
-    double *Sj = update ? h->Sh[j] + sl.off : nullptr, *Yj = update ? h->Yh[j] + sl.off : nullptr;
+    const double *G = h->G + sl.off;
+    const double *Gk = update ? h->G_k + sl.off : nullptr;
+    double *Yj = update ? h->Yh[j] + sl.off : nullptr;
     double *tmp = h->lb_small + kGramNB * kGramNB;
-#define GP_LAUNCH(VECN, UPD) k_gram_pass<VECN, M, UPD><<<sl.grid, TPB, 0, h->stream>>>(sl.nu, alpha, P, G, D, Sj, Yj, p0, p1, p2, h->partials, h->ticket, tmp)
+#define GP_LAUNCH(VECN, UPD) k_gram_pass<VECN, M, UPD><<<sl.grid, TPB, 0, h->stream>>>(sl.nu, alpha, P, G, Gk, Yj, p0, p1, p2, h->partials, h->ticket, tmp)
     if (sl.vec == 2) { if (update) GP_LAUNCH(2, true); else GP_LAUNCH(2, false); }
     else { if (update) GP_LAUNCH(1, true); else GP_LAUNCH(1, false); }
 #undef GP_LAUNCH
@@ -337,29 +352,27 @@
 }
 
 template <int M>
-int32_t gram_form_m(sdplrp_handle *h, const Slice &sl, int jpre) {
+int32_t gram_form_m(sdplrp_handle *h, const Slice &sl) {
     const LbPtrs P = gram_ptrs(h, sl.off);
     const double *coef = h->lb_small + kGramNB * kGramNB + 3 * kGramNB;
     if (sl.vec == 2)
-        k_gram_form<2, M><<<sl.grid, TPB, 0, h->stream>>>(sl.nu, P, h->G + sl.off, coef, h->D + sl.off, h->Yh[jpre] + sl.off, jpre,
-                                                          h->partials, h->ticket, h->dscal + SC_DESCENT);
+        k_gram_form<2, M><<<sl.grid, TPB, 0, h->stream>>>(sl.nu, P, h->G + sl.off, coef, h->D + sl.off, h->partials, h->ticket, h->dscal + SC_DESCENT);
     else
-        k_gram_form<1, M><<<sl.grid, TPB, 0, h->stream>>>(sl.nu, P, h->G + sl.off, coef, h->D + sl.off, h->Yh[jpre] + sl.off, jpre,
-                                                          h->partials, h->ticket, h->dscal + SC_DESCENT);
+        k_gram_form<1, M><<<sl.grid, TPB, 0, h->stream>>>(sl.nu, P, h->G + sl.off, coef, h->D + sl.off, h->partials, h->ticket, h->dscal + SC_DESCENT);
     KLAUNCH(h);
     CUDA_TRY(h, cudaGetLastError());
     return SDPLRP_OK;
 }
-int32_t gram_form(sdplrp_handle *h, const Slice &sl, int jpre) {
+int32_t gram_form(sdplrp_handle *h, const Slice &sl) {
     switch (h->hist) {
-    case 1: return gram_form_m<1>(h, sl, jpre);
-    case 2: return gram_form_m<2>(h, sl, jpre);
-    case 3: return gram_form_m<3>(h, sl, jpre);
-    case 4: return gram_form_m<4>(h, sl, jpre);
-    case 5: return gram_form_m<5>(h, sl, jpre);
-    case 6: return gram_form_m<6>(h, sl, jpre);
-    case 7: return gram_form_m<7>(h, sl, jpre);
-    default: return gram_form_m<8>(h, sl, jpre);
+    case 1: return gram_form_m<1>(h, sl);
+    case 2: return gram_form_m<2>(h, sl);
+    case 3: return gram_form_m<3>(h, sl);
+    case 4: return gram_form_m<4>(h, sl);
+    case 5: return gram_form_m<5>(h, sl);
+    case 6: return gram_form_m<6>(h, sl);
+    case 7: return gram_form_m<7>(h, sl);
+    default: return gram_form_m<8>(h, sl);
     }
 }
 
@@ -377,15 +390,38 @@
     return SDPLRP_OK;
 }
 
+bool is_slot(const sdplrp_handle *h, const double *p) {
+    for (int j = 0; j < h->hist; j++)
+        if (p == h->Sh[j]) return true;
+    return false;
+}
+
+double *spare_buffer(const sdplrp_handle *h) { return h->G == h->G_mem ? h->D_mem : h->G_mem; }
+
+int32_t release_d(sdplrp_handle *h) {
+    if (!is_slot(h, h->D)) return SDPLRP_OK;
+    double *to = spare_buffer(h);
+    CUDA_TRY(h, cudaMemcpyAsync(to, h->D, (size_t)h->state_cap * sizeof(double), cudaMemcpyDeviceToDevice, h->stream));
+    h->D = to;
+    return SDPLRP_OK;
+}
+
 int32_t lb_dir_gram(sdplrp_handle *h) {
     const Slice sl = owned(h);
     const int M = h->hist;
+    const int jpre = h->latest % M;
+    if (h->G_k) {
+        CUDA_TRY(h, cudaMemcpyAsync(h->Yh[jpre] + sl.off, h->G_k + sl.off, (size_t)sl.len * sizeof(double), cudaMemcpyDeviceToDevice, h->stream));
+        DISPATCH_VEC(sl, k_scale_inplace, sl.nu, -1.0, h->Yh[jpre] + sl.off);
+        h->gram_pairs_valid = false;
+    }
     SDP_CHECK(gram_refresh(h, sl));
     double *coef = h->lb_small + kGramNB * kGramNB + 3 * kGramNB;
     k_gram_coef<<<1, 32, 0, h->stream>>>(M, h->latest, h->lb_small, h->dscal + SC_RHO, coef);
     KLAUNCH(h);
-    const int jpre = h->latest % M;
-    SDP_CHECK(gram_form(h, sl, jpre));
+    h->G_k = h->G;
+    h->D = h->Sh[jpre];
+    SDP_CHECK(gram_form(h, sl));
     SDP_CHECK(comm_reduce_ptr(h, h->dscal + SC_DESCENT, 1));
     h->gram_pairs_valid = false;
     h->gram_prestored = jpre;
@@ -396,6 +432,14 @@
     const Slice sl = owned(h);
     const int M = h->hist;
     const int j = h->latest % M;
+    if (!h->G_k) {
+        if (h->D != h->Sh[j]) {
+            CUDA_TRY(h, cudaMemcpyAsync(h->Sh[j], h->D, (size_t)h->state_cap * sizeof(double), cudaMemcpyDeviceToDevice, h->stream));
+            h->D = h->Sh[j];
+        }
+        DISPATCH_VEC(sl, k_scale_inplace, sl.nu, -1.0, h->Yh[j] + sl.off);
+        h->G_k = h->Yh[j];
+    }
     if (!h->gram_pairs_valid && h->gram_prestored != j) {
         for (int p = 0; p < 2 * M; p++) {
             if (p == j || p == M + j) continue;
@@ -403,6 +447,8 @@
         }
     }
     SDP_CHECK(gram_pass(h, sl, true, alpha, j, j, M + j, 2 * M));
+    h->lb_alpha[j] = alpha;
+    h->G_k = nullptr;
     h->gram_pairs_valid = true; h->gram_g_valid = true; h->gram_prestored = -1;
     h->latest = j + 1;
     return SDPLRP_OK;
@@ -476,6 +522,11 @@
 }
 
 int32_t lb_clear(sdplrp_handle *h) {
+    if (h->lb_implicit) {
+        SDP_CHECK(release_d(h));
+        h->G_k = nullptr;
+        for (int j = 0; j < kMaxHist; j++) h->lb_alpha[j] = 0.0;
+    }
     const size_t bytes = (size_t)h->n * h->r * sizeof(double);
     for (int j = 0; j < h->hist; j++) {
         CUDA_TRY(h, cudaMemsetAsync(h->Sh[j], 0, bytes, h->stream));
@@ -490,6 +541,57 @@
     return SDPLRP_OK;
 }
 
+double *lb_g_target(sdplrp_handle *h) {
+    if (h->G_k && h->G == h->G_k) h->G = (h->G_k == h->G_mem) ? h->D_mem : h->G_mem;
+    return h->G;
+}
+
+double *lb_d_target(sdplrp_handle *h) {
+    if (h->lb_implicit && !h->G_k && is_slot(h, h->D)) h->D = spare_buffer(h);
+    return h->D;
+}
+
+int32_t lb_layout_reset(sdplrp_handle *h, bool keep) {
+    h->G_k = nullptr;
+    if (keep && h->G_mem && h->D_mem) {
+        const Slice sl = {0, h->state_cap, h->state_cap, 1, grid_for(h->state_cap, TPB * 4, kRedBlocks)};
+        const size_t bytes = (size_t)h->state_cap * sizeof(double);
+        if (h->G == h->D_mem && h->D == h->G_mem) {
+            DISPATCH_VEC(sl, k_swap, sl.nu, h->G_mem, h->D_mem);
+        } else {
+            if (h->G != h->G_mem) CUDA_TRY(h, cudaMemcpyAsync(h->G_mem, h->G, bytes, cudaMemcpyDeviceToDevice, h->stream));
+            if (h->D != h->D_mem) CUDA_TRY(h, cudaMemcpyAsync(h->D_mem, h->D, bytes, cudaMemcpyDeviceToDevice, h->stream));
+        }
+        if (h->lb_implicit)
+            for (int j = 0; j < h->hist; j++)
+                if (h->lb_alpha[j] != 1.0) DISPATCH_VEC(sl, k_scale_inplace, sl.nu, h->lb_alpha[j], h->Sh[j]);
+    }
+    h->G = h->G_mem; h->D = h->D_mem;
+    for (int j = 0; j < kMaxHist; j++) h->lb_alpha[j] = 1.0;
+    h->lb_implicit = gram_enabled(h);
+    h->gram_pairs_valid = h->gram_g_valid = false; h->gram_prestored = -1;
+    CUDA_TRY(h, cudaGetLastError());
+    return SDPLRP_OK;
+}
+
+static int slot_of(const sdplrp_handle *h, int id) { return (id >= SDPLRP_MAT_S0 && id < SDPLRP_MAT_S0 + h->hist) ? id - SDPLRP_MAT_S0 : -1; }
+
+int32_t lb_slot_written(sdplrp_handle *h, int id) {
+    const int j = slot_of(h, id);
+    if (!h->lb_implicit || j < 0) return SDPLRP_OK;
+    if (h->D == h->Sh[j]) {
+        if (h->G_k) return fail(h, SDPLRP_ERR_STATE, "history slot s_" + std::to_string(j) + " holds the current direction until sdplrp_lbfgs_update");
+        SDP_CHECK(release_d(h));
+    }
+    h->lb_alpha[j] = 1.0;
+    return SDPLRP_OK;
+}
+
+double lb_slot_scale(const sdplrp_handle *h, int id) {
+    const int j = slot_of(h, id);
+    return (h->lb_implicit && j >= 0) ? h->lb_alpha[j] : 1.0;
+}
+
 int32_t lb_axpy(sdplrp_handle *h, double alpha, const double *x, double *y) {
     const Slice sl = owned(h);
     DISPATCH_VEC(sl, k_axpy, sl.nu, alpha, x + sl.off, y + sl.off);
@@ -506,7 +608,9 @@
 
 int32_t lb_neg_copy(sdplrp_handle *h) {
     const Slice sl = owned(h);
-    DISPATCH_VEC(sl, k_neg_copy, sl.nu, h->G + sl.off, h->D + sl.off);
+    const double *gin = h->G;
+    double *gout = lb_g_target(h), *d = lb_d_target(h);
+    DISPATCH_VEC(sl, k_neg_copy, sl.nu, gin + sl.off, gout + sl.off, d + sl.off);
     CUDA_TRY(h, cudaGetLastError());
     return SDPLRP_OK;
 }
```

Result: faster. 127.0 (median of 6 runs) (+4.1%).
